# techshoww/RoMa

Measured on AMD Instinct MI355X. Metric: image-pairs/sec at 560->864, higher is better.
Workload: dtype fp16; 1 GPU; roma_outdoor 560->864 full coarse-to-fine symmetric match (BASELINE configs[1]; configs[2] = --pairs 8 --gpus 8); launch=eager launches, coarse_res=560, upsample_res=864, parallelism=single GPU

## Files before the change

include/roma_hip.h:

```cpp
#ifndef ROMA_HIP_H
#define ROMA_HIP_H

#include <stdint.h>

#ifdef __cplusplus
extern "C" {
#endif

#define ROMA_ABI_VERSION 5

enum { ROMA_F32 = 0, ROMA_F16 = 1, ROMA_BF16 = 2 };
enum { ROMA_NCHW = 0, ROMA_NHWC = 1 };
enum { ROMA_LC_AUTO = 0, ROMA_LC_TILE8X4 = 1, ROMA_LC_TILE8X8 = 2, ROMA_LC_ROWS8 = 3 };
enum { ROMA_E_ARG = -1, ROMA_E_DTYPE = -2, ROMA_E_SHAPE = -3, ROMA_E_ALIGN = -4, ROMA_E_UNSUPPORTED = -5 };

int roma_abi_version(void);
const char* roma_last_error(void);

int roma_local_corr(const void* f0, const void* f1, const float* flow, void* out,
                    int B, int C, int H, int W, int r, int dtype,
                    int layout, int f0_pitch, int f1_pitch, int out_layout, int out_pitch, int f1_batch_shift, int variant,
                    void* stream);

int roma_warp_bilinear(const void* src, const float* flow, void* dst,
                       int B, int C, int Hs, int Ws, int H, int W, int dtype,
                       int layout, int src_pitch, int dst_layout, int dst_pitch, int src_batch_shift, void* stream);

int roma_disp_emb(const float* flow, const float* weight, const float* bias, void* dst,
                  int B, int E, int H, int W, float gain, int dtype, int dst_layout, int dst_pitch, void* stream);

int roma_interp_bilinear(const float* x, float* y, int N, int Hi, int Wi, int Ho, int Wo, void* stream);

int roma_interp_bilinear_pair(const float* x0, float* y0, int N0, const float* x1, float* y1, int N1, int Hi, int Wi, int Ho, int Wo,
                              void* stream);

int roma_refiner_assemble(const void* src, const float* flow, const float* weight, const float* bias, void* buf, int B, int C, int E,
                          int D, int pitch, int Hs, int Ws, int H, int W, int src_pitch, int src_batch_shift, float gain, int dtype,
                          void* stream);

int roma_flow_update(float* flow, float* cert, const float* cert_in, const float* delta,
                     int B, int H, int W, float sx, float sy, void* stream);

int roma_cls_to_flow_refine(const void* logits, float* flow_out, float* cert_out,
                            int B, int C, int HW, long stride_b, long stride_c, long stride_p,
                            int dtype, void* stream);

int roma_cos_kernel(const void* x, const void* y, float* K, int B, int N, int M, int D, int dtype, int x_pitch, int y_pitch,
                    int y_batch_shift, float T, float eps, float diag_add, void* stream);

int roma_chol_diag_block(float* A, int lda, long strideA, float* W, int ldw, long strideW, int nb, int B, int* info,
                         int info_base, void* stream);

int roma_chol_step(float* A, int lda, long strideA, int n, int ncols, int j, int nb, const float* W, int ldw, long strideW, float* R,
                   int ldr, long strideR, float* Wn, int ldwn, long strideWn, int* info, int info_base, int B, void* stream);

int roma_chol_subst_step(int dir, const float* W, int ldw, long strideW, const float* R, long strideRb, long strideRs, int ldr, float* T,
                         long strideTb, long strideTs, int ldt, int t_in_panel, float* X, int ldx, long strideX, int n, int m, int nb,
                         int s, int B, void* stream);

int roma_attention_fwd(const void* q, const void* k, const void* v, void* o, int B, int H, int Nq, int Nk, int head_dim, long q_sb,
                       long q_sn, long q_sh, long k_sb, long k_sn, long k_sh, long v_sb, long v_sn, long v_sh, long o_sb, long o_sn,
                       long o_sh, float scale, int dtype, void* stream);

int roma_match_finalize(const float* flow, const float* cert, const float* cert16, float* warp, float* certainty,
                        int P, int H, int W, int H16, int W16, int symmetric, void* stream);

int roma_kde_density(const float* x, float* density, int N, int down, float std, int half_mode, void* stream);

int roma_race_keys(const float* p, const long* counter, float* keys, long N, float thresh, unsigned seed, unsigned stage,
                   void* stream);

long roma_race_select_workspace(int P, long N, int k);
int roma_race_select(const float* p, const long* counter, const long* seeds, int P, long N, int k, float thresh, unsigned stage,
                     long* sel_key, long* sel_idx, void* workspace, long workspace_bytes, void* stream);

int roma_kde_density_batch(const float* x, const long* index, float* density, int P, long N, int n, int down, float std,
                           int half_mode, void* stream);

int roma_nn_argmin(const float* q, const float* r, int* idx, int NQ, int NR, void* stream);

int roma_resample_u8(const void* in, void* out, int H, int W, int C, int out_size, int axis, const int* bounds,
                     const int* coef, int ksize, void* stream);
int roma_normalize_u8(const void* in, float* out, int H, int W, const float* mean3, const float* std3, void* stream);

int roma_bias_relu_nchw(void* x, const void* bias, int B, int C, int HW, int dtype, void* stream);

int roma_bias_relu_pool2_nchw(void* x, const void* bias, void* pooled, int B, int C, int H, int W, int dtype, void* stream);

int roma_bias_relu_nhwc(void* x, const void* bias, long npix, int C, int dtype, void* stream);
int roma_bias_relu_pool2_nhwc(void* x, const void* bias, void* pooled, int B, int C, int H, int W, int dtype, void* stream);

int roma_dwconv5x5_bn_relu(const void* x, const float* w, const float* scale, const float* shift, void* y,
                           int B, int C, int H, int W, int dtype, int x_pitch, int y_pitch, void* stream);

int roma_refiner_block(const void* x, const void* w25, const float* scale, const float* shift, const void* wt,
                       const float* bias, void* y, int B, int C, int H, int W, int kpad, int dtype, int x_pitch, int y_pitch,
                       void* stream);

int roma_refiner_wide_pack(const void* wt, void* wp, int D);
int roma_refiner_wide_taps(const void* w25, void* w25p, int D);
int roma_refiner_block_wide(const void* x, const void* w25p, const float* scale, const float* shift, const void* wp,
                            const float* bias, void* y, int B, int H, int W, int D, int x_pitch, int y_pitch, int dtype,
                            void* stream);

int roma_pointwise_mfma(const void* x, const void* wt, const float* bias, void* y, long M, int C, int kpad, int dtype,
                        int x_pitch, int y_pitch, void* stream);

int roma_refiner_block_mid(const void* x, const float* w25, const float* scale, const float* shift, const void* wt,
                           const float* bias, void* y, int B, int C, int H, int W, int dtype, int x_pitch, int y_pitch,
                           void* stream);

int roma_refiner_head(const void* x, const float* wo, const float* bo, float* flow, const float* cert_in, float* cert_out,
                      float* delta_out, int B, int H, int W, int C, int pitch, int dtype, float sx, float sy, void* stream);

int roma_pointwise_small(const void* x, const float* wt, const float* bias, void* y, long M, int C, int dtype,
                         int x_pitch, int y_pitch, void* stream);

int roma_project_skinny(const void* x, const void* wt, const float* bias, void* y, long M, int K, int N, int dtype, int x_pitch,
                        int y_pitch, void* stream);

int roma_add_layernorm(void* x, int x_dtype, long x_stride, const void* y, int y_dtype, long y_stride, const float* ls,
                       const float* gamma, const float* beta, void* out, int out_dtype, long out_stride, long rows, int C,
                       float eps, void* stream);

int roma_tiny_corr_posembed(const float* f0, const float* f1, float* out, int B, int C,
                            int H0, int W0, int H1, int W1, int exact, void* stream);

int roma_jpeg_info(const void* data, long nbytes, int* info);
int roma_jpeg_entropy_decode(const void* data, long nbytes, int16_t* coef, uint16_t* qt);
int roma_jpeg_reconstruct(const int16_t* coef, const uint16_t* qt, void* planes, void* rgb, const int* info, void* stream);

long roma_ransac_workspace(int kind, int P, int N, int iters, long* offsets);
int roma_ransac_hypotheses(int kind, const double* xa, const double* xb, int P, int N, int iters, float threshold, unsigned seed,
                           int p0, void* ws, long ws_bytes, void* stream);
int roma_ransac_select(int kind, const double* xa, const double* xb, int P, int N, int iters, float threshold, int lo_iters,
                       const void* ws, long ws_bytes, double* model, unsigned char* mask, void* stream);

int roma_ransac_hypotheses_ex(int kind, const double* xa, const double* xb, int P, int N, int iters, float threshold, int scoring,
                              unsigned seed, int p0, void* ws, long ws_bytes, void* stream);
int roma_ransac_select_ex(int kind, const double* xa, const double* xb, int P, int N, int iters, float threshold, int scoring,
                          int lo_iters, const void* ws, long ws_bytes, double* model, unsigned char* mask, void* stream);
int roma_magsac_table(float* loss, float* weight);

long roma_essential_workspace(int P, int N, int iters, long* offsets);
int roma_essential_hypotheses(const double* xa, const double* xb, const double* Ka, const double* Kb, int P, int N, int iters,
                              float threshold, unsigned seed, int p0, void* ws, long ws_bytes, void* stream);
int roma_essential_select(const double* xa, const double* xb, const double* Ka, const double* Kb, int P, int N, int iters,
                          float threshold, int lo_iters, const void* ws, long ws_bytes, double* E, unsigned char* mask, void* stream);
int roma_recover_pose(const double* xa, const double* xb, const double* Ka, const double* Kb, const double* E,
                      const unsigned char* mask_in, int P, int N, double* R, double* t, int* count, unsigned char* mask_out,
                      void* stream);

int roma_essential_hypotheses_ex(const double* xa, const double* xb, const double* Ka, const double* Kb, int P, int N, int iters,
                                 float threshold, int scoring, unsigned seed, int p0, void* ws, long ws_bytes, void* stream);
int roma_essential_select_ex(const double* xa, const double* xb, const double* Ka, const double* Kb, int P, int N, int iters,
                             float threshold, int scoring, int lo_iters, const void* ws, long ws_bytes, double* E, unsigned char* mask,
                             void* stream);

int roma_refine_pose(const double* xa, const double* xb, const double* Ka, const double* Kb, const double* R_in, const double* t_in,
                     const unsigned char* mask_in, int P, int N, double threshold, int iters, double* R, double* t,
                     unsigned char* mask, double* cost, int* count, int* steps, void* stream);

int roma_refine_fundamental(const double* xa, const double* xb, const double* F_in, const unsigned char* mask_in, int P, int N,
                            double threshold, int iters, double* F, unsigned char* mask, double* cost, int* count, int* steps,
                            void* stream);

int roma_refine_homography(const double* xa, const double* xb, const double* H_in, const unsigned char* mask_in, int P, int N,
                           double threshold, int iters, double* H, unsigned char* mask, double* cost, int* count, int* steps,
                           void* stream);

long roma_absolute_pose_workspace(int P, int N, int iters, long* offsets);
int roma_absolute_pose_hypotheses(const double* X, const double* x, const double* K, int P, int N, int iters, float threshold,
                                  int scoring, unsigned seed, int p0, void* ws, long ws_bytes, void* stream);
int roma_absolute_pose_select(const double* X, const double* x, const double* K, int P, int N, int iters, float threshold, int scoring,
                              int lo_iters, const void* ws, long ws_bytes, double* R, double* t, unsigned char* mask, void* stream);
int roma_refine_absolute_pose(const double* X, const double* x, const double* K, const double* R_in, const double* t_in,
                              const unsigned char* mask_in, int P, int N, double threshold, int iters, double* R, double* t,
                              unsigned char* mask, double* cost, int* count, int* steps, void* stream);

int roma_triangulate(const float* m, const float* to_px, const double* Ka, const double* Kb, const double* R, const double* t,
                     const unsigned char* mask_in, int P, int N, int method, float max_reproj, float max_cos_parallax, float* points,
                     float* depth_a, float* depth_b, float* reproj, float* cos_parallax, unsigned char* valid, void* stream);

int roma_triangulate_nview(const float* const* obs, const float* to_px, const unsigned char* const* visible, long vis_row_stride,
                           const double* K, const double* R, const double* t, int V, int rows, int row_len, long row_stride,
                           long point_stride, float max_view_error, int iters, int min_views, int ref_view, float max_reproj,
                           float max_cos_parallax, float* points, float* depth, float* reproj, float* cos_parallax, unsigned* views,
                           unsigned char* valid, void* stream);

int roma_warp_kpts(const float* x, int x_stride, const float* depth_a, const float* depth_b, const double* T, const double* Ka,
                   const double* Kb, int P, int N, int Ha, int Wa, int Hb, int Wb, int mode, double threshold, double* x2,
                   unsigned char* valid, double* rel_err, void* stream);

int roma_dense_match_metrics(const float* warp, long pitch, const float* depth_a, const float* depth_b, const double* T,
                             const double* Ka, const double* Kb, int P, int H, int W, int Ha, int Wa, int Hb, int Wb, int mode,
                             double threshold, void* workspace, long workspace_bytes, double* epe_sum, long long* counts, double* gd,
                             unsigned char* valid, void* stream);

#ifdef __cplusplus
}
#endif
#endif
```

roma_amd/_lib.py:

```python
from __future__ import annotations

import ctypes
import os
from ctypes import c_char_p, c_float, c_int, c_long, c_void_p

_HERE = os.path.dirname(os.path.abspath(__file__))
LIB_PATH = os.path.join(_HERE, "csrc", "libroma_hip.so")

ROMA_F32, ROMA_F16, ROMA_BF16 = 0, 1, 2
ROMA_NCHW, ROMA_NHWC = 0, 1
LC_VARIANTS = {"auto": 0, "tile8x4": 1, "tile8x8": 2, "rows8": 3}
ABI_VERSION = 5
SCORE_MSAC, SCORE_MAGSAC = 0, 1
ROMA_E_ARG, ROMA_E_DTYPE, ROMA_E_SHAPE, ROMA_E_ALIGN, ROMA_E_UNSUPPORTED = -1, -2, -3, -4, -5

SIGNATURES = {
    "roma_abi_version": [],
    "roma_last_error": [],
    "roma_local_corr": [c_void_p, c_void_p, c_void_p, c_void_p, c_int, c_int, c_int, c_int, c_int, c_int,
                        c_int, c_int, c_int, c_int, c_int, c_int, c_int, c_void_p],
    "roma_warp_bilinear": [c_void_p, c_void_p, c_void_p, c_int, c_int, c_int, c_int, c_int, c_int, c_int,
                           c_int, c_int, c_int, c_int, c_int, c_void_p],
    "roma_disp_emb": [c_void_p, c_void_p, c_void_p, c_void_p, c_int, c_int, c_int, c_int, c_float, c_int, c_int, c_int, c_void_p],
    "roma_interp_bilinear": [c_void_p, c_void_p, c_int, c_int, c_int, c_int, c_int, c_void_p],
    "roma_interp_bilinear_pair": [c_void_p, c_void_p, c_int, c_void_p, c_void_p, c_int, c_int, c_int, c_int, c_int, c_void_p],
    "roma_refiner_assemble": [c_void_p, c_void_p, c_void_p, c_void_p, c_void_p, c_int, c_int, c_int, c_int, c_int, c_int, c_int, c_int,
                              c_int, c_int, c_int, c_float, c_int, c_void_p],
    "roma_project_skinny": [c_void_p, c_void_p, c_void_p, c_void_p, c_long, c_int, c_int, c_int, c_int, c_int, c_void_p],
    "roma_flow_update": [c_void_p, c_void_p, c_void_p, c_void_p, c_int, c_int, c_int, c_float, c_float, c_void_p],
    "roma_cls_to_flow_refine": [c_void_p, c_void_p, c_void_p, c_int, c_int, c_int, c_long, c_long, c_long, c_int, c_void_p],
    "roma_cos_kernel": [c_void_p, c_void_p, c_void_p, c_int, c_int, c_int, c_int, c_int, c_int, c_int, c_int, c_float, c_float,
                        c_float, c_void_p],
    "roma_add_layernorm": [c_void_p, c_int, c_long, c_void_p, c_int, c_long, c_void_p, c_void_p, c_void_p, c_void_p, c_int, c_long,
                           c_long, c_int, c_float, c_void_p],
    "roma_attention_fwd": [c_void_p, c_void_p, c_void_p, c_void_p, c_int, c_int, c_int, c_int, c_int] + [c_long] * 12 + [c_float, c_int, c_void_p],
    "roma_chol_diag_block": [c_void_p, c_int, c_long, c_void_p, c_int, c_long, c_int, c_int, c_void_p, c_int, c_void_p],
    "roma_chol_step": [c_void_p, c_int, c_long, c_int, c_int, c_int, c_int, c_void_p, c_int, c_long, c_void_p, c_int, c_long,
                       c_void_p, c_int, c_long, c_void_p, c_int, c_int, c_void_p],
    "roma_chol_subst_step": [c_int, c_void_p, c_int, c_long, c_void_p, c_long, c_long, c_int, c_void_p, c_long, c_long, c_int, c_int,
                             c_void_p, c_int, c_long, c_int, c_int, c_int, c_int, c_int, c_void_p],
    "roma_match_finalize": [c_void_p, c_void_p, c_void_p, c_void_p, c_void_p, c_int, c_int, c_int, c_int, c_int, c_int, c_void_p],
    "roma_kde_density": [c_void_p, c_void_p, c_int, c_int, c_float, c_int, c_void_p],
    "roma_nn_argmin": [c_void_p, c_void_p, c_void_p, c_int, c_int, c_void_p],
    "roma_race_keys": [c_void_p, c_void_p, c_void_p, c_long, c_float, ctypes.c_uint, ctypes.c_uint, c_void_p],
    "roma_race_select_workspace": [c_int, c_long, c_int],
    "roma_race_select": [c_void_p, c_void_p, c_void_p, c_int, c_long, c_int, c_float, ctypes.c_uint, c_void_p, c_void_p, c_void_p, c_long,
                         c_void_p],
    "roma_kde_density_batch": [c_void_p, c_void_p, c_void_p, c_int, c_long, c_int, c_int, c_float, c_int, c_void_p],
    "roma_dwconv5x5_bn_relu": [c_void_p, c_void_p, c_void_p, c_void_p, c_void_p, c_int, c_int, c_int, c_int, c_int, c_int, c_int, c_void_p],
    "roma_resample_u8": [c_void_p, c_void_p, c_int, c_int, c_int, c_int, c_int, c_void_p, c_void_p, c_int, c_void_p],
    "roma_normalize_u8": [c_void_p, c_void_p, c_int, c_int, c_void_p, c_void_p, c_void_p],
    "roma_bias_relu_nchw": [c_void_p, c_void_p, c_int, c_int, c_int, c_int, c_void_p],
    "roma_bias_relu_pool2_nchw": [c_void_p, c_void_p, c_void_p, c_int, c_int, c_int, c_int, c_int, c_void_p],
    "roma_bias_relu_nhwc": [c_void_p, c_void_p, c_long, c_int, c_int, c_void_p],
    "roma_bias_relu_pool2_nhwc": [c_void_p, c_void_p, c_void_p, c_int, c_int, c_int, c_int, c_int, c_void_p],
    "roma_pointwise_mfma": [c_void_p, c_void_p, c_void_p, c_void_p, c_long, c_int, c_int, c_int, c_int, c_int, c_void_p],
    "roma_refiner_block": [c_void_p, c_void_p, c_void_p, c_void_p, c_void_p, c_void_p, c_void_p, c_int, c_int, c_int, c_int, c_int, c_int,
                           c_int, c_int, c_void_p],
    "roma_refiner_block_mid": [c_void_p, c_void_p, c_void_p, c_void_p, c_void_p, c_void_p, c_void_p, c_int, c_int, c_int, c_int, c_int, c_int,
                               c_int, c_void_p],
    "roma_refiner_wide_pack": [c_void_p, c_void_p, c_int],
    "roma_refiner_wide_taps": [c_void_p, c_void_p, c_int],
    "roma_jpeg_info": [c_void_p, c_long, c_void_p],
    "roma_jpeg_entropy_decode": [c_void_p, c_long, c_void_p, c_void_p],
    "roma_jpeg_reconstruct": [c_void_p, c_void_p, c_void_p, c_void_p, c_void_p, c_void_p],
    "roma_refiner_block_wide": [c_void_p, c_void_p, c_void_p, c_void_p, c_void_p, c_void_p, c_void_p, c_int, c_int, c_int, c_int, c_int, c_int,
                                c_int, c_void_p],
    "roma_refiner_head": [c_void_p, c_void_p, c_void_p, c_void_p, c_void_p, c_void_p, c_void_p, c_int, c_int, c_int, c_int, c_int, c_int,
                          c_float, c_float, c_void_p],
    "roma_pointwise_small": [c_void_p, c_void_p, c_void_p, c_void_p, c_long, c_int, c_int, c_int, c_int, c_void_p],
    "roma_tiny_corr_posembed": [c_void_p, c_void_p, c_void_p, c_int, c_int, c_int, c_int, c_int, c_int, c_int, c_void_p],
    "roma_ransac_workspace": [c_int, c_int, c_int, c_int, c_void_p],
    "roma_ransac_hypotheses": [c_int, c_void_p, c_void_p, c_int, c_int, c_int, c_float, ctypes.c_uint, c_int, c_void_p, c_long, c_void_p],
    "roma_ransac_select": [c_int, c_void_p, c_void_p, c_int, c_int, c_int, c_float, c_int, c_void_p, c_long, c_void_p, c_void_p,
                           c_void_p],
    "roma_ransac_hypotheses_ex": [c_int, c_void_p, c_void_p, c_int, c_int, c_int, c_float, c_int, ctypes.c_uint, c_int, c_void_p, c_long,
                                  c_void_p],
    "roma_ransac_select_ex": [c_int, c_void_p, c_void_p, c_int, c_int, c_int, c_float, c_int, c_int, c_void_p, c_long, c_void_p, c_void_p,
                              c_void_p],
    "roma_magsac_table": [c_void_p, c_void_p],
    "roma_essential_workspace": [c_int, c_int, c_int, c_void_p],
    "roma_essential_hypotheses": [c_void_p, c_void_p, c_void_p, c_void_p, c_int, c_int, c_int, c_float, ctypes.c_uint, c_int, c_void_p,
                                  c_long, c_void_p],
    "roma_essential_select": [c_void_p, c_void_p, c_void_p, c_void_p, c_int, c_int, c_int, c_float, c_int, c_void_p, c_long, c_void_p,
                              c_void_p, c_void_p],
    "roma_essential_hypotheses_ex": [c_void_p, c_void_p, c_void_p, c_void_p, c_int, c_int, c_int, c_float, c_int, ctypes.c_uint, c_int,
                                     c_void_p, c_long, c_void_p],
    "roma_essential_select_ex": [c_void_p, c_void_p, c_void_p, c_void_p, c_int, c_int, c_int, c_float, c_int, c_int, c_void_p, c_long,
                                 c_void_p, c_void_p, c_void_p],
    "roma_recover_pose": [c_void_p, c_void_p, c_void_p, c_void_p, c_void_p, c_void_p, c_int, c_int, c_void_p, c_void_p, c_void_p,
                          c_void_p, c_void_p],
    "roma_refine_pose": [c_void_p, c_void_p, c_void_p, c_void_p, c_void_p, c_void_p, c_void_p, c_int, c_int, ctypes.c_double, c_int,
                         c_void_p, c_void_p, c_void_p, c_void_p, c_void_p, c_void_p, c_void_p],
    "roma_refine_fundamental": [c_void_p, c_void_p, c_void_p, c_void_p, c_int, c_int, ctypes.c_double, c_int, c_void_p, c_void_p, c_void_p,
                                c_void_p, c_void_p, c_void_p],
    "roma_refine_homography": [c_void_p, c_void_p, c_void_p, c_void_p, c_int, c_int, ctypes.c_double, c_int, c_void_p, c_void_p, c_void_p,
                               c_void_p, c_void_p, c_void_p],
    "roma_triangulate": [c_void_p, c_void_p, c_void_p, c_void_p, c_void_p, c_void_p, c_void_p, c_int, c_int, c_int, c_float, c_float,
                         c_void_p, c_void_p, c_void_p, c_void_p, c_void_p, c_void_p, c_void_p],
    "roma_triangulate_nview": [c_void_p, c_void_p, c_void_p, c_long, c_void_p, c_void_p, c_void_p, c_int, c_int, c_int, c_long, c_long,
                               c_float, c_int, c_int, c_int, c_float, c_float, c_void_p, c_void_p, c_void_p, c_void_p, c_void_p, c_void_p,
                               c_void_p],
    "roma_warp_kpts": [c_void_p, c_int, c_void_p, c_void_p, c_void_p, c_void_p, c_void_p, c_int, c_int, c_int, c_int, c_int, c_int, c_int,
                       ctypes.c_double, c_void_p, c_void_p, c_void_p, c_void_p],
    "roma_dense_match_metrics": [c_void_p, c_long, c_void_p, c_void_p, c_void_p, c_void_p, c_void_p, c_int, c_int, c_int, c_int, c_int, c_int,
                                 c_int, c_int, ctypes.c_double, c_void_p, c_long, c_void_p, c_void_p, c_void_p, c_void_p, c_void_p],
    "roma_absolute_pose_workspace": [c_int, c_int, c_int, c_void_p],
    "roma_absolute_pose_hypotheses": [c_void_p, c_void_p, c_void_p, c_int, c_int, c_int, c_float, c_int, ctypes.c_uint, c_int, c_void_p,
                                      c_long, c_void_p],
    "roma_absolute_pose_select": [c_void_p, c_void_p, c_void_p, c_int, c_int, c_int, c_float, c_int, c_int, c_void_p, c_long, c_void_p,
                                  c_void_p, c_void_p, c_void_p],
    "roma_refine_absolute_pose": [c_void_p, c_void_p, c_void_p, c_void_p, c_void_p, c_void_p, c_int, c_int, ctypes.c_double, c_int,
                                  c_void_p, c_void_p, c_void_p, c_void_p, c_void_p, c_void_p, c_void_p],
}
_RESTYPES = {"roma_last_error": c_char_p, "roma_ransac_workspace": c_long, "roma_essential_workspace": c_long,
             "roma_race_select_workspace": c_long, "roma_absolute_pose_workspace": c_long}

_lib = None


class RomaHipError(RuntimeError):
    pass


def load() -> ctypes.CDLL:
    global _lib
    if _lib is not None:
        return _lib
    if not os.path.exists(LIB_PATH):
        raise RomaHipError(f"{LIB_PATH} is missing: build it with `python -c 'import __graft_entry__ as g; g.build()'` "
                           f"or `make -C roma_amd/csrc`.  roma_amd has no CPU/PyTorch fallback for its kernels.")
    lib = ctypes.CDLL(LIB_PATH)
    for name, argtypes in SIGNATURES.items():
        fn = getattr(lib, name)
        fn.argtypes = argtypes
        fn.restype = _RESTYPES.get(name, c_int)
    if lib.roma_abi_version() != ABI_VERSION:
        raise RomaHipError(f"libroma_hip.so ABI {lib.roma_abi_version()} != binding ABI {ABI_VERSION}")
    _lib = lib
    return lib


def check(rc: int, what: str):
    if rc == 0:
        return
    msg = load().roma_last_error().decode(errors="replace")
    if rc < 0:
        raise ValueError(f"{what}: {msg} (code {rc})")
    raise RomaHipError(f"{what}: HIP error {rc}: {msg}")
```

roma_amd/csrc/refiner_block.hip:

```cpp
#include <algorithm>
#include "common.h"
#include "lc_device.h"
#include "refiner_mid_device.h"

namespace roma {
namespace {

typedef _Float16 h8v __attribute__((ext_vector_type(8)));
typedef __bf16 b8v __attribute__((ext_vector_type(8)));

__device__ __forceinline__ float4_t mfma_blk(const u32x4& a, const u32x4& b, float4_t c, half_t) {
  return __builtin_amdgcn_mfma_f32_16x16x32_f16(__builtin_bit_cast(h8v, a), __builtin_bit_cast(h8v, b), c, 0, 0, 0);
}
__device__ __forceinline__ float4_t mfma_blk(const u32x4& a, const u32x4& b, float4_t c, bf16_t) {
  return __builtin_amdgcn_mfma_f32_16x16x32_bf16(__builtin_bit_cast(b8v, a), __builtin_bit_cast(b8v, b), c, 0, 0, 0);
}

struct RBParams {
  const void* x;
  void* y;
  const void* w25;
  const void* wt;
  const float* scale;
  const float* shift;
  const float* bias;
  int B, H, W, C, x_pitch, y_pitch;
  int tiles_x, tiles_y;
  float inv_tiles_per_img, inv_tiles_x;
};

constexpr int XT = 16, YT = 8, HX = XT + 4, HY = YT + 4, NPOS = HX * HY;

template <typename T, int KP>
__global__ __launch_bounds__(256, 1) void refiner_block_kernel(RBParams p) {
  constexpr int KPAD = 32 * KP;
  constexpr int NT = KPAD / 16;
  constexpr int RS = KPAD / 8 + 1;
  extern __shared__ __attribute__((aligned(16))) unsigned char smem[];
  u32x4* s_in = reinterpret_cast<u32x4*>(smem);
  u32x4* s_pw = s_in + NPOS * RS;
  u32x4* s_dw = s_pw + KPAD * RS;
  float* s_cs = reinterpret_cast<float*>(s_dw + 25 * (KPAD / 8));
  T* s_out = reinterpret_cast<T*>(s_in);
  constexpr int OS = KPAD + 8;

  const int tid = threadIdx.x, lane = tid & 63, wv = tid >> 6;
  const int m = lane & 15, kq = lane >> 4;
  const int PKT = p.C / 8;
  const T* x = static_cast<const T*>(p.x);
  T* y = static_cast<T*>(p.y);
  const int tiles_per_img = p.tiles_x * p.tiles_y;
  auto tile_origin = [&](int tile, int& b, int& ty0, int& tx0) {
    b = (int)(((float)tile + 0.5f) * p.inv_tiles_per_img);
    const int tt = tile - b * tiles_per_img;
    const int tyi = (int)(((float)tt + 0.5f) * p.inv_tiles_x);
    ty0 = tyi * YT;
    tx0 = (tt - tyi * p.tiles_x) * XT;
  };

  for (int i = tid; i < KPAD * (KPAD / 8); i += 256) {
    const int n = i / (KPAD / 8), k = i % (KPAD / 8);
    s_pw[n * RS + k] = reinterpret_cast<const u32x4*>(p.wt)[i];
  }
  for (int i = tid; i < 25 * (KPAD / 8); i += 256) s_dw[i] = reinterpret_cast<const u32x4*>(p.w25)[i];
  for (int i = tid; i < KPAD; i += 256) {
    s_cs[i] = p.scale[i];
    s_cs[KPAD + i] = p.shift[i];
    s_cs[2 * KPAD + i] = p.bias[i];
  }
  const int ntile = p.tiles_x * p.tiles_y * p.B;
  constexpr int NLD = (NPOS * (KPAD / 8) + 255) / 256;
  const int nload = NPOS * PKT;
  u32x4 pre[NLD];
  auto fetch = [&](int tile) {
    int b, ty0, tx0;
    tile_origin(tile, b, ty0, tx0);
    const T* xb = x + (size_t)b * p.H * p.W * p.x_pitch;
#pragma unroll
    for (int j = 0; j < NLD; ++j) {
      const int i = min(tid + j * 256, nload - 1);
      const int pos = i / PKT, k = i - pos * PKT;
      const int yy = ty0 - 2 + pos / HX, xx = tx0 - 2 + pos % HX;
      const bool ok = yy >= 0 && yy < p.H && xx >= 0 && xx < p.W;
      const int yc = min(max(yy, 0), p.H - 1), xc = min(max(xx, 0), p.W - 1);
      u32x4 v = *reinterpret_cast<const u32x4*>(xb + ((size_t)yc * p.W + xc) * p.x_pitch + k * 8);
      if (!ok) v = u32x4{0, 0, 0, 0};
      pre[j] = v;
    }
  };
  for (int i = tid; i < NPOS * (KPAD / 8 - PKT); i += 256) {
    const int pos = i / (KPAD / 8 - PKT), k = PKT + i % (KPAD / 8 - PKT);
    s_in[pos * RS + k] = u32x4{0, 0, 0, 0};
  }
  if ((int)blockIdx.x < ntile) fetch(blockIdx.x);
  for (int tile = blockIdx.x; tile < ntile; tile += gridDim.x) {
    int b, ty0, tx0;
    tile_origin(tile, b, ty0, tx0);
    __syncthreads();
#pragma unroll
    for (int j = 0; j < NLD; ++j) {
      const int i = tid + j * 256;
      if (i < nload) {
        const int pos = i / PKT, k = i - pos * PKT;
        s_in[pos * RS + k] = pre[j];
      }
    }
    __syncthreads();
    if (tile + (int)gridDim.x < ntile) fetch(tile + gridDim.x);
    u32x4 afrag[2][KP];
#pragma unroll
    for (int ks = 0; ks < KP; ++ks) {
      const int pk = 4 * ks + kq;
      float acc0[8], acc1[8];
#pragma unroll
      for (int e = 0; e < 8; ++e) acc0[e] = acc1[e] = 0.f;
#pragma unroll
      for (int dy = 0; dy < 6; ++dy) {
#pragma unroll
        for (int dx = 0; dx < 5; ++dx) {
          float fi[8];
          unpack16<T>(s_in[((2 * wv + dy) * HX + m + dx) * RS + pk], fi);
          if (dy < 5) {
            float fw[8];
            unpack16<T>(s_dw[(dy * 5 + dx) * (KPAD / 8) + pk], fw);
#pragma unroll
            for (int e = 0; e < 8; ++e) acc0[e] = __builtin_fmaf(fi[e], fw[e], acc0[e]);
          }
          if (dy >= 1) {
            float fw[8];
            unpack16<T>(s_dw[((dy - 1) * 5 + dx) * (KPAD / 8) + pk], fw);
#pragma unroll
            for (int e = 0; e < 8; ++e) acc1[e] = __builtin_fmaf(fi[e], fw[e], acc1[e]);
          }
        }
      }
      float v0[8], v1[8];
#pragma unroll
      for (int e = 0; e < 8; ++e) {
        const float sc = s_cs[pk * 8 + e], sh = s_cs[KPAD + pk * 8 + e];
        v0[e] = fmaxf(__builtin_fmaf(acc0[e], sc, sh), 0.f);
        v1[e] = fmaxf(__builtin_fmaf(acc1[e], sc, sh), 0.f);
      }
      afrag[0][ks] = pack16<T>(v0);
      afrag[1][ks] = pack16<T>(v1);
    }
    float4_t acc[2][NT];
#pragma unroll
    for (int nt = 0; nt < NT; ++nt) acc[0][nt] = acc[1][nt] = float4_t{0.f, 0.f, 0.f, 0.f};
#pragma unroll
    for (int nt = 0; nt < NT; ++nt) {
#pragma unroll
      for (int ks = 0; ks < KP; ++ks) {
        const u32x4 bfrag = s_pw[(nt * 16 + m) * RS + 4 * ks + kq];
        acc[0][nt] = mfma_blk(afrag[0][ks], bfrag, acc[0][nt], T{});
        acc[1][nt] = mfma_blk(afrag[1][ks], bfrag, acc[1][nt], T{});
      }
    }
    __syncthreads();
#pragma unroll
    for (int row = 0; row < 2; ++row)
#pragma unroll
      for (int nt = 0; nt < NT; ++nt) {
        const int ch = nt * 16 + m;
        const float bsv = s_cs[2 * KPAD + ch];
#pragma unroll
        for (int r4 = 0; r4 < 4; ++r4)
          s_out[((2 * wv + row) * XT + 4 * kq + r4) * OS + ch] = from_f32<T>(acc[row][nt][r4] + bsv);
      }
    __syncthreads();
    T* yb = y + (size_t)b * p.H * p.W * p.y_pitch;
    for (int i = tid; i < XT * YT * PKT; i += 256) {
      const int pix = i / PKT, k = i - pix * PKT;
      const int yy = ty0 + pix / XT, xx = tx0 + pix % XT;
      if (yy < p.H && xx < p.W)
        *reinterpret_cast<u32x4*>(yb + ((size_t)yy * p.W + xx) * p.y_pitch + k * 8) = *reinterpret_cast<const u32x4*>(s_out + pix * OS + k * 8);
    }
  }
}

template <typename T, int KP>
int launch_rb(RBParams p, hipStream_t s) {
  constexpr int KPAD = 32 * KP, RS = KPAD / 8 + 1;
  const size_t smem = (size_t)(NPOS * RS + KPAD * RS + 25 * (KPAD / 8)) * 16 + 3 * KPAD * 4;
  static std::atomic<uint64_t> attr_done{0};
  if (int rc = ensure_dyn_smem(reinterpret_cast<const void*>(refiner_block_kernel<T, KP>), (int)smem, attr_done, "roma_refiner_block")) return rc;
  const long ntile = (long)p.B * p.tiles_x * p.tiles_y;
  ROMA_REQUIRE(ntile < (1 << 21), ROMA_E_SHAPE, "roma_refiner_block: %ld tiles in one launch (< 2^21)", ntile);
  p.inv_tiles_per_img = 1.0f / (float)(p.tiles_x * p.tiles_y);
  p.inv_tiles_x = 1.0f / (float)p.tiles_x;
  const int per_cu = KP == 1 ? 4 : 1;
  const int grid = ntile < 256 * per_cu ? (int)ntile : 256 * per_cu;
  hipLaunchKernelGGL((refiner_block_kernel<T, KP>), dim3(grid), dim3(256), smem, s, p);
  ROMA_CHECK_LAUNCH();
}


constexpr int TPX = 16, TPY = 16, TPHX = TPX + 4, TPHY = TPY + 4;
constexpr int TP_PR = 64;
constexpr int TP_PLB = TPHY * TP_PR;
constexpr int TP_NCH = 24, TP_FRAG = 13 * 16;
constexpr int TP_TROW = TPX * 64 + 16;
constexpr int TP_OS = 40;
constexpr int TP_TOEP = TP_NCH * 5 * TP_FRAG;
constexpr int TP_PL = TP_NCH * TP_PLB, TP_TB = TPX * TPY * TP_OS * 2, TP_PW = 32 * 5 * 16;
constexpr int TP_SMEM = TP_TOEP + TP_PL + TP_TB + TP_PW + 3 * 32 * 4;
static_assert(TPY * TP_TROW <= TP_TB && 2 * TP_SMEM <= 160 * 1024, "LDS budget of the Toeplitz block: two workgroups per CU");

template <typename T>
__global__ __launch_bounds__(256, 2) void refiner_block_toep_kernel(RBParams p) {
  extern __shared__ __attribute__((aligned(16))) unsigned char smem[];
  unsigned char* s_toep = smem;
  unsigned char* s_pl = s_toep + TP_TOEP;
  unsigned char* s_t = s_pl + TP_PL;
  u32x4* s_pw = reinterpret_cast<u32x4*>(s_t + TP_TB);
  float* s_cs = reinterpret_cast<float*>(s_pw + 32 * 5);
  const int tid = threadIdx.x, lane = tid & 63;
  const int wv = __builtin_amdgcn_readfirstlane(tid >> 6);
  const int m = lane & 15, q = lane >> 4;
  const T* x = static_cast<const T*>(p.x);
  T* y = static_cast<T*>(p.y);
  const int tiles_per_img = p.tiles_x * p.tiles_y;
  auto tile_origin = [&](int tile, int& b, int& ty0, int& tx0) {
    b = (int)(((float)tile + 0.5f) * p.inv_tiles_per_img);
    const int tt = tile - b * tiles_per_img;
    const int tyi = (int)(((float)tt + 0.5f) * p.inv_tiles_x);
    ty0 = tyi * TPY;
    tx0 = (tt - tyi * p.tiles_x) * TPX;
  };

  {
    const T* w25 = static_cast<const T*>(p.w25);
    for (int i = tid; i < TP_NCH * 5 * 13; i += 256) {
      const int f = i / 13, wi = i - f * 13, c = f / 5, dy = f - c * 5;
      T v[8];
#pragma unroll
      for (int j = 0; j < 8; ++j) {
        const int dx = wi - 7 + j;
        v[j] = (wi < 12 && dx >= 0 && dx <= 4) ? w25[(dy * 5 + dx) * 32 + c] : from_f32<T>(0.f);
      }
      *reinterpret_cast<u32x4*>(s_toep + (size_t)i * 16) = *reinterpret_cast<const u32x4*>(v);
    }
    for (int i = tid; i < 32 * 4; i += 256) s_pw[(i >> 2) * 5 + (i & 3)] = reinterpret_cast<const u32x4*>(p.wt)[i];
    if (tid < 32) { s_cs[tid] = p.scale[tid]; s_cs[32 + tid] = p.shift[tid]; s_cs[64 + tid] = p.bias[tid]; }
    for (int i = tid; i < (TP_PL + TP_TB) / 16; i += 256) reinterpret_cast<u32x4*>(s_pl)[i] = u32x4{0, 0, 0, 0};
  }
  const int ntile = tiles_per_img * p.B;
  constexpr int NLD = (TPHX * TPHY * 3 + 255) / 256;
  u32x4 pre[NLD];
  uint32_t okm = 0;
  uint32_t pdst[NLD];
  int ihy[NLD], ihx[NLD], ik8[NLD];
#pragma unroll
  for (int j = 0; j < NLD; ++j) {
    const int idx = tid + 256 * j, idc = min(idx, TPHX * TPHY * 3 - 1);
    const int k = idc / (TPHX * TPHY), pos = idc - k * (TPHX * TPHY), hy = pos / TPHX, hx = pos - hy * TPHX;
    pdst[j] = idx < TPHX * TPHY * 3 ? (uint32_t)(k * 8 * TP_PLB + hy * TP_PR + hx * 2) : 0xffffffffu;
    ihy[j] = hy - 2; ihx[j] = hx - 2; ik8[j] = k * 8;
  }
  auto fetch = [&](int tile) {
    int b, ty0, tx0;
    tile_origin(tile, b, ty0, tx0);
    const T* xb = x + (size_t)b * p.H * p.W * p.x_pitch;
    okm = 0xffffffffu;
#pragma unroll
    for (int j = 0; j < NLD; ++j) {
      const int yy = ty0 + ihy[j], xx = tx0 + ihx[j];
      if (!(yy >= 0 && yy < p.H && xx >= 0 && xx < p.W)) okm &= ~(1u << j);
      pre[j] = *reinterpret_cast<const u32x4*>(xb + (uint32_t)((min(max(yy, 0), p.H - 1) * p.W + min(max(xx, 0), p.W - 1)) * p.x_pitch + ik8[j]));
    }
  };
  auto scatter = [&]() {
#pragma unroll
    for (int j = 0; j < NLD; ++j) {
      if (pdst[j] == 0xffffffffu) continue;
      const bool ok = (okm >> j) & 1u;
#pragma unroll
      for (int e = 0; e < 8; ++e) {
        const uint32_t w = ok ? pre[j][e >> 1] : 0u;
        *reinterpret_cast<uint16_t*>(s_pl + pdst[j] + e * TP_PLB) = (uint16_t)((e & 1) ? (w >> 16) : (w & 0xffffu));
      }
    }
  };
  const bool xcd_order = (gridDim.x & 7) == 0 && ntile >= 64;
  const int nx = xcd_order ? (int)(gridDim.x >> 3) : (int)gridDim.x;
  const int band = xcd_order ? (ntile + 7) >> 3 : ntile;
  const int t_beg = xcd_order ? (int)(blockIdx.x & 7) * band + (int)(blockIdx.x >> 3) : (int)blockIdx.x;
  const int t_end = xcd_order ? min(((int)(blockIdx.x & 7) + 1) * band, ntile) : ntile;
  if (t_beg < t_end) fetch(t_beg);
  __syncthreads();
  if (t_beg < t_end) scatter();
  if (t_beg + nx < t_end) fetch(t_beg + nx);
  __syncthreads();

  const int swz = (m >> 1) & 3;
  const int wsh = 8 * q - m;
  const int woff = (wsh >= -7 && wsh <= 4 ? wsh + 7 : 12) * 16;
  float scv[8], shv[8], bsv4[2][4];
#pragma unroll
  for (int e = 0; e < 8; ++e) { scv[e] = s_cs[min(wv, 2) * 8 + e]; shv[e] = s_cs[32 + min(wv, 2) * 8 + e]; }
#pragma unroll
  for (int nb = 0; nb < 2; ++nb)
#pragma unroll
    for (int i = 0; i < 4; ++i) bsv4[nb][i] = s_cs[64 + nb * 16 + 4 * q + i];
  for (int tile = t_beg; tile < t_end; tile += nx) {
    int b, ty0, tx0;
    tile_origin(tile, b, ty0, tx0);
    const bool more = tile + nx < t_end, more2 = tile + 2 * nx < t_end;
    if (wv < 3) {
      float vals[8][4];
      u32x4 av[5], bv[5];
      auto load_op = [&](int c, int dy, u32x4& a, u32x4& bq) {
        a = *reinterpret_cast<const u32x4*>(s_toep + (c * 5 + dy) * TP_FRAG + woff);
        bq = *reinterpret_cast<const u32x4*>(s_pl + c * TP_PLB + (m + dy) * TP_PR + q * 16);
      };
#pragma unroll
      for (int dy = 0; dy < 5; ++dy) load_op(wv * 8, dy, av[dy], bv[dy]);
#pragma unroll
      for (int e = 0; e < 8; ++e) {
        const int c = wv * 8 + e;
        u32x4 an[5], bn[5];
        float4_t acc = {0.f, 0.f, 0.f, 0.f};
#pragma unroll
        for (int dy = 0; dy < 5; ++dy) {
          __builtin_amdgcn_sched_barrier(0);
          acc = lc::mfma16r(av[dy], bv[dy], acc, T{});
          if (e < 7) load_op(c + 1, dy, an[dy], bn[dy]);
        }
        __builtin_amdgcn_sched_barrier(0);
#pragma unroll
        for (int i = 0; i < 4; ++i) vals[e][i] = fmaxf(__builtin_fmaf(acc[i], scv[e], shv[e]), 0.f);
        if (e < 7) {
#pragma unroll
          for (int dy = 0; dy < 5; ++dy) { av[dy] = an[dy]; bv[dy] = bn[dy]; }
        }
      }
#pragma unroll
      for (int i = 0; i < 4; ++i) {
        float f8[8];
#pragma unroll
        for (int e = 0; e < 8; ++e) f8[e] = vals[e][i];
        const int xo = 4 * q + i;
        *reinterpret_cast<u32x4*>(s_t + m * TP_TROW + xo * 64 + ((wv ^ ((xo >> 1) & 3)) << 4)) = pack16<T>(f8);
      }
    }
    __syncthreads();
    float4_t acc2[4][2];
#pragma unroll
    for (int r = 0; r < 4; ++r) {
      const u32x4 tb = *reinterpret_cast<const u32x4*>(s_t + (wv * 4 + r) * TP_TROW + m * 64 + ((q ^ swz) << 4));
#pragma unroll
      for (int nb = 0; nb < 2; ++nb) acc2[r][nb] = lc::mfma16r(s_pw[(nb * 16 + m) * 5 + q], tb, float4_t{0.f, 0.f, 0.f, 0.f}, T{});
    }
    __syncthreads();
    T* s_out = reinterpret_cast<T*>(s_t);
#pragma unroll
    for (int r = 0; r < 4; ++r)
#pragma unroll
      for (int nb = 0; nb < 2; ++nb) {
        T o4[4];
#pragma unroll
        for (int i = 0; i < 4; ++i) o4[i] = from_f32<T>(acc2[r][nb][i] + bsv4[nb][i]);
        *reinterpret_cast<uint2*>(s_out + ((wv * 4 + r) * TPX + m) * TP_OS + nb * 16 + 4 * q) = *reinterpret_cast<const uint2*>(o4);
      }
    if (more) scatter();
    if (more2) fetch(tile + 2 * nx);
    __syncthreads();
    T* yb = y + (size_t)b * p.H * p.W * p.y_pitch;
#pragma unroll
    for (int j = 0; j < 3; ++j) {
      const int i = tid + 256 * j, pix = i / 3, k = i - pix * 3;
      const int yy = ty0 + (pix >> 4), xx = tx0 + (pix & 15);
      if (yy < p.H && xx < p.W)
        *reinterpret_cast<u32x4*>(yb + ((size_t)yy * p.W + xx) * p.y_pitch + k * 8) = *reinterpret_cast<const u32x4*>(s_out + pix * TP_OS + k * 8);
    }
    __syncthreads();
    for (int i = tid; i < TPX * TPY; i += 256) {
      const int row = i >> 4, xo = i & 15;
      *reinterpret_cast<u32x4*>(s_t + row * TP_TROW + xo * 64 + ((3 ^ ((xo >> 1) & 3)) << 4)) = u32x4{0, 0, 0, 0};
    }
  }
}

template <typename T>
int launch_rb_toep(RBParams p, hipStream_t s) {
  static std::atomic<uint64_t> attr_done{0};
  if (int rc = ensure_dyn_smem(reinterpret_cast<const void*>(refiner_block_toep_kernel<T>), TP_SMEM, attr_done, "roma_refiner_block")) return rc;
  p.tiles_x = (p.W + TPX - 1) / TPX;
  p.tiles_y = (p.H + TPY - 1) / TPY;
  const long ntile = (long)p.B * p.tiles_x * p.tiles_y;
  ROMA_REQUIRE(ntile < (1 << 21), ROMA_E_SHAPE, "roma_refiner_block: %ld tiles in one launch (< 2^21)", ntile);
  p.inv_tiles_per_img = 1.0f / (float)(p.tiles_x * p.tiles_y);
  p.inv_tiles_x = 1.0f / (float)p.tiles_x;
  const int grid = ntile < 2 * num_cus() ? (int)ntile : 2 * num_cus();
  hipLaunchKernelGGL((refiner_block_toep_kernel<T>), dim3(grid), dim3(256), TP_SMEM, s, p);
  ROMA_CHECK_LAUNCH();
}

template <typename T>
int launch_rb_any(const RBParams& p, int kpad, hipStream_t s) {
  if (kpad == 32 && p.C == 24) return launch_rb_toep<T>(p, s);
  return kpad == 32 ? launch_rb<T, 1>(p, s) : launch_rb<T, 5>(p, s);
}



struct PWParams {
  const void* x;
  void* y;
  const void* wt;
  const float* bias;
  long M;
  int C, x_pitch, y_pitch;
};

template <typename T, int KP>
__global__ __launch_bounds__(256, 2) void pointwise_mfma_kernel(PWParams p) {
  constexpr int KPAD = 32 * KP, RS = KPAD / 8 + 1, OS = KPAD + 8;
  extern __shared__ __attribute__((aligned(16))) unsigned char smem[];
  u32x4* s_pw = reinterpret_cast<u32x4*>(smem);
  float* s_b = reinterpret_cast<float*>(s_pw + KPAD * RS);
  T* s_out = reinterpret_cast<T*>(s_b + KPAD);
  const int tid = threadIdx.x, lane = tid & 63, wv = tid >> 6;
  const int m = lane & 15, kq = lane >> 4;
  const int PKT = p.C / 8;
  for (int i = tid; i < KPAD * (KPAD / 8); i += 256) {
    const int n = i / (KPAD / 8), k = i % (KPAD / 8);
    s_pw[n * RS + k] = reinterpret_cast<const u32x4*>(p.wt)[i];
  }
  for (int i = tid; i < KPAD; i += 256) s_b[i] = p.bias[i];
  __syncthreads();
  const T* x = static_cast<const T*>(p.x);
  T* y = static_cast<T*>(p.y);
  T* so = s_out + wv * 16 * OS;
  const long ntile = (p.M + 15) / 16;
  for (long tile = (long)blockIdx.x * 4 + wv; tile < ntile; tile += (long)gridDim.x * 4) {
    const long row0 = tile * 16;
    const long r = row0 + m < p.M ? row0 + m : p.M - 1;
    u32x4 a[1][KP];
#pragma unroll
    for (int ks = 0; ks < KP; ++ks) {
      const int pk = 4 * ks + kq;
      u32x4 v = *reinterpret_cast<const u32x4*>(x + r * p.x_pitch + (pk < PKT ? pk : 0) * 8);
      if (pk >= PKT) v = u32x4{0, 0, 0, 0};
      a[0][ks] = v;
    }
    T* const stage[1] = {so};
    mid::pw_row_groups<T, KP, 1>(a, s_pw, s_b, stage, m, kq);
    for (int i = lane; i < 16 * PKT; i += 64) {
      const int row = i / PKT, k = i - row * PKT;
      if (row0 + row < p.M) *reinterpret_cast<u32x4*>(y + (row0 + row) * p.y_pitch + k * 8) = *reinterpret_cast<const u32x4*>(so + row * OS + k * 8);
    }
  }
}

template <typename T, int KP>
int launch_pw(const PWParams& p, hipStream_t s) {
  constexpr int KPAD = 32 * KP, RS = KPAD / 8 + 1, OS = KPAD + 8;
  const size_t smem = (size_t)KPAD * RS * 16 + KPAD * 4 + (size_t)4 * 16 * OS * sizeof(T);
  static std::atomic<uint64_t> attr_done{0};
  if (int rc = ensure_dyn_smem(reinterpret_cast<const void*>(pointwise_mfma_kernel<T, KP>), (int)smem, attr_done, "roma_pointwise_mfma")) return rc;
  const long need = (p.M + 63) / 64;
  const int grid = (int)(need < 512 ? need : 512);
  hipLaunchKernelGGL((pointwise_mfma_kernel<T, KP>), dim3(grid), dim3(256), smem, s, p);
  ROMA_CHECK_LAUNCH();
}

}
}

using namespace roma;

extern "C" int roma_refiner_block(const void* x, const void* w25, const float* scale, const float* shift, const void* wt,
                                  const float* bias, void* y, int B, int C, int H, int W, int kpad, int dtype, int x_pitch, int y_pitch,
                                  void* stream) {
  ROMA_REQUIRE(x && w25 && scale && shift && wt && bias && y, ROMA_E_ARG, "roma_refiner_block: null pointer");
  ROMA_REQUIRE(B > 0 && C > 0 && H > 0 && W > 0 && x_pitch >= C && y_pitch >= C, ROMA_E_SHAPE, "roma_refiner_block: bad shape");
  ROMA_REQUIRE(dtype == ROMA_F16 || dtype == ROMA_BF16, ROMA_E_DTYPE, "roma_refiner_block: fp16 / bf16 only (the fp32 parity mode uses the separate kernels)");
  ROMA_REQUIRE((kpad == 32 || kpad == 160) && C <= kpad && C % 8 == 0, ROMA_E_UNSUPPORTED, "roma_refiner_block: C=%d, kpad=%d (kpad must be 32 or 160, C a multiple of 8)", C, kpad);
  ROMA_REQUIRE(x_pitch % 8 == 0 && y_pitch % 8 == 0 && aligned16(x) && aligned16(y) && aligned16(w25) && aligned16(wt), ROMA_E_ALIGN,
               "roma_refiner_block: pitches must be multiples of 8 and bases 16-byte aligned");
  RBParams p{x, y, w25, wt, scale, shift, bias, B, H, W, C, x_pitch, y_pitch, (W + XT - 1) / XT, (H + YT - 1) / YT, 0.f, 0.f};
  hipStream_t s = static_cast<hipStream_t>(stream);
  return dtype == ROMA_F16 ? launch_rb_any<half_t>(p, kpad, s) : launch_rb_any<bf16_t>(p, kpad, s);
}

extern "C" int roma_pointwise_mfma(const void* x, const void* wt, const float* bias, void* y, long M, int C, int kpad, int dtype,
                                   int x_pitch, int y_pitch, void* stream) {
  ROMA_REQUIRE(x && wt && bias && y, ROMA_E_ARG, "roma_pointwise_mfma: null pointer");
  ROMA_REQUIRE(M > 0 && C > 0 && x_pitch >= C && y_pitch >= C, ROMA_E_SHAPE, "roma_pointwise_mfma: bad shape");
  ROMA_REQUIRE(dtype == ROMA_F16 || dtype == ROMA_BF16, ROMA_E_DTYPE, "roma_pointwise_mfma: fp16 / bf16 only");
  ROMA_REQUIRE((kpad == 32 || kpad == 160) && C <= kpad && C % 8 == 0, ROMA_E_UNSUPPORTED, "roma_pointwise_mfma: C=%d, kpad=%d", C, kpad);
  ROMA_REQUIRE(x_pitch % 8 == 0 && y_pitch % 8 == 0 && aligned16(x) && aligned16(y) && aligned16(wt), ROMA_E_ALIGN,
               "roma_pointwise_mfma: pitches must be multiples of 8 and bases 16-byte aligned");
  PWParams p{x, y, wt, bias, M, C, x_pitch, y_pitch};
  hipStream_t s = static_cast<hipStream_t>(stream);
  if (dtype == ROMA_F16) return kpad == 32 ? launch_pw<half_t, 1>(p, s) : launch_pw<half_t, 5>(p, s);
  return kpad == 32 ? launch_pw<bf16_t, 1>(p, s) : launch_pw<bf16_t, 5>(p, s);
}
```

roma_amd/csrc/refiner_head.hip:

```cpp
#include "common.h"

namespace roma {
namespace {

template <typename T, int L>
__global__ __launch_bounds__(256) void refiner_head_kernel(const T* __restrict__ x, const float* __restrict__ wo,
                                                          const float* __restrict__ bo, float* __restrict__ flow,
                                                          const float* __restrict__ cert_in, float* __restrict__ cert_out,
                                                          float* __restrict__ delta_out, int B, int HW, int C, int pitch, float sx, float sy) {
  constexpr int E = ElemTraits<T>::kPer16B;
  const int PK = C / E;
  const size_t M = (size_t)B * HW;
  const int sub = threadIdx.x % L;
  for (size_t m = ((size_t)blockIdx.x * blockDim.x + threadIdx.x) / L; m < M; m += (size_t)gridDim.x * blockDim.x / L) {
    float a0 = 0.f, a1 = 0.f, a2 = 0.f;
    for (int pk = sub; pk < PK; pk += L) {
      float f[E];
      unpack16<T>(*reinterpret_cast<const u32x4*>(x + m * pitch + pk * E), f);
      const float* w = wo + (size_t)pk * E * 3;
#pragma unroll
      for (int e = 0; e < E; ++e) {
        a0 = __builtin_fmaf(f[e], w[e * 3 + 0], a0);
        a1 = __builtin_fmaf(f[e], w[e * 3 + 1], a1);
        a2 = __builtin_fmaf(f[e], w[e * 3 + 2], a2);
      }
    }
#pragma unroll
    for (int o = L / 2; o > 0; o >>= 1) {
      a0 += __shfl_xor(a0, o, 64);
      a1 += __shfl_xor(a1, o, 64);
      a2 += __shfl_xor(a2, o, 64);
    }
    if (sub == 0) {
      a0 += bo[0]; a1 += bo[1]; a2 += bo[2];
      const int b = (int)(m / HW);
      const size_t p = m - (size_t)b * HW;
      float* fl = flow + (size_t)b * 2 * HW + p;
      fl[0] += sx * a0;
      fl[HW] += sy * a1;
      cert_out[m] = (cert_in ? cert_in[m] : 0.f) + a2;
      if (delta_out) {
        delta_out[(size_t)b * 3 * HW + p] = a0;
        delta_out[(size_t)b * 3 * HW + HW + p] = a1;
        delta_out[(size_t)b * 3 * HW + 2 * (size_t)HW + p] = a2;
      }
    }
  }
}

}
}

using namespace roma;

extern "C" int roma_refiner_head(const void* x, const float* wo, const float* bo, float* flow, const float* cert_in, float* cert_out,
                                 float* delta_out, int B, int H, int W, int C, int pitch, int dtype, float sx, float sy, void* stream) {
  ROMA_REQUIRE(x && wo && bo && flow && cert_out, ROMA_E_ARG, "roma_refiner_head: null pointer");
  ROMA_REQUIRE(B > 0 && H > 0 && W > 0 && C > 0 && pitch >= C, ROMA_E_SHAPE, "roma_refiner_head: bad shape");
  ROMA_REQUIRE(dtype >= ROMA_F32 && dtype <= ROMA_BF16, ROMA_E_DTYPE, "roma_refiner_head: unknown dtype %d", dtype);
  const int e = dtype == ROMA_F32 ? 4 : 8;
  ROMA_REQUIRE(C % e == 0 && pitch % e == 0 && aligned16(x), ROMA_E_ALIGN, "roma_refiner_head: C and pitch must be multiples of %d, x 16-byte aligned", e);
  hipStream_t s = static_cast<hipStream_t>(stream);
  const int pk = C / e;
  const int L = pk >= 64 ? 64 : (pk >= 16 ? 16 : 4);
  const size_t threads = (size_t)B * H * W * L;
  size_t g = (threads + 255) / 256;
  if (g > 32768) g = 32768;
#define ROMA_RH(T, LL) \
  hipLaunchKernelGGL((refiner_head_kernel<T, LL>), dim3((int)g), dim3(256), 0, s, (const T*)x, wo, bo, flow, cert_in, cert_out, delta_out, B, H * W, C, pitch, sx, sy)
#define ROMA_RH_T(T) \
  if (L == 64) { ROMA_RH(T, 64); } else if (L == 16) { ROMA_RH(T, 16); } else { ROMA_RH(T, 4); }
  if (dtype == ROMA_F32) { ROMA_RH_T(float) } else if (dtype == ROMA_F16) { ROMA_RH_T(half_t) } else { ROMA_RH_T(bf16_t) }
#undef ROMA_RH_T
#undef ROMA_RH
  ROMA_CHECK_LAUNCH();
}
```

roma_amd/csrc/refiner_mid.hip:

```cpp
#include "common.h"
#include "refiner_mid_device.h"

namespace roma {
namespace {

constexpr int MID_NT = 512;
constexpr int MID_KP = 5, MID_KPAD = 32 * MID_KP;
constexpr int MID_RS = MID_KPAD / 8 + 1;
constexpr int MID_SMAX = 28, MID_ROWS = MID_SMAX * mid::kStrip;
constexpr int MID_SMEM = (MID_ROWS * MID_RS + MID_KPAD * MID_RS) * 16 + 25 * MID_KPAD * 4 + MID_KPAD * 4 + MID_ROWS * 4 + 16 * (MID_KPAD / 8) * 4;
static_assert(MID_SMEM <= 160 * 1024, "LDS budget: t 75.3 KB + weights 53.8 KB + taps 16 KB + bias + the two index tables");
static_assert(MID_ROWS % 16 == 0 && MID_ROWS / 16 <= 16, "a wave takes row groups wv and wv + 8");

struct MidParams {
  const void* x;
  void* y;
  const float* w25;
  const float* scale;
  const float* shift;
  const void* wt;
  const float* bias;
  int B, H, W, C, x_pitch, y_pitch;
  int S;
  unsigned nstrip, ntile, band;
};

template <typename T>
__global__ __launch_bounds__(MID_NT) void refiner_mid_kernel(MidParams p) {
  constexpr int RS = MID_RS, OS = MID_KPAD + 8;
  static_assert(OS == RS * 8, "a staged output row is one row of t");
  extern __shared__ __attribute__((aligned(16))) unsigned char smem[];
  u32x4* s_t = reinterpret_cast<u32x4*>(smem);
  u32x4* s_pw = s_t + MID_ROWS * RS;
  float* s_w = reinterpret_cast<float*>(s_pw + MID_KPAD * RS);
  float* s_b = s_w + 25 * MID_KPAD;
  int* s_pix = reinterpret_cast<int*>(s_b + MID_KPAD);
  int* s_item = s_pix + MID_ROWS;
  const int tid = threadIdx.x;
  const int wv = __builtin_amdgcn_readfirstlane(tid >> 6);
  const int C = p.C, H = p.H, W = p.W, PK = C / 8, S = p.S;

  for (int i = tid; i < MID_KPAD * (MID_KPAD / 8); i += MID_NT) {
    const int n = i / (MID_KPAD / 8), k = i % (MID_KPAD / 8);
    s_pw[n * RS + k] = reinterpret_cast<const u32x4*>(p.wt)[i];
  }
  for (int i = tid; i < 25 * C / 4; i += MID_NT) reinterpret_cast<float4_t*>(s_w)[i] = reinterpret_cast<const float4_t*>(p.w25)[i];
  for (int i = tid; i < MID_KPAD; i += MID_NT) s_b[i] = p.bias[i];
  for (int i = tid; i < MID_ROWS; i += MID_NT) s_pix[i] = -1;
  for (int i = tid; i < 16 * (MID_KPAD / 8); i += MID_NT) s_item[i] = i < 16 * PK ? (i / PK) << 8 | (i % PK) : -1;
  __syncthreads();

  const T* x = static_cast<const T*>(p.x);
  T* y = static_cast<T*>(p.y);
  const unsigned WS = (unsigned)(W + mid::kStrip - 1) / mid::kStrip;
  const int sl = tid / PK, k = tid - sl * PK;
  const int ngrp = (S * mid::kStrip + 15) / 16;
  const unsigned nx = gridDim.x >> 3;
  const unsigned beg = (blockIdx.x & 7u) * p.band;
  const unsigned end = min(beg + p.band, p.ntile);
  for (unsigned tile = beg + (blockIdx.x >> 3); tile < end; tile += nx) {
    if (sl < S) {
      const unsigned strip = tile * (unsigned)S + (unsigned)sl;
      if (strip < p.nstrip) {
        unsigned r = strip;
        const int xs = (int)(r % WS) * mid::kStrip;
        r /= WS;
        const int ys = (int)(r % (unsigned)H), b = (int)(r / (unsigned)H);
        u32x4* trow = s_t + sl * mid::kStrip * RS + k;
        mid::dw_strip<T>(x, s_w, p.scale, p.shift, b, ys, xs, k * 8, C, H, W, p.x_pitch, mid::kStrip,
                         [&](int o, const u32x4& v) { trow[o * RS] = v; });
        if (k == 0) {
          const int pix0 = (b * H + ys) * W + xs;
#pragma unroll
          for (int o = 0; o < mid::kStrip; ++o) s_pix[sl * mid::kStrip + o] = xs + o < W ? pix0 + o : -1;
        }
      } else if (k == 0) {
#pragma unroll
        for (int o = 0; o < mid::kStrip; ++o) s_pix[sl * mid::kStrip + o] = -1;
      }
    }
    __syncthreads();
    int lane = tid & 63;
    asm volatile("" : "+v"(lane));
    const int m = lane & 15, kq = lane >> 4;
    auto fragments = [&](int g, u32x4 (&a)[MID_KP]) {
#pragma unroll
      for (int ks = 0; ks < MID_KP; ++ks) {
        const int pk = 4 * ks + kq;
        u32x4 v = s_t[(g * 16 + m) * RS + (pk < PK ? pk : 0)];
        if (pk >= PK) v = u32x4{0, 0, 0, 0};
        a[ks] = v;
      }
    };
    auto store_groups = [&](const int (&g)[2], auto ng) {
      constexpr int G = decltype(ng)::value, NIT = 16 * (MID_KPAD / 8) / 64;
      int item[NIT], pix[G][NIT];
#pragma unroll
      for (int j = 0; j < NIT; ++j) item[j] = s_item[lane + 64 * j];
#pragma unroll
      for (int q = 0; q < G; ++q)
#pragma unroll
        for (int j = 0; j < NIT; ++j) pix[q][j] = item[j] >= 0 ? s_pix[g[q] * 16 + (item[j] >> 8)] : -1;
#pragma unroll
      for (int q = 0; q < G; ++q) {
        const T* so = reinterpret_cast<const T*>(s_t + g[q] * 16 * RS);
#pragma unroll
        for (int j = 0; j < NIT; ++j)
          if (pix[q][j] >= 0)
            *reinterpret_cast<u32x4*>(y + (size_t)pix[q][j] * p.y_pitch + (item[j] & 255) * 8) =
                *reinterpret_cast<const u32x4*>(so + (item[j] >> 8) * OS + (item[j] & 255) * 8);
      }
    };
    if (wv + 8 < ngrp) {
      u32x4 a[2][MID_KP];
      fragments(wv, a[0]);
      fragments(wv + 8, a[1]);
      T* const stage[2] = {reinterpret_cast<T*>(s_t + wv * 16 * RS), reinterpret_cast<T*>(s_t + (wv + 8) * 16 * RS)};
      mid::pw_row_groups<T, MID_KP, 2>(a, s_pw, s_b, stage, m, kq);
      store_groups({wv, wv + 8}, std::integral_constant<int, 2>{});
    } else if (wv < ngrp) {
      u32x4 a[1][MID_KP];
      fragments(wv, a[0]);
      T* const stage[1] = {reinterpret_cast<T*>(s_t + wv * 16 * RS)};
      mid::pw_row_groups<T, MID_KP, 1>(a, s_pw, s_b, stage, m, kq);
      store_groups({wv, wv}, std::integral_constant<int, 1>{});
    }
    __syncthreads();
  }
}

template <typename T>
int launch_mid(MidParams p, hipStream_t s) {
  static std::atomic<uint64_t> attr_done{0};
  if (int rc = ensure_dyn_smem(reinterpret_cast<const void*>(refiner_mid_kernel<T>), MID_SMEM, attr_done, "roma_refiner_block_mid")) return rc;
  const int cus = num_cus() & ~7;
  ROMA_REQUIRE(cus >= 8, ROMA_E_UNSUPPORTED, "roma_refiner_block_mid: needs a device with at least 8 compute units");
  const unsigned want = (p.ntile + 7u) & ~7u;
  const int grid = want < (unsigned)cus ? (int)want : cus;
  hipLaunchKernelGGL((refiner_mid_kernel<T>), dim3(grid), dim3(MID_NT), MID_SMEM, s, p);
  ROMA_CHECK_LAUNCH();
}

}
}

using namespace roma;

extern "C" int roma_refiner_block_mid(const void* x, const float* w25, const float* scale, const float* shift, const void* wt,
                                      const float* bias, void* y, int B, int C, int H, int W, int dtype, int x_pitch, int y_pitch,
                                      void* stream) {
  ROMA_REQUIRE(x && w25 && scale && shift && wt && bias && y, ROMA_E_ARG, "roma_refiner_block_mid: null pointer");
  ROMA_REQUIRE(B > 0 && C > 0 && H > 0 && W > 0 && x_pitch >= C && y_pitch >= C, ROMA_E_SHAPE, "roma_refiner_block_mid: bad shape");
  ROMA_REQUIRE(dtype == ROMA_F16 || dtype == ROMA_BF16, ROMA_E_DTYPE, "roma_refiner_block_mid: fp16 / bf16 only");
  ROMA_REQUIRE(C > 32 && C <= MID_KPAD && C % 8 == 0, ROMA_E_UNSUPPORTED,
               "roma_refiner_block_mid: C=%d (a multiple of 8, 32 < C <= 160)", C);
  ROMA_REQUIRE(x_pitch % 8 == 0 && y_pitch % 8 == 0 && aligned16(x) && aligned16(y) && aligned16(w25) && aligned16(scale) &&
                   aligned16(shift) && aligned16(wt),
               ROMA_E_ALIGN, "roma_refiner_block_mid: pitches must be multiples of 8 and bases 16-byte aligned");
  const size_t npix = (size_t)B * H * W;
  ROMA_REQUIRE(npix * x_pitch * 2 < (1ull << 32) && npix * y_pitch * 2 < (1ull << 32), ROMA_E_SHAPE,
               "roma_refiner_block_mid: a map of 4 GB or more in one launch");
  const char *xb = static_cast<const char*>(x), *yb = static_cast<const char*>(y);
  ROMA_REQUIRE(yb + npix * y_pitch * 2 <= xb || xb + npix * x_pitch * 2 <= yb, ROMA_E_ARG, "roma_refiner_block_mid: x and y overlap");
  MidParams p{x, y, w25, scale, shift, wt, bias, B, H, W, C, x_pitch, y_pitch, 0, 0, 0, 0};
  const int S0 = MID_NT / (C / 8);
  p.S = S0 < MID_SMAX ? S0 : MID_SMAX;
  p.nstrip = (unsigned)((size_t)B * H * ((W + mid::kStrip - 1) / mid::kStrip));
  p.ntile = (p.nstrip + p.S - 1) / p.S;
  p.band = (p.ntile + 7) / 8;
  hipStream_t s = static_cast<hipStream_t>(stream);
  return dtype == ROMA_F16 ? launch_mid<half_t>(p, s) : launch_mid<bf16_t>(p, s);
}
```

roma_amd/csrc/refiner_wide.hip:

```cpp
#include "common.h"
#include "lc_device.h"

namespace roma {
namespace {

using lc::mfma16r;

struct RWParams {
  const void* x;
  void* y;
  const void* w25p;
  const void* wp;
  const float* scale;
  const float* shift;
  const float* bias;
  int B, H, W, x_pitch, y_pitch, tiles_x, tiles_y;
};

typedef const __attribute__((address_space(4))) float cfloat;
__device__ __forceinline__ cfloat* as_const(const float* p) { return (cfloat*)(uintptr_t)p; }

constexpr int TW = 16, TH = 8, HXW = TW + 4, HYH = TH + 4, HPR = 16;
constexpr int PLANE = HYH * HPR * 32 + 16;
constexpr int NTAPV = 5 * 4 * 2 * 6;

template <typename T, int D>
__global__ __launch_bounds__(512, 1) void refiner_wide_kernel(RWParams p) {
  constexpr int NKP = D / 32, NB = D / 16, NBW = NB / 4, MBW = 4;
  constexpr int WBUF = D * 64, XBUF = 4 * PLANE, TBUF = TW * TH * 64, DWBUF = NTAPV * 16;
  static_assert(NB % 4 == 0 && 2 * (WBUF + XBUF + TBUF + DWBUF) <= 160 * 1024, "tile does not fit");
  extern __shared__ __attribute__((aligned(16))) unsigned char smem[];
  unsigned char* s_w = smem;
  unsigned char* s_x = s_w + 2 * WBUF;
  unsigned char* s_t = s_x + 2 * XBUF;
  unsigned char* s_dw = s_t + 2 * TBUF;
  const uint32_t lds_w = (uint32_t)(size_t)(__attribute__((address_space(3))) unsigned char*)s_w;

  const int tid = threadIdx.x, lane = tid & 63;
  const int wave = __builtin_amdgcn_readfirstlane(tid >> 6);
  const int tiles = p.tiles_x * p.tiles_y;
  const int b = blockIdx.x / tiles, tt = blockIdx.x - b * tiles;
  const int ty0 = (tt / p.tiles_x) * TH, tx0 = (tt % p.tiles_x) * TW;
  const T* xb = static_cast<const T*>(p.x) + (size_t)b * p.H * p.W * p.x_pitch;
  T* yb = static_cast<T*>(p.y) + (size_t)b * p.H * p.W * p.y_pitch;

  uint32_t xsrc[2], xdst;
  bool xok[2], xuse;
  {
    const int pr = min(tid >> 2, (HXW / 2) * HYH - 1), kql = tid & 3;
    const int hy = pr / (HXW / 2), jj = pr - hy * (HXW / 2);
    const int yy = ty0 - 2 + hy;
    xuse = tid < 4 * (HXW / 2) * HYH;
#pragma unroll
    for (int s = 0; s < 2; ++s) {
      const int xx = tx0 - 2 + 2 * jj + s;
      xok[s] = xuse && yy >= 0 && yy < p.H && xx >= 0 && xx < p.W;
      xsrc[s] = (uint32_t)((min(max(yy, 0), p.H - 1) * p.W + min(max(xx, 0), p.W - 1)) * p.x_pitch + kql * 8);
    }
    xdst = (uint32_t)(kql * PLANE + (hy * HPR + jj) * 32);
  }
  u32x4 xreg[2], dwreg;
  auto load_x = [&](int kp) {
#pragma unroll
    for (int s = 0; s < 2; ++s) xreg[s] = *reinterpret_cast<const u32x4*>(xb + xsrc[s] + kp * 32);
    if (tid < NTAPV) dwreg = reinterpret_cast<const u32x4*>(p.w25p)[kp * NTAPV + tid];
  };
  auto store_x = [&](int buf) {
    if (xuse) {
      const u32x4 a = xok[0] ? xreg[0] : u32x4{0, 0, 0, 0}, c = xok[1] ? xreg[1] : u32x4{0, 0, 0, 0};
      u32x4 lo, hi;
      lo[0] = __builtin_amdgcn_perm(c[0], a[0], 0x05040100u); lo[1] = __builtin_amdgcn_perm(c[0], a[0], 0x07060302u);
      lo[2] = __builtin_amdgcn_perm(c[1], a[1], 0x05040100u); lo[3] = __builtin_amdgcn_perm(c[1], a[1], 0x07060302u);
      hi[0] = __builtin_amdgcn_perm(c[2], a[2], 0x05040100u); hi[1] = __builtin_amdgcn_perm(c[2], a[2], 0x07060302u);
      hi[2] = __builtin_amdgcn_perm(c[3], a[3], 0x05040100u); hi[3] = __builtin_amdgcn_perm(c[3], a[3], 0x07060302u);
      *reinterpret_cast<u32x4*>(s_x + buf * XBUF + xdst) = lo;
      *reinterpret_cast<u32x4*>(s_x + buf * XBUF + xdst + 16) = hi;
    }
    if (tid < NTAPV) *reinterpret_cast<u32x4*>(s_dw + buf * DWBUF + tid * 16) = dwreg;
  };
  auto dma_w_all = [&](int kp, int buf) {
    const unsigned char* src = static_cast<const unsigned char*>(p.wp) + (size_t)kp * WBUF;
#pragma unroll
    for (int k = 0; k < (WBUF / 1024 + 7) / 8; ++k) {
      const int ii = k * 8 + wave;
      if (ii < WBUF / 1024) lc::dma16_so(src, (uint32_t)(ii * 1024 + lane * 16), lds_w + (uint32_t)(buf * WBUF + ii * 1024));
    }
  };
  const int kq = wave & 3;
  const int hsel = lane & 1, jp = (lane >> 1) & 7;
  const int prow = (wave >> 2) * 4 + (lane >> 4);
  const int ple = prow * 16 + 2 * jp;
  const uint32_t xrd = (uint32_t)(kq * PLANE + ((prow * HPR + jp) * 2 + hsel) * 16);
  const uint32_t twr = (uint32_t)(ple * 64 + ((kq ^ ((ple >> 1) & 3)) << 4) + hsel * 8);
  const int n16 = lane & 15, kg = lane >> 4;
  const int mh = wave & 1, nq = wave >> 1;
  const uint32_t fo = (uint32_t)(n16 * 64 + ((kg ^ ((n16 >> 1) & 3)) << 4));
  float4_t acc[NBW][MBW];
#pragma unroll
  for (int nb = 0; nb < NBW; ++nb)
#pragma unroll
    for (int mb = 0; mb < MBW; ++mb) acc[nb][mb] = float4_t{0.f, 0.f, 0.f, 0.f};

  auto dw_panel = [&](int kp, int buf) {
    const int c0 = __builtin_amdgcn_readfirstlane(kp * 32 + kq * 8);
    const unsigned char* wts = s_dw + buf * DWBUF + (kq * 2 + hsel) * 96;
    float ae[4], ao[4];
#pragma unroll
    for (int e = 0; e < 4; ++e) ae[e] = ao[e] = 0.f;
    const unsigned char* xs = s_x + buf * XBUF + xrd;
#pragma unroll
    for (int dy = 0; dy < 5; ++dy) {
      u32x4 ev[3], tv[6];
#pragma unroll
      for (int k = 0; k < 3; ++k) ev[k] = *reinterpret_cast<const u32x4*>(xs + (dy * HPR + k) * 32);
#pragma unroll
      for (int q = 0; q < 6; ++q) tv[q] = *reinterpret_cast<const u32x4*>(wts + dy * (4 * 2 * 96) + q * 16);
      __builtin_amdgcn_sched_barrier(0);
#pragma unroll
      for (int k = 0; k < 3; ++k)
#pragma unroll
        for (int e = 0; e < 4; ++e) {
          const half2_t xe = __builtin_bit_cast(half2_t, (uint32_t)ev[k][e]);
          ae[e] = __builtin_amdgcn_fdot2(xe, __builtin_bit_cast(half2_t, (uint32_t)tv[k][e]), ae[e], false);
          ao[e] = __builtin_amdgcn_fdot2(xe, __builtin_bit_cast(half2_t, (uint32_t)tv[3 + k][e]), ao[e], false);
        }
      __builtin_amdgcn_sched_barrier(0);
    }
    cfloat* sc = as_const(p.scale) + c0;
    cfloat* sh = as_const(p.shift) + c0;
    uint32_t oe[2], oo[2];
#pragma unroll
    for (int e = 0; e < 4; e += 2) {
      float re[2], ro[2];
#pragma unroll
      for (int i = 0; i < 2; ++i) {
        const float scv = hsel ? sc[4 + e + i] : sc[e + i], shv = hsel ? sh[4 + e + i] : sh[e + i];
        re[i] = fmaxf(__builtin_fmaf(ae[e + i], scv, shv), 0.f);
        ro[i] = fmaxf(__builtin_fmaf(ao[e + i], scv, shv), 0.f);
      }
      oe[e >> 1] = __builtin_bit_cast(uint32_t, half2_t{(half_t)re[0], (half_t)re[1]});
      oo[e >> 1] = __builtin_bit_cast(uint32_t, half2_t{(half_t)ro[0], (half_t)ro[1]});
    }
    *reinterpret_cast<uint2*>(s_t + buf * TBUF + twr) = uint2{oe[0], oe[1]};
    *reinterpret_cast<uint2*>(s_t + buf * TBUF + twr + 64) = uint2{oo[0], oo[1]};
  };
  static_assert(4 * NBW == WBUF / 1024, "one weight DMA per wave 0-3 and MFMA block");
  auto mfma_panel = [&](int buf, int kpn) {
    const unsigned char* tb = s_t + buf * TBUF + mh * (MBW * 1024) + fo;
    const unsigned char* wb = s_w + buf * WBUF + nq * (NBW * 1024) + fo;
    const unsigned char* src = static_cast<const unsigned char*>(p.wp) + (size_t)max(kpn, 0) * WBUF;
    u32x4 bt[MBW];
#pragma unroll
    for (int mb = 0; mb < MBW; ++mb) bt[mb] = *reinterpret_cast<const u32x4*>(tb + mb * 1024);
#pragma unroll
    for (int nb = 0; nb < NBW; ++nb) {
      if (kpn >= 0) {
        const int ii = nb * 4 + wave;
        lc::dma16_so(src, (uint32_t)(ii * 1024 + lane * 16), lds_w + (uint32_t)((buf ^ 1) * WBUF + ii * 1024));
      }
      const u32x4 aw = *reinterpret_cast<const u32x4*>(wb + nb * 1024);
#pragma unroll
      for (int mb = 0; mb < MBW; ++mb) acc[nb][mb] = mfma16r(aw, bt[mb], acc[nb][mb], T{});
    }
  };

  dma_w_all(0, 0);
  load_x(0);
  store_x(0);
  if (NKP > 1) load_x(1);
  __syncthreads();
  dw_panel(0, 0);
  if (NKP > 1) store_x(1);
  asm volatile("s_waitcnt vmcnt(0)" ::: "memory");
  __syncthreads();
  auto phase = [&](int kp, auto buf_c) {
    constexpr int buf = decltype(buf_c)::value;
    if (kp + 2 < NKP) load_x(kp + 2);
    const bool dw_first = wave >= 4;
    if (dw_first && kp + 1 < NKP) dw_panel(kp + 1, buf ^ 1);
    mfma_panel(buf, !dw_first && kp + 1 < NKP ? kp + 1 : -1);
    if (!dw_first && kp + 1 < NKP) dw_panel(kp + 1, buf ^ 1);
    if (kp + 2 < NKP) store_x(buf);
    asm volatile("s_waitcnt vmcnt(0)" ::: "memory");
    __syncthreads();
  };
  for (int kp = 0; kp < NKP; kp += 2) {
    phase(kp, std::integral_constant<int, 0>{});
    if (kp + 1 < NKP) phase(kp + 1, std::integral_constant<int, 1>{});
  }
  constexpr int OPITCH = D * 2 + 16;
  static_assert(TW * TH * OPITCH <= 160 * 1024, "output tile fits LDS");
  unsigned char* s_o = smem;
#pragma unroll
  for (int nb = 0; nb < NBW; ++nb) {
    const int ch = (nq * NBW + nb) * 16 + 4 * kg;
    const float4_t bv = *reinterpret_cast<const float4_t*>(p.bias + ch);
#pragma unroll
    for (int mb = 0; mb < MBW; ++mb) {
      const float4_t v = acc[nb][mb] + bv;
      const half2_t lo{(half_t)v[0], (half_t)v[1]}, hi{(half_t)v[2], (half_t)v[3]};
      uint2 pk;
      pk.x = __builtin_bit_cast(uint32_t, lo);
      pk.y = __builtin_bit_cast(uint32_t, hi);
      *reinterpret_cast<uint2*>(s_o + ((mh * MBW + mb) * 16 + n16) * OPITCH + ch * 2) = pk;
    }
  }
  __syncthreads();
  constexpr int PKR = D / 8;
  for (int id = tid; id < TW * TH * PKR; id += 512) {
    const int px = id / PKR, pk = id - px * PKR;
    const int oy = ty0 + (px >> 4), ox = tx0 + (px & 15);
    if (oy < p.H && ox < p.W)
      *reinterpret_cast<u32x4*>(yb + (size_t)(oy * p.W + ox) * p.y_pitch + pk * 8) = *reinterpret_cast<const u32x4*>(s_o + px * OPITCH + pk * 16);
  }
}

}
}

using namespace roma;

extern "C" int roma_refiner_wide_pack(const void* wt, void* wp, int D) {
  ROMA_REQUIRE(wt && wp, ROMA_E_ARG, "roma_refiner_wide_pack: null pointer");
  ROMA_REQUIRE(D > 0 && D % 64 == 0, ROMA_E_SHAPE, "roma_refiner_wide_pack: D = %d must be a multiple of 64", D);
  const uint16_t* src = static_cast<const uint16_t*>(wt);
  uint16_t* dst = static_cast<uint16_t*>(wp);
  for (int kp = 0; kp < D / 32; ++kp)
    for (int n = 0; n < D; ++n)
      for (int slot = 0; slot < 4; ++slot) {
        const int kgl = slot ^ ((n >> 1) & 3);
        for (int e = 0; e < 8; ++e) dst[((size_t)kp * D + n) * 32 + slot * 8 + e] = src[(size_t)n * D + kp * 32 + kgl * 8 + e];
      }
  return 0;
}

extern "C" int roma_refiner_wide_taps(const void* w25, void* w25p, int D) {
  ROMA_REQUIRE(w25 && w25p, ROMA_E_ARG, "roma_refiner_wide_taps: null pointer");
  ROMA_REQUIRE(D > 0 && D % 32 == 0, ROMA_E_SHAPE, "roma_refiner_wide_taps: D = %d must be a multiple of 32", D);
  const uint16_t* src = static_cast<const uint16_t*>(w25);
  uint16_t* dst = static_cast<uint16_t*>(w25p);
  static const int lo[6] = {0, 2, 4, -1, 1, 3}, hi[6] = {1, 3, -1, 0, 2, 4};
  size_t o = 0;
  for (int kp = 0; kp < D / 32; ++kp)
    for (int dy = 0; dy < 5; ++dy)
      for (int kq = 0; kq < 4; ++kq)
        for (int h = 0; h < 2; ++h)
          for (int st = 0; st < 6; ++st)
            for (int ch = 0; ch < 4; ++ch) {
              const int c = kp * 32 + kq * 8 + h * 4 + ch;
              dst[o++] = lo[st] < 0 ? (uint16_t)0 : src[(size_t)(dy * 5 + lo[st]) * D + c];
              dst[o++] = hi[st] < 0 ? (uint16_t)0 : src[(size_t)(dy * 5 + hi[st]) * D + c];
            }
  return 0;
}

extern "C" int roma_refiner_block_wide(const void* x, const void* w25p, const float* scale, const float* shift, const void* wp,
                                       const float* bias, void* y, int B, int H, int W, int D, int x_pitch, int y_pitch, int dtype,
                                       void* stream) {
  ROMA_REQUIRE(x && w25p && scale && shift && wp && bias && y, ROMA_E_ARG, "roma_refiner_block_wide: null pointer");
  ROMA_REQUIRE(B > 0 && H > 0 && W > 0, ROMA_E_SHAPE, "roma_refiner_block_wide: bad shape");
  ROMA_REQUIRE(D == 576 && dtype == ROMA_F16, ROMA_E_UNSUPPORTED, "roma_refiner_block_wide: built for D = 576, fp16 (got D = %d, dtype %d)", D, dtype);
  ROMA_REQUIRE(x_pitch >= D && y_pitch >= D && x_pitch % 8 == 0 && y_pitch % 4 == 0 && aligned16(x) && aligned16(wp) && aligned16(w25p) &&
               aligned16(y) && y_pitch % 8 == 0 && aligned16(bias), ROMA_E_ALIGN, "roma_refiner_block_wide: pitch / alignment");
  ROMA_REQUIRE((size_t)H * W * x_pitch < (1ull << 31), ROMA_E_SHAPE, "roma_refiner_block_wide: map too large for 32-bit offsets");
  RWParams p{x, y, w25p, wp, scale, shift, bias, B, H, W, x_pitch, y_pitch, (W + TW - 1) / TW, (H + TH - 1) / TH};
  constexpr int smem_loop = 2 * (576 * 64 + 4 * PLANE + TW * TH * 64 + NTAPV * 16), smem_out = TW * TH * (576 * 2 + 16);
  constexpr int smem = smem_loop > smem_out ? smem_loop : smem_out;
  static std::atomic<uint64_t> attr_done{0};
  if (int rc = ensure_dyn_smem(reinterpret_cast<const void*>(refiner_wide_kernel<half_t, 576>), smem, attr_done, "roma_refiner_block_wide")) return rc;
  hipLaunchKernelGGL((refiner_wide_kernel<half_t, 576>), dim3(B * p.tiles_x * p.tiles_y), dim3(512), smem, static_cast<hipStream_t>(stream), p);
  ROMA_CHECK_LAUNCH();
}
```

roma_amd/matcher.py:

```python
from __future__ import annotations

import math
import os
from collections import namedtuple
from typing import Dict, Optional
from warnings import warn

import numpy as np
import torch
import torch.nn as nn
import torch.nn.functional as F

from . import ops
from .transformer import Block, TransformerDecoder

IMAGENET_MEAN = (0.485, 0.456, 0.406)
IMAGENET_STD = (0.229, 0.224, 0.225)


def pixel_grid(b, h, w, device):
    ys = torch.linspace(-1 + 1 / h, 1 - 1 / h, h, device=device)
    xs = torch.linspace(-1 + 1 / w, 1 - 1 / w, w, device=device)
    return torch.stack((xs[None, :].expand(h, w), ys[:, None].expand(h, w)), dim=0)[None].expand(b, 2, h, w).contiguous()


def _params_version(module):
    return tuple((p.data_ptr(), 0 if p.is_inference() else p._version) for p in list(module.parameters()) + list(module.buffers()))


def _zero_pad(t, *shape):
    out = torch.zeros(shape, dtype=t.dtype, device=t.device)
    out[tuple(slice(0, s) for s in t.shape)] = t
    return out


BlockInOut = namedtuple("BlockInOut", "w25 scale shift wt_in_out bias")
BlockOutIn = namedtuple("BlockOutIn", "w25 scale shift wt_out_in bias")
BlockWide = namedtuple("BlockWide", "taps scale shift wt_panels bias")
RefinerPlan = namedtuple("RefinerPlan", "D Dp blocks wo bo we be")


def padded_width(D):
    m = 64 if D > 160 else 8
    return (D + m - 1) // m * m


def block_impl(Dp, dtype, B, h, w):
    half = dtype in (torch.float16, torch.bfloat16)
    if dtype == torch.float16 and Dp == 576 and B * ((h + 7) // 8) * ((w + 15) // 16) >= 2 * 256:
        return "wide"
    if half and Dp <= 32:
        return "fused"
    if half and Dp <= 160:
        return "split_mfma"
    return "split_small" if Dp <= 32 else "split_gemm"


MID_ONE_MIN_PIXELS = 2 * 280 * 280


def mid_block_impl(dtype, Dp, B, h, w):
    half = dtype in (torch.float16, torch.bfloat16)
    if not (half and 32 < Dp <= 160):
        return "two"
    return "one" if B * h * w >= MID_ONE_MIN_PIXELS else "two"


def project_impl(dtype, channels_last, K, N, out_pitch):
    half = dtype in (torch.float16, torch.bfloat16)
    if half and channels_last and (K, N) in ((64, 9), (128, 64)) and out_pitch % 8 == 0:
        return "skinny"
    return "gemm"


def assemble_impl(dtype, y_channels_last, y_pitch, C, E, D, Dp):
    half = dtype in (torch.float16, torch.bfloat16)
    if not (half and y_channels_last and y_pitch % 8 == 0):
        return "split"
    if C % 8 == 0 and E % 8 == 0:
        return "fused"
    return "fused" if (C, E, D, Dp) == (9, 6, 24, 24) and y_pitch >= 16 else "split"


class ConvRefiner(nn.Module):

    def __init__(self, in_dim, hidden_dim, out_dim, hidden_blocks, displacement_emb_dim, local_corr_radius=None,
                 amp_dtype=torch.float16):
        super().__init__()
        assert in_dim == hidden_dim, "depthwise refiner blocks keep the channel count (all shipped models)"

        def block(i, o):
            return nn.Sequential(nn.Conv2d(i, o, 5, 1, 2, groups=i), nn.BatchNorm2d(o), nn.ReLU(inplace=True), nn.Conv2d(o, o, 1, 1, 0))

        self.block1 = block(in_dim, hidden_dim)
        self.hidden_blocks = nn.Sequential(*[block(hidden_dim, hidden_dim) for _ in range(hidden_blocks)])
        self.out_conv = nn.Conv2d(hidden_dim, out_dim, 1, 1, 0)
        self.disp_emb = nn.Conv2d(2, displacement_emb_dim, 1, 1, 0)
        self.has_displacement_emb = True
        self.local_corr_radius = local_corr_radius
        self.in_dim, self.out_dim = in_dim, out_dim
        self.amp_dtype = amp_dtype
        self._prep = None

    def prepare(self, dtype):
        key = (dtype, _params_version(self))
        if self._prep is not None and self._prep[0] == key:
            return self._prep[1]
        D = self.in_dim
        Dp = padded_width(D)
        dev = self.out_conv.weight.device
        blocks = {impl: [] for impl in (block_impl(Dp, dtype, 1, 1, 1), block_impl(Dp, dtype, 512, 8, 16))}
        for blk in [self.block1] + list(self.hidden_blocks):
            dw, bn, _, pw = blk
            s = bn.weight.float() / torch.sqrt(bn.running_var.float() + bn.eps)
            w25 = torch.zeros(25, Dp, device=dev)
            w25[:, :D] = dw.weight.float().reshape(D, 25).t()
            scale = torch.zeros(Dp, device=dev)
            shift = torch.zeros(Dp, device=dev)
            scale[:D] = s
            b_dw = dw.bias.float() if dw.bias is not None else torch.zeros(D, device=dev)
            shift[:D] = (b_dw - bn.running_mean.float()) * s + bn.bias.float()
            wt = torch.zeros(Dp, Dp, device=dev)
            wt[:D, :D] = pw.weight.float().reshape(D, D).t()
            b = torch.zeros(Dp, device=dev)
            b[:D] = pw.bias.float()
            for impl, out in blocks.items():
                if impl == "wide":
                    out.append(BlockWide(ops.refiner_wide_taps(w25, dtype), scale, shift, ops.refiner_wide_pack(wt.t().contiguous().to(dtype)), b))
                elif impl == "fused":
                    out.append(BlockOutIn(_zero_pad(w25, 25, 32).to(dtype), _zero_pad(scale, 32), _zero_pad(shift, 32),
                                          _zero_pad(wt.t(), 32, 32).to(dtype), _zero_pad(b, 32)))
                elif impl == "split_mfma":
                    out.append(BlockOutIn(w25, scale, shift, _zero_pad(wt.t(), 160, 160).to(dtype), _zero_pad(b, 160)))
                else:
                    out.append(BlockInOut(w25, scale, shift, wt.to(dtype), b.to(dtype)))
        wo = torch.zeros(Dp, self.out_dim, device=dev)
        wo[:D] = self.out_conv.weight.float().reshape(self.out_dim, D).t()
        prep = RefinerPlan(D, Dp, blocks, wo.contiguous(), self.out_conv.bias.float(),
                           self.disp_emb.weight.float().reshape(-1, 2).contiguous(), self.disp_emb.bias.float())
        self._prep = (key, prep)
        return prep

    def new_buffer(self, B, h, w, dtype, device):
        return torch.empty((B, h, w, self.prepare(dtype).Dp), dtype=dtype, device=device)

    @torch.no_grad()
    def _body(self, x, y, flow, scale_factor, dtype, buf=None, batch_shift=0):
        P = self.prepare(dtype)
        B, C, h, w = x.shape
        D, Dp = P.D, P.Dp
        E = P.we.shape[0]
        r = self.local_corr_radius
        K = (2 * r + 1) ** 2 if r else 0
        assert 2 * C + E + K == D, "feature width does not match this refiner"
        x_in_place = buf is not None
        if buf is None:
            buf = torch.empty((B, h, w, Dp), dtype=dtype, device=x.device)
        assert buf.shape == (B, h, w, Dp) and buf.dtype == dtype and buf.is_contiguous()
        d = buf.permute(0, 3, 1, 2)
        if x_in_place:
            assert x.data_ptr() == buf.data_ptr() and x.stride(1) == 1, "x must already be channels [0, C) of buf"
        else:
            d[:, :C].copy_(x)
        yy = y.to(dtype)
        y_layout, y_pitch, yy = ops.feat_layout(yy)
        y_ok = y_layout == ops.ROMA_NHWC and yy.data_ptr() % 16 == 0
        if assemble_impl(dtype, y_ok, y_pitch, C, E, D, Dp) == "fused":
            ops.refiner_assemble(buf, yy, flow, P.we, P.be, 40 / 32 * scale_factor, C, D, batch_shift=batch_shift)
        else:
            if Dp > D:
                buf[..., D:].zero_()
            ops.warp_bilinear(yy, flow, out=d[:, C:2 * C], batch_shift=batch_shift)
            ops.disp_emb(flow, P.we, P.be, 40 / 32 * scale_factor, out=d[:, 2 * C:2 * C + E])
        if r:
            ops.local_correlation(d[:, :C], yy, r, flow=flow, out=d[:, 2 * C + E:D], batch_shift=batch_shift)
        impl = block_impl(Dp, dtype, B, h, w)
        cur = buf
        mid_one = impl == "split_mfma" and mid_block_impl(dtype, Dp, B, h, w) == "one"
        nxt = torch.empty_like(buf) if impl in ("wide", "fused") or mid_one else None
        for blk in P.blocks[impl]:
            if impl == "wide":
                ops.refiner_block_wide(cur, blk.taps, blk.scale, blk.shift, blk.wt_panels, blk.bias, out=nxt)
                cur, nxt = nxt, cur
            elif impl == "fused":
                ops.refiner_block(cur, blk.w25, blk.scale, blk.shift, blk.wt_out_in, blk.bias, Dp, out=nxt)
                cur, nxt = nxt, cur
            elif mid_one:
                ops.refiner_block_mid(cur, blk.w25, blk.scale, blk.shift, blk.wt_out_in, blk.bias, Dp, out=nxt)
                cur, nxt = nxt, cur
            else:
                t = ops.dwconv5x5_bn_relu(cur.permute(0, 3, 1, 2), blk.w25, blk.scale, blk.shift)
                rows = t.permute(0, 2, 3, 1).reshape(B * h * w, Dp)
                if impl == "split_mfma":
                    cur = ops.pointwise_mfma(rows, blk.wt_out_in, blk.bias, Dp)
                elif impl == "split_small":
                    cur = ops.pointwise_small(rows, blk.wt_in_out, blk.bias)
                else:
                    cur = torch.addmm(blk.bias, rows, blk.wt_in_out)
                cur = cur.view(B, h, w, Dp)
        return cur, P

    @torch.no_grad()
    def forward(self, x, y, flow, scale_factor=1, logits=None, dtype=None):
        flow = flow.float().contiguous()
        cur, P = self._body(x, y, flow, scale_factor, dtype or self.amp_dtype)
        B, h, w, Dp = cur.shape
        out = torch.addmm(P.bo, cur.reshape(B * h * w, Dp).float(), P.wo)
        out = out.view(B, h, w, self.out_dim).permute(0, 3, 1, 2).contiguous()
        return out[:, :-1], out[:, -1:]

    @torch.no_grad()
    def forward_update(self, x, y, flow, certainty, scale_factor, sx, sy, dtype=None, buf=None, batch_shift=0):
        cur, P = self._body(x, y, flow, scale_factor, dtype or self.amp_dtype, buf=buf, batch_shift=batch_shift)
        return ops.refiner_head(cur, P.wo, P.bo, flow, certainty, sx, sy)


class CosKernel(nn.Module):
    def __init__(self, T=0.2, learn_temperature=False):
        super().__init__()
        self.T = T

    def __call__(self, x, y, eps=1e-6):
        return ops.cos_kernel(x, y, T=self.T, eps=eps)


class GP(nn.Module):

    def __init__(self, gp_dim=512, T=0.2, sigma_noise=0.1, kernel=None, **_):
        super().__init__()
        self.K = CosKernel(T=T)
        self.sigma_noise = sigma_noise
        self.pos_conv = nn.Conv2d(2, gp_dim, 1, 1)
        self.dim = gp_dim
        self._basis = {}

    def basis(self, b, h, w, device):
        key = (h, w, device, _params_version(self.pos_conv))
        f = self._basis.get(key)
        if f is None:
            g = pixel_grid(1, h, w, device)
            f = torch.cos(8 * math.pi * F.conv2d(g, self.pos_conv.weight.float(), self.pos_conv.bias.float()))
            f = f.flatten(2).transpose(1, 2).contiguous()
            self._basis = {key: f}
        return f.expand(b, -1, -1)

    @torch.no_grad()
    def forward(self, x, y, **kwargs):
        b, c, h1, w1 = x.shape
        _, _, h2, w2 = y.shape
        xs = x.float().flatten(2).transpose(1, 2).contiguous()
        ys = y.float().flatten(2).transpose(1, 2).contiguous()
        K_yy = ops.cos_kernel(ys, ys, T=self.K.T, diag_add=self.sigma_noise)
        K_xy = ops.cos_kernel(xs, ys, T=self.K.T)
        mu = self.posterior_product(K_xy, ops.spd_solve(K_yy, self.basis(1, h2, w2, x.device)))
        return mu.transpose(1, 2).reshape(b, self.dim, h1, w1)

    def posterior_rows(self, xs, ys, h2, w2, fp64=False, batch_shift=0, out=None, check="now"):
        B, n = xs.shape[0], xs.shape[1]
        s = batch_shift % B
        basis = self.basis(1, h2, w2, xs.device)
        if fp64:
            a = xs.double()
            c = (a.roll(-s, 0) if s else a) if ys is None else ys.double()

            def cosk(u, v):
                g = torch.einsum("bnd,bmd->bnm", u, v) / (u.norm(dim=-1)[..., None] * v.norm(dim=-1)[:, None] + 1e-6)
                return ((g - 1.0) / self.K.T).exp()

            Kyy = cosk(c, c) + self.sigma_noise * torch.eye(c.shape[1], device=c.device, dtype=torch.float64)
            Z = torch.cholesky_solve(basis.double().expand(B, -1, -1), torch.linalg.cholesky(Kyy))
            mu = (cosk(a, c) @ Z).float()
            if out is not None:
                out.copy_(mu)
                return out
            return mu
        if ys is None:
            K_self = ops.cos_kernel(xs, xs, T=self.K.T, diag_add=self.sigma_noise)
            K_xy = ops.cos_kernel(xs, xs, T=self.K.T, batch_shift=s)
            Z = ops.spd_solve(K_self, basis, check=check)
            if s:
                assert 2 * s == B, "only the half swap of forward_symmetric"
                Z = torch.cat((Z[s:], Z[:s]), dim=0)
        else:
            K_yy = ops.cos_kernel(ys, ys, T=self.K.T, diag_add=self.sigma_noise)
            K_xy = ops.cos_kernel(xs, ys, T=self.K.T)
            Z = ops.spd_solve(K_yy, basis, check=check)
        return self.posterior_product(K_xy, Z, out)

    @staticmethod
    def posterior_product(K_xy, Z, out=None):
        mu = torch.bmm(K_xy.double(), Z.double())
        if out is None:
            return mu.float()
        out.copy_(mu)
        return out


class Decoder(nn.Module):
    def __init__(self, embedding_decoder, gps, proj, conv_refiner, detach=True, scales=("16", "8", "4", "2", "1"),
                 amp_dtype=torch.float16, **_):
        super().__init__()
        self.embedding_decoder, self.gps, self.proj, self.conv_refiner = embedding_decoder, gps, proj, conv_refiner
        self.scales = list(scales)
        self.refine_init = 4
        self.amp_dtype = amp_dtype
        self.gp_precision = "fp32"
        self.record = None
        self.flow_override = None
        self._proj = None

    def _embedding_decoder_for(self, dtype):
        if dtype == torch.float32:
            return self.embedding_decoder
        key = (dtype, _params_version(self.embedding_decoder))
        hit = self.__dict__.get("_embed_cast")
        if hit is None or hit[0] != key:
            import copy
            with torch.inference_mode(False), torch.no_grad():
                cp = copy.deepcopy(self.embedding_decoder).eval()
                for m in cp.modules():
                    if isinstance(m, nn.Linear):
                        m.to(dtype)
                hit = (key, cp)
            self.__dict__["_embed_cast"] = hit
        return hit[1]

    def get_placeholder_flow(self, b, h, w, device):
        return pixel_grid(b, h, w, device)

    def folded_proj(self, dtype):
        key = (dtype, _params_version(self.proj))
        if self._proj is not None and self._proj[0] == key:
            return self._proj[1]
        out = {}
        for s, seq in self.proj.items():
            conv, bn = seq[0], seq[1]
            g = bn.weight.float() / torch.sqrt(bn.running_var.float() + bn.eps)
            wt = (conv.weight.float().reshape(conv.out_channels, -1) * g[:, None]).t().contiguous().to(dtype)
            b = ((conv.bias.float() - bn.running_mean.float()) * g + bn.bias.float()).to(dtype)
            out[s] = (wt, b)
            if wt.shape[1] < 16:
                out[s + "/16"] = (F.pad(wt, (0, 16 - wt.shape[1])).contiguous(), F.pad(b, (0, 16 - b.shape[0])).contiguous())
            if project_impl(dtype, True, *wt.shape, 8) == "skinny":
                out[s + "/skinny"] = ops.project_skinny_pack(wt, b)
        self._proj = (key, out)
        return out

    def project(self, s, f, dtype, out=None):
        proj = self.folded_proj(dtype)
        wt, b = proj[s]
        B, C, h, w = f.shape
        f = f.to(dtype)
        n = wt.shape[1]
        dense_nhwc = f.stride() == (h * w * C, 1, w * C, C) and f.data_ptr() % 16 == 0
        if out is None:
            pitch = (n + 15) // 16 * 16 if project_impl(dtype, dense_nhwc, C, n, 8) == "skinny" else n
            out = torch.empty((B, h, w, pitch), dtype=dtype, device=f.device)[..., :n]
        out_rows = out.stride() == (h * w * out.stride(2), w * out.stride(2), out.stride(2), 1) and out.data_ptr() % 16 == 0
        if project_impl(dtype, dense_nhwc and out_rows, C, n, out.stride(2)) == "skinny":
            ops.project_skinny(f.permute(0, 2, 3, 1).reshape(B * h * w, C), *proj[s + "/skinny"], n,
                               out.as_strided((B * h * w, n), (out.stride(2), 1)))
            return out.permute(0, 3, 1, 2)
        tgt = out
        if n < 16 and out.stride(2) >= 16 and out.storage_offset() == 0:
            tgt = out.as_strided((B, h, w, 16), out.stride())
            wt, b = proj[s + "/16"]
        torch.baddbmm(b, f.flatten(2).transpose(1, 2), wt.unsqueeze(0).expand(B, -1, -1), out=tgt.view(B, h * w, tgt.shape[-1]))
        return out.permute(0, 3, 1, 2)

    @torch.no_grad()
    def forward(self, f1, f2, gt_warp=None, gt_prob=None, upsample=False, flow=None, certainty=None, scale_factor=1,
                swapped_pair=False, wait_events=None):
        dtype = self.amp_dtype
        all_scales = self.scales if not upsample else ["8", "4", "2", "1"]
        sizes = {s: tuple(f1[s].shape[-2:]) for s in f1}
        h, w = sizes[1]
        b = f1[1].shape[0]
        device = f1[1].device
        first = int(all_scales[0])
        if not upsample:
            flow = pixel_grid(b, *sizes[first], device)
            certainty = None
        else:
            flow, certainty = ops.interp_bilinear_pair(flow, certainty, sizes[first])
        corresps = {}
        for s in all_scales:
            ins = int(s)
            corresps[ins] = {}
            if wait_events and ins in wait_events:
                torch.cuda.current_stream().wait_event(wait_events[ins])
            hs, ws = sizes[ins]
            refiner = self.conv_refiner[s]
            buf = refiner.new_buffer(b, hs, ws, dtype, device)
            x = self.project(s, f1[ins], dtype, out=buf[..., :self.proj[s][0].out_channels])
            shift = 0
            if swapped_pair:
                y, shift = x, b // 2
            else:
                y = self.project(s, f2[ins], dtype)
            if ins in self.embedding_decoder.scales():
                n = hs * ws
                xs = x.permute(0, 2, 3, 1).reshape(b, n, -1)
                ys = None if swapped_pair else y.permute(0, 2, 3, 1).reshape(b, n, -1)
                gp = self.gps[s]
                C = xs.shape[2]
                npad = n if dtype == torch.float32 else n + (-n % 128)
                tokens = torch.empty((b, npad, gp.dim + C), dtype=torch.float32, device=device)
                if npad > n:
                    tokens[:, n:].zero_()
                tokens[:, :n, gp.dim:].copy_(xs)
                capturing = torch.cuda.is_current_stream_capturing()
                gp.posterior_rows(xs, ys, hs, ws, fp64=(self.gp_precision == "fp64"), batch_shift=shift,
                                  out=tokens[:, :n, :gp.dim],
                                  check=None if capturing else ("defer" if ops.deferring() else "now"))
                rows = self._embedding_decoder_for(dtype).forward_rows(tokens, n_valid=n, owned=True)
                flow, certainty = ops.cls_rows_to_flow(rows, b, hs, ws)
                if self.record is not None and not upsample:
                    self.record["argmax16"] = rows[..., :-1].float().argmax(dim=-1).cpu()
                    self.record["mu16"] = tokens[:, :n, :gp.dim].detach().clone()
            if self.flow_override is not None:
                forced = self.flow_override(ins, b, hs, ws, device, upsample)
                if forced is not None:
                    flow = forced
            flow, certainty = refiner.forward_update(
                x, y, flow, certainty, scale_factor, ins / (self.refine_init * w), ins / (self.refine_init * h), dtype=dtype, buf=buf,
                batch_shift=shift)
            corresps[ins].update({"certainty": certainty, "flow": flow})
            if s != "1":
                flow, certainty = ops.interp_bilinear_pair(flow, certainty, sizes[ins // 2])
        return corresps


def _check_rgb(im):
    if im.mode != "RGB":
        raise NotImplementedError("Can't handle non-RGB images")


def _check_not_i16(im):
    if im.mode == "I;16":
        raise NotImplementedError("Can't handle 16 bit images")


def preprocess(im, size):
    from PIL import Image
    h, w = size
    a = np.array(im.resize((w, h), Image.BICUBIC), dtype=np.float32).transpose(2, 0, 1) / 255.0
    t = torch.from_numpy(a)
    return (t - torch.tensor(IMAGENET_MEAN)[:, None, None]) / torch.tensor(IMAGENET_STD)[:, None, None]


class RegressionMatcher(nn.Module):
    def __init__(self, encoder, decoder, h=448, w=448, sample_mode="threshold_balanced", upsample_preds=False,
                 symmetric=False, name=None, attenuate_cert=None):
        super().__init__()
        self.attenuate_cert = attenuate_cert
        self.encoder, self.decoder = encoder, decoder
        self.name = name
        self.w_resized, self.h_resized = w, h
        self.sample_mode = sample_mode
        self.upsample_preds = upsample_preds
        self.upsample_res = (14 * 16 * 6, 14 * 16 * 6)
        self.symmetric = symmetric
        self.sample_thresh = 0.05
        self.host_preprocess = False
        self.device_jpeg = True

    def get_output_resolution(self):
        return self.upsample_res if self.upsample_preds else (self.h_resized, self.w_resized)

    def extract_backbone_features(self, batch, batched=True, upsample=False):
        if batched:
            return self.encoder(torch.cat((batch["im_A"], batch["im_B"]), dim=0), upsample=upsample)
        return self.encoder(batch["im_A"], upsample=upsample), self.encoder(batch["im_B"], upsample=upsample)

    def forward(self, batch, batched=True, upsample=False, scale_factor=1):
        pyr = batch.get("pyramid") or self.extract_backbone_features(batch, batched=batched, upsample=upsample)
        if batched:
            f_q = {s: f.chunk(2)[0] for s, f in pyr.items()}
            f_s = {s: f.chunk(2)[1] for s, f in pyr.items()}
        else:
            f_q, f_s = pyr
        return self.decoder(f_q, f_s, upsample=upsample, scale_factor=scale_factor, wait_events=batch.get("wait_events"),
                            **(batch.get("corresps") or {}))

    def forward_symmetric(self, batch, batched=True, upsample=False, scale_factor=1):
        pyr = batch.get("pyramid") or self.extract_backbone_features(batch, batched=batched, upsample=upsample)
        kw = {k: v for k, v in (batch.get("corresps") or {}).items() if k in ("flow", "certainty")}
        return self.decoder(pyr, None, upsample=upsample, scale_factor=scale_factor, swapped_pair=True,
                            wait_events=batch.get("wait_events"), **kw)

    def sample(self, matches, certainty, num=10000, seed=None):
        if seed is None:
            seed = int(torch.randint(0, 2 ** 31 - 1, (1,)).item())
        thresh = self.sample_thresh if "threshold" in self.sample_mode else -1.0
        matches, certainty = matches.reshape(-1, 4), certainty.reshape(-1)
        expansion = 4 if "balanced" in self.sample_mode else 1
        good = torch.topk(ops.race_keys(certainty, thresh, seed), min(expansion * num, len(certainty))).indices
        good_matches, good_certainty = matches[good], certainty[good]
        if thresh >= 0:
            good_certainty = torch.where(good_certainty > thresh, torch.ones_like(good_certainty), good_certainty)
        if "balanced" not in self.sample_mode:
            return good_matches, good_certainty
        density = ops.kde(good_matches, std=0.1)
        p = 1 / (density + 1)
        p[density < 10] = 1e-7
        bal = torch.topk(ops.race_keys(p, -1.0, seed, counter=good, stage=1), min(num, len(good_certainty))).indices
        return good_matches[bal], good_certainty[bal]

    def sample_batch(self, matches, certainty, num=10000, seeds=None):
        return ops.sample_batch(matches, certainty, num, seeds, self.sample_mode, self.sample_thresh)

    def to_pixel_coordinates(self, coords, H_A, W_A, H_B=None, W_B=None):
        if coords.shape[-1] == 2:
            return self._to_pixel_coordinates(coords, H_A, W_A)
        if isinstance(coords, (list, tuple)):
            kA, kB = coords[0], coords[1]
        else:
            kA, kB = coords[..., :2], coords[..., 2:]
        return self._to_pixel_coordinates(kA, H_A, W_A), self._to_pixel_coordinates(kB, H_B, W_B)

    def _to_pixel_coordinates(self, coords, H, W):
        return torch.stack((W / 2 * (coords[..., 0] + 1), H / 2 * (coords[..., 1] + 1)), axis=-1)

    def to_normalized_coordinates(self, coords, H_A, W_A, H_B, W_B):
        if isinstance(coords, (list, tuple)):
            kA, kB = coords[0], coords[1]
        else:
            kA, kB = coords[..., :2], coords[..., 2:]
        kA = torch.stack((2 / W_A * kA[..., 0] - 1, 2 / H_A * kA[..., 1] - 1), axis=-1)
        kB = torch.stack((2 / W_B * kB[..., 0] - 1, 2 / H_B * kB[..., 1] - 1), axis=-1)
        return kA, kB

    def match_keypoints(self, x_A, x_B, warp, certainty, return_tuple=True, return_inds=False):
        x_A_to_B = F.grid_sample(warp[..., -2:].permute(2, 0, 1)[None], x_A[None, None], align_corners=False, mode="bilinear")[0, :, 0].mT
        cert = F.grid_sample(certainty[None, None, ...], x_A[None, None], align_corners=False, mode="bilinear")[0, 0, 0]
        nn_b = ops.nn_argmin(x_A_to_B, x_B)
        nn_a = ops.nn_argmin(x_B, x_A_to_B)
        iA = torch.nonzero((nn_a[nn_b] == torch.arange(len(nn_b), device=nn_b.device)) & (cert > self.sample_thresh), as_tuple=True)[0]
        iB = nn_b[iA]
        if return_tuple:
            return (iA, iB) if return_inds else (x_A[iA], x_B[iB])
        return torch.cat((iA, iB), dim=-1) if return_inds else torch.cat((x_A[iA], x_B[iB]), dim=-1)

    def conf_from_fb_consistency(self, flow_forward, flow_backward, th=2):
        has_batch = flow_forward.dim() != 3
        if not has_batch:
            flow_forward, flow_backward = flow_forward[None], flow_backward[None]
        H, W = flow_forward.shape[-3:-1]
        th_n = 2 * th / max(H, W)
        dev = flow_forward.device
        coords = torch.stack(torch.meshgrid(torch.linspace(-1 + 1 / W, 1 - 1 / W, W, device=dev),
                                            torch.linspace(-1 + 1 / H, 1 - 1 / H, H, device=dev), indexing="xy"), dim=-1)
        coords_fb = ops.warp_bilinear(flow_backward.permute(0, 3, 1, 2), flow_forward.permute(0, 3, 1, 2)).permute(0, 2, 3, 1)
        in_th = ((coords - coords_fb).norm(dim=-1) < th_n).float()
        return in_th if has_batch else in_th[0]

    @torch.inference_mode()
    def match_tensors(self, A_lo, B_lo, A_hi=None, B_hi=None):
        with ops.deferred_spd_checks():
            return self._match_tensors(A_lo, B_lo, A_hi, B_hi)

    def _match_tensors(self, A_lo, B_lo, A_hi=None, B_hi=None):
        symmetric = self.symmetric
        batch = {"im_A": A_lo, "im_B": B_lo}
        hi_pyr = None
        overlap = getattr(self, "overlap_upsample_encoder", True) and hasattr(self.encoder, "vit_features")
        if overlap:
            x_lo = torch.cat((A_lo, B_lo), dim=0)
            pyr = {16: self.encoder.vit_features(x_lo)}
            main = torch.cuda.current_stream()
            side = self._side_stream = getattr(self, "_side_stream", None) or torch.cuda.Stream()
            side.wait_stream(main)
            with torch.cuda.stream(side):
                pyr.update(self.encoder.cnn(x_lo, self.encoder.amp_dtype))
                lo_ready = torch.cuda.Event()
                lo_ready.record(side)
                if self.upsample_preds and A_hi is not None and B_hi is not None:
                    hi_pyr = self.extract_backbone_features({"im_A": A_hi, "im_B": B_hi}, batched=True, upsample=True)
            batch["pyramid"] = pyr
            batch["wait_events"] = {8: lo_ready}
        else:
            batch["pyramid"] = self.extract_backbone_features(batch, batched=True)
        corresps = self.forward_symmetric(batch) if symmetric else self.forward(batch, batched=True)
        hs, ws = A_lo.shape[-2:]
        cert16 = corresps[16]["certainty"] if self.attenuate_cert else None
        if self.upsample_preds:
            if A_hi is None or B_hi is None:
                raise ValueError("upsample_preds=True needs the high-resolution images (A_hi, B_hi)")
            hs, ws = A_hi.shape[-2:]
            scale_factor = math.sqrt(hs * ws / (A_lo.shape[-2] * A_lo.shape[-1]))
            batch = {"im_A": A_hi, "im_B": B_hi, "corresps": corresps[1]}
            if hi_pyr is not None:
                torch.cuda.current_stream().wait_stream(self._side_stream)
                batch["pyramid"] = hi_pyr
            corresps = (self.forward_symmetric(batch, upsample=True, scale_factor=scale_factor) if symmetric
                        else self.forward(batch, batched=True, upsample=True, scale_factor=scale_factor))
        return ops.match_finalize(corresps[1]["flow"], corresps[1]["certainty"], cert16, symmetric=symmetric)

    def make_graphed(self, A_lo, B_lo, A_hi=None, B_hi=None, warmup=2):
        ins = [None if t is None else t.clone() for t in (A_lo, B_lo, A_hi, B_hi)]
        with torch.inference_mode():
            for _ in range(warmup):
                self.match_tensors(*ins)
            torch.cuda.synchronize()
            graph = torch.cuda.CUDAGraph()
            with torch.cuda.graph(graph):
                out = self.match_tensors(*ins)

        def run(*new):
            for dst, src in zip(ins, new):
                if dst is not None and src is not None and src.data_ptr() != dst.data_ptr():
                    dst.copy_(src)
            graph.replay()
            return out

        run.graph, run.static_inputs, run.static_outputs = graph, ins, out
        return run

    @torch.inference_mode()
    def encode(self, im_lo, im_hi=None):
        lo = self.encoder(im_lo, upsample=False)
        hi = self.encoder(im_hi, upsample=True) if (self.upsample_preds and im_hi is not None) else None
        return {"lo": lo, "hi": hi, "lo_size": tuple(im_lo.shape[-2:]), "hi_size": None if im_hi is None else tuple(im_hi.shape[-2:])}

    @torch.inference_mode()
    def match_encoded(self, enc_A, enc_B):
        if not self.symmetric:
            raise NotImplementedError("match_encoded implements the symmetric mode the shipped models use")
        with ops.deferred_spd_checks():
            return self._match_encoded(enc_A, enc_B)

    def _match_encoded(self, enc_A, enc_B):
        pyr = {s: torch.cat((enc_A["lo"][s], enc_B["lo"][s]), dim=0) for s in enc_A["lo"]}
        corresps = self.forward_symmetric({"pyramid": pyr})
        cert16 = corresps[16]["certainty"] if self.attenuate_cert else None
        if self.upsample_preds:
            if enc_A["hi"] is None or enc_B["hi"] is None:
                raise ValueError("upsample_preds=True needs encode(im_lo, im_hi)")
            (h, w), (hs, ws) = enc_A["lo_size"], enc_A["hi_size"]
            pyr = {s: torch.cat((enc_A["hi"][s], enc_B["hi"][s]), dim=0) for s in enc_A["hi"]}
            corresps = self.forward_symmetric({"pyramid": pyr, "corresps": corresps[1]}, upsample=True,
                                              scale_factor=math.sqrt(hs * ws / (h * w)))
        return ops.match_finalize(corresps[1]["flow"], corresps[1]["certainty"], cert16, symmetric=True)

    @torch.inference_mode()
    def match(self, im_A_input, im_B_input, *args, batched=False, device=None, im_A_hi=None, im_B_hi=None):
        from PIL import Image
        if device is None:
            device = torch.device("cuda" if torch.cuda.is_available() else "cpu")
        device = torch.device(device)
        if device.type != "cuda":
            raise RuntimeError("roma_amd runs on an MI355X only; there is no CPU path (use the oracle for CPU numbers)")
        self.train(False)
        if batched:
            b, c, h, w = im_A_input.shape
            b2, c2, h2, w2 = im_B_input.shape
            assert w == w2 and h == h2, "For batched images we assume same size"
            if h != self.h_resized or self.w_resized != w:
                warn("Model resolution and batch resolution differ, may produce unexpected results")
            hi = (None, None) if im_A_hi is None else (im_A_hi.to(device), im_B_hi.to(device))
            return self.match_tensors(im_A_input.to(device), im_B_input.to(device), *hi)
        ims = []
        for im in (im_A_input, im_B_input):
            if isinstance(im, (str, os.PathLike)):
                if not getattr(self, "host_preprocess", False) and getattr(self, "device_jpeg", True):
                    from .preproc import decode_jpeg_device
                    dec = decode_jpeg_device(im, device) if str(im).lower().endswith((".jpg", ".jpeg")) else None
                    if dec is not None:
                        ims.append(dec)
                        continue
                im = Image.open(im)
                _check_not_i16(im)
                im = im.convert("RGB")
            else:
                _check_rgb(im)
            ims.append(im)
        if getattr(self, "host_preprocess", False):
            lo = [preprocess(im, (self.h_resized, self.w_resized))[None].to(device) for im in ims]
            hi = [preprocess(im, self.upsample_res)[None].to(device) for im in ims] if self.upsample_preds else [None, None]
        else:
            from .preproc import preprocess_device
            src = [im if isinstance(im, torch.Tensor) else torch.from_numpy(np.array(im, dtype=np.uint8)).to(device) for im in ims]
            lo = [preprocess_device(s, (self.h_resized, self.w_resized), device)[None] for s in src]
            hi = [preprocess_device(s, self.upsample_res, device)[None] for s in src] if self.upsample_preds else [None, None]
        warp, cert = self.match_tensors(lo[0], lo[1], hi[0], hi[1])
        return warp[0], cert[0]

    def visualize_warp(self, warp, certainty, im_A=None, im_B=None, im_A_path=None, im_B_path=None, device="cuda",
                       symmetric=True, save_path=None, unnormalize=False):
        from PIL import Image
        H, W2, _ = warp.shape
        W = W2 // 2 if symmetric else W2
        if im_A is None:
            im_A, im_B = Image.open(im_A_path).convert("RGB"), Image.open(im_B_path).convert("RGB")
        if not isinstance(im_A, torch.Tensor):
            im_A, im_B = im_A.resize((W, H)), im_B.resize((W, H))
            x_B = (torch.tensor(np.array(im_B)) / 255).to(device).permute(2, 0, 1)
            x_A = (torch.tensor(np.array(im_A)) / 255).to(device).permute(2, 0, 1)
        else:
            x_A, x_B = im_A, im_B
        a2b = F.grid_sample(x_B[None], warp[:, :W, 2:][None], mode="bilinear", align_corners=False)[0]
        if symmetric:
            b2a = F.grid_sample(x_A[None], warp[:, W:, :2][None], mode="bilinear", align_corners=False)[0]
            warp_im = torch.cat((a2b, b2a), dim=2)
        else:
            warp_im = a2b
        white = torch.ones((H, W2 if symmetric else W), device=device)
        vis = certainty * warp_im + (1 - certainty) * white
        if save_path is not None:
            arr = (vis.permute(1, 2, 0).clamp(0, 1).cpu().numpy() * 255).astype(np.uint8)
            Image.fromarray(arr).save(save_path)
        return vis
```

roma_amd/ops.py:

```python
from __future__ import annotations

import math
from typing import Optional

import torch

from . import _lib
from ._lib import ROMA_BF16, ROMA_F16, ROMA_F32, ROMA_NCHW, ROMA_NHWC, check

_DT = {torch.float32: ROMA_F32, torch.float16: ROMA_F16, torch.bfloat16: ROMA_BF16}


class KernelTimer:

    def __init__(self):
        self.enabled = False
        self.bracket_overhead_s = 0.0
        self.records = []

    def start(self):
        self.records.clear()
        torch.cuda.synchronize()
        pairs = []
        for _ in range(32):
            s, e = torch.cuda.Event(enable_timing=True), torch.cuda.Event(enable_timing=True)
            s.record()
            e.record()
            pairs.append((s, e))
        torch.cuda.synchronize()
        gaps = sorted(s.elapsed_time(e) * 1e-3 for s, e in pairs)
        self.bracket_overhead_s = gaps[len(gaps) // 2]
        self.enabled = True

    def stop(self):
        self.enabled = False

    def wrap(self, name, nbytes, tag, launch):
        if not self.enabled or torch.cuda.is_current_stream_capturing():
            return launch()
        s, e = torch.cuda.Event(enable_timing=True), torch.cuda.Event(enable_timing=True)
        s.record()
        out = launch()
        e.record()
        self.records.append((name, nbytes, s, e, tag))
        return out

    def summary(self):
        out = {}
        for name, nbytes, s, e, tag in self.records:
            d = out.setdefault(name, {"launches": 0, "bytes": 0, "seconds": 0.0, "by_tag": {}})
            t = max(s.elapsed_time(e) * 1e-3 - self.bracket_overhead_s, 1e-7)
            d["launches"] += 1
            d["bytes"] += nbytes
            d["seconds"] += t
            bt = d["by_tag"].setdefault(tag, [0, 0, 0.0])
            bt[0] += 1
            bt[1] += nbytes
            bt[2] += t
        return out


TIMER = KernelTimer()


def _need_gpu(*ts):
    dev = None
    for t in ts:
        if t is None:
            continue
        if not t.is_cuda:
            raise RuntimeError("roma_amd kernels run on an MI355X (ROCm device tensors) only; got a "
                               f"{t.device} tensor and there is no CPU fallback")
        if dev is None:
            dev = t.device
        elif t.device != dev:
            raise RuntimeError(f"roma_amd kernel arguments live on different devices ({dev} and {t.device})")
    if dev is not None and dev.index != torch.cuda.current_device():
        raise RuntimeError(f"roma_amd kernel arguments live on {dev} but the current device is cuda:{torch.cuda.current_device()}; "
                           "wrap the call in `with torch.cuda.device(t.device):`")


def _stream():
    return torch.cuda.current_stream().cuda_stream


def _dt(t):
    try:
        return _DT[t.dtype]
    except KeyError:
        raise ValueError(f"unsupported dtype {t.dtype}") from None


def _p(t):
    return None if t is None else t.data_ptr()


def feat_layout(t: torch.Tensor):
    B, C, H, W = t.shape
    sb, sc, sh, sw = t.stride()
    if sc == 1 and sh == W * sw and sb == H * W * sw and sw >= C:
        return ROMA_NHWC, sw, t
    if t.is_contiguous():
        return ROMA_NCHW, C, t
    t = t.contiguous()
    return ROMA_NCHW, C, t


def nhwc_empty(B, C, H, W, dtype, device, pitch=None):
    pitch = pitch or C
    buf = torch.empty((B, H, W, pitch), dtype=dtype, device=device)
    return buf[..., :C].permute(0, 3, 1, 2)


def local_correlation(feature0, feature1, local_radius, padding_mode="zeros", flow=None, sample_mode="bilinear", out=None,
                      batch_shift=0, variant="auto"):
    if padding_mode != "zeros" or sample_mode != "bilinear":
        raise NotImplementedError("only padding_mode='zeros', sample_mode='bilinear' (the modes RoMa uses)")
    _need_gpu(feature0, feature1, flow, out)
    if feature0.shape != feature1.shape or feature0.dtype != feature1.dtype:
        raise ValueError("feature0/feature1 must have the same shape and dtype")
    B, C, H, W = feature0.shape
    r = int(local_radius)
    K = (2 * r + 1) ** 2
    l0, p0, f0 = feat_layout(feature0)
    l1, p1, f1 = feat_layout(feature1)
    if l0 != l1:
        f1 = f1.contiguous(memory_format=torch.channels_last if l0 == ROMA_NHWC else torch.contiguous_format)
        l1, p1, f1 = feat_layout(f1)
    if flow is not None:
        if tuple(flow.shape) != (B, 2, H, W):
            raise ValueError(f"flow must be (B,2,h,w), got {tuple(flow.shape)}")
        flow = flow.float().contiguous()
    if out is None:
        out = nhwc_empty(B, K, H, W, feature0.dtype, feature0.device) if l0 == ROMA_NHWC else \
            torch.empty((B, K, H, W), dtype=feature0.dtype, device=feature0.device)
    lo, po, o = feat_layout(out)
    if o is not out or tuple(out.shape) != (B, K, H, W) or out.dtype != feature0.dtype:
        raise ValueError("out must be a (B,K,h,w) tensor of the input dtype, contiguous or channels-last")
    es = f0.element_size()
    nbytes = 2 * B * C * H * W * es + B * 2 * H * W * 4 + B * K * H * W * es
    TIMER.wrap("local_corr", nbytes, f"C{C}_h{H}x{W}_r{r}",
               lambda: check(_lib.load().roma_local_corr(_p(f0), _p(f1), _p(flow), _p(out), B, C, H, W, r, _dt(f0), l0, p0, p1,
                                                         lo, po, int(batch_shift) % B, _lib.LC_VARIANTS[variant], _stream()), "roma_local_corr"))
    return out


def warp_bilinear(src, flow, out=None, batch_shift=0):
    _need_gpu(src, flow, out)
    B, C, Hs, Ws = src.shape
    _, _, H, W = flow.shape
    ls, ps, s = feat_layout(src)
    flow = flow.float().contiguous()
    if out is None:
        out = nhwc_empty(B, C, H, W, src.dtype, src.device) if ls == ROMA_NHWC else torch.empty((B, C, H, W), dtype=src.dtype, device=src.device)
    lo, po, o = feat_layout(out)
    if o is not out:
        raise ValueError("out must be contiguous or channels-last")
    check(_lib.load().roma_warp_bilinear(_p(s), _p(flow), _p(out), B, C, Hs, Ws, H, W, _dt(s), ls, ps, lo, po, int(batch_shift) % B, _stream()),
          "roma_warp_bilinear")
    return out


def disp_emb(flow, weight, bias, gain, out=None, dtype=torch.float32):
    _need_gpu(flow, weight, bias, out)
    B, _, H, W = flow.shape
    E = weight.shape[0]
    flow = flow.float().contiguous()
    w = weight.reshape(E, 2).float().contiguous()
    bvec = bias.float().contiguous()
    if out is None:
        out = torch.empty((B, E, H, W), dtype=dtype, device=flow.device)
    lo, po, o = feat_layout(out)
    if o is not out:
        raise ValueError("out must be contiguous or channels-last")
    check(_lib.load().roma_disp_emb(_p(flow), _p(w), _p(bvec), _p(out), B, E, H, W, float(gain), _dt(out), lo, po, _stream()),
          "roma_disp_emb")
    return out


def interp_bilinear(x, size):
    _need_gpu(x)
    B, C, Hi, Wi = x.shape
    Ho, Wo = int(size[0]), int(size[1])
    x = x.float().contiguous()
    y = torch.empty((B, C, Ho, Wo), dtype=torch.float32, device=x.device)
    check(_lib.load().roma_interp_bilinear(_p(x), _p(y), B * C, Hi, Wi, Ho, Wo, _stream()), "roma_interp_bilinear")
    return y


def interp_bilinear_pair(a, b, size):
    _need_gpu(a, b)
    B, Ca, Hi, Wi = a.shape
    Bb, Cb = b.shape[:2]
    if tuple(b.shape[2:]) != (Hi, Wi):
        raise ValueError(f"the two maps differ in size: {tuple(a.shape)} and {tuple(b.shape)}")
    Ho, Wo = int(size[0]), int(size[1])
    a = a.float().contiguous()
    b = b.float().contiguous()
    ya = torch.empty((B, Ca, Ho, Wo), dtype=torch.float32, device=a.device)
    yb = torch.empty((Bb, Cb, Ho, Wo), dtype=torch.float32, device=a.device)
    check(_lib.load().roma_interp_bilinear_pair(_p(a), _p(ya), B * Ca, _p(b), _p(yb), Bb * Cb, Hi, Wi, Ho, Wo, _stream()),
          "roma_interp_bilinear_pair")
    return ya, yb


def refiner_assemble(buf, src, flow, weight, bias, gain, C, D, batch_shift=0):
    _need_gpu(buf, src, flow, weight, bias)
    B, H, W, Dp = buf.shape
    E = weight.shape[0]
    ls, ps, s = feat_layout(src)
    if ls != ROMA_NHWC or s is not src or src.dtype != buf.dtype or not buf.is_contiguous():
        raise ValueError("refiner_assemble: buf must be contiguous (B,h,w,Dp), src channels-last and of buf's dtype")
    if tuple(flow.shape) != (B, 2, H, W) or src.shape[0] != B or src.shape[1] != C:
        raise ValueError(f"refiner_assemble: flow {tuple(flow.shape)} / src {tuple(src.shape)} do not match buf {tuple(buf.shape)}, C = {C}")
    flow = flow.float().contiguous()
    w = weight.reshape(E, 2).float().contiguous()
    bvec = bias.float().contiguous()
    check(_lib.load().roma_refiner_assemble(_p(src), _p(flow), _p(w), _p(bvec), _p(buf), B, C, E, D, Dp, src.shape[2], src.shape[3], H, W,
                                            ps, int(batch_shift) % B, float(gain), _dt(buf), _stream()), "roma_refiner_assemble")
    return buf


def flow_update(flow, certainty, delta, sx, sy):
    _need_gpu(flow, certainty, delta)
    B, _, H, W = flow.shape
    assert flow.dtype == torch.float32 and flow.is_contiguous() and delta.dtype == torch.float32 and delta.is_contiguous()
    cert_in = None if certainty is None else certainty.float().contiguous()
    cert = torch.empty((B, 1, H, W), dtype=torch.float32, device=flow.device)
    check(_lib.load().roma_flow_update(_p(flow), _p(cert), _p(cert_in), _p(delta), B, H, W, float(sx), float(sy), _stream()),
          "roma_flow_update")
    return flow, cert


def cls_to_flow_refine(cls):
    _need_gpu(cls)
    B, C, H, W = cls.shape
    sb, sc, sh, sw = cls.stride()
    if sh != W * sw:
        cls = cls.contiguous()
        sb, sc, sh, sw = cls.stride()
    flow = torch.empty((B, 2, H, W), dtype=torch.float32, device=cls.device)
    check(_lib.load().roma_cls_to_flow_refine(_p(cls), _p(flow), None, B, C, H * W, sb, sc, sw, _dt(cls), _stream()),
          "roma_cls_to_flow_refine")
    return flow.permute(0, 2, 3, 1)


def cls_rows_to_flow(rows, B, H, W):
    _need_gpu(rows)
    assert rows.dim() == 3 and rows.shape[0] == B and rows.shape[1] == H * W and rows.stride(2) == 1
    C = rows.shape[2] - 1
    flow = torch.empty((B, 2, H, W), dtype=torch.float32, device=rows.device)
    cert = torch.empty((B, 1, H, W), dtype=torch.float32, device=rows.device)
    check(_lib.load().roma_cls_to_flow_refine(_p(rows), _p(flow), _p(cert), B, C, H * W, rows.stride(0), 1, rows.stride(1),
                                              _dt(rows), _stream()), "roma_cls_to_flow_refine")
    return flow, cert


def _rows(t):
    B, N, D = t.shape
    es = t.element_size()
    if t.stride(2) == 1 and t.stride(0) == N * t.stride(1) and t.stride(1) >= D and (t.stride(1) * es) % 16 == 0 \
            and t.data_ptr() % 16 == 0 and t.dtype in _DT:
        return t, t.stride(1)
    t = (t if t.dtype in _DT else t.float()).contiguous()
    return t, D


def cos_kernel(x, y, T=0.2, eps=1e-6, diag_add=0.0, batch_shift=0):
    _need_gpu(x, y)
    if x.dtype != y.dtype:
        x, y = x.float(), y.float()
    x, xp = _rows(x)
    y, yp = _rows(y)
    B, N, D = x.shape
    M = y.shape[1]
    K = torch.empty((B, N, M), dtype=torch.float32, device=x.device)
    check(_lib.load().roma_cos_kernel(_p(x), _p(y), _p(K), B, N, M, D, _dt(x), xp, yp, int(batch_shift) % B, float(T), float(eps),
                                      float(diag_add), _stream()), "roma_cos_kernel")
    return K


class _PendingSpdCheck:

    def __init__(self, info):
        self.host = torch.empty(info.shape, dtype=info.dtype, pin_memory=True)
        self.host.copy_(info, non_blocking=True)
        self.event = torch.cuda.Event()
        self.event.record()

    def result(self):
        self.event.synchronize()
        return self.host.tolist()


_PENDING = []


def _raise_if_not_spd(bad):
    if any(bad):
        b = next(i for i, v in enumerate(bad) if v)
        raise _lib.RomaHipError(f"spd_solve: matrix {b} of the batch is not positive definite (block step {(bad[b] - 1) // 64}, pivot "
                                f"{(bad[b] - 1) % 64} is <= 0 or NaN) — non-finite or degenerate features?  The reference's "
                                f"torch.linalg.inv raises here too (matcher.py:261).")


_DEFER_DEPTH = [0]


def deferring():
    return _DEFER_DEPTH[0] > 0


class deferred_spd_checks:

    def __enter__(self):
        _DEFER_DEPTH[0] += 1
        return self

    def __exit__(self, et, ev, tb):
        _DEFER_DEPTH[0] -= 1
        if _DEFER_DEPTH[0] > 0:
            return False
        todo, _PENDING[:] = list(_PENDING), []
        if et is None and not torch.cuda.is_current_stream_capturing():
            for chk in todo:
                _raise_if_not_spd(chk.result())
        return False


def raise_pending():
    if torch.cuda.is_current_stream_capturing():
        return
    todo, _PENDING[:] = list(_PENDING), []
    for chk in todo:
        _raise_if_not_spd(chk.result())


def spd_solve(K, F, check="now", refine=0):
    _need_gpu(K, F)
    assert K.dtype == torch.float32 and F.dtype == torch.float32
    tun = torch.cuda.tunable.is_enabled()
    if tun:
        torch.cuda.tunable.enable(False)
    try:
        X, info = _spd_solve(K, F, refine)
    finally:
        if tun:
            torch.cuda.tunable.enable(True)
    if check == "now":
        _raise_if_not_spd(info.tolist())
    elif check == "defer":
        _PENDING.append(_PendingSpdCheck(info))
    return X


def _spd_solve(K, F, refine=0):
    nb = 64
    B, n, _ = K.shape
    m = F.shape[2]
    lib = _lib.load()
    A = torch.cat((K, F.expand(B, -1, -1)), dim=2)
    steps = [(j, min(j + nb, n)) for j in range(0, n, nb)]
    W = torch.empty((B, len(steps), nb, nb), dtype=torch.float32, device=K.device)
    info = torch.zeros((B,), dtype=torch.int32, device=K.device)
    Rall = torch.empty((B, len(steps), nb, n + m), dtype=torch.float32, device=K.device)
    check(lib.roma_chol_diag_block(A.data_ptr(), A.stride(1), A.stride(0), W.data_ptr(), nb, W.stride(0), steps[0][1], B,
                                   info.data_ptr(), 0, _stream()), "roma_chol_diag_block")
    for s, (j, e) in enumerate(steps):
        last = s + 1 == len(steps)
        check(lib.roma_chol_step(A.data_ptr(), A.stride(1), A.stride(0), n, n + m, j, e - j, W[:, s].data_ptr(), nb, W.stride(0),
                                 Rall[:, s].data_ptr(), n + m, Rall.stride(0), None if last else W[:, s + 1].data_ptr(), nb, W.stride(0),
                                 info.data_ptr(), nb * (s + 1), B, _stream()), "roma_chol_step")
    X = torch.empty((B, n, m), dtype=torch.float32, device=K.device)
    S = len(steps)

    def subst(direction, T, sTb, sTs, ldt, in_panel, out):
        for s in (range(S - 1, -1, -1) if direction < 0 else range(S)):
            check(lib.roma_chol_subst_step(direction, W[:, s].data_ptr(), nb, W.stride(0), Rall.data_ptr(), Rall.stride(0), Rall.stride(1),
                                           n + m, T.data_ptr(), sTb, sTs, ldt, in_panel, out.data_ptr(), m, out.stride(0), n, m, nb, s, B,
                                           _stream()), "roma_chol_subst_step")

    subst(-1, Rall, Rall.stride(0), Rall.stride(1), n + m, 1, X)
    for _ in range(int(refine)):
        g = (F.double() - torch.bmm(K.double(), X.double())).float().contiguous()
        y = torch.empty_like(g)
        subst(+1, g, g.stride(0), nb * m, m, 0, y)
        d = torch.empty_like(g)
        subst(-1, y, y.stride(0), nb * m, m, 0, d)
        X = X + d
    return X, info


def match_finalize(flow, certainty, cert16, symmetric=True):
    _need_gpu(flow, certainty, cert16)
    B, _, H, W = flow.shape
    P = B // 2 if symmetric else B
    flow = flow.float().contiguous()
    certainty = certainty.float().contiguous()
    H16 = W16 = 0
    if cert16 is not None:
        cert16 = cert16.float().contiguous()
        H16, W16 = cert16.shape[-2:]
    WW = 2 * W if symmetric else W
    warp = torch.empty((P, H, WW, 4), dtype=torch.float32, device=flow.device)
    cert = torch.empty((P, H, WW), dtype=torch.float32, device=flow.device)
    check(_lib.load().roma_match_finalize(_p(flow), _p(certainty), _p(cert16), _p(warp), _p(cert), P, H, W, H16, W16,
                                          1 if symmetric else 0, _stream()), "roma_match_finalize")
    return warp, cert


def kde(x, std=0.1, half=True, down=None):
    _need_gpu(x)
    if x.dim() != 2 or x.shape[1] != 4:
        raise ValueError("kde expects (N,4) matches")
    xs = (x.half() if half else x).float().contiguous()
    N = xs.shape[0]
    dens = torch.empty((N,), dtype=torch.float32, device=x.device)
    check(_lib.load().roma_kde_density(_p(xs), _p(dens), N, int(down or 1), float(std), 1 if half else 0, _stream()), "roma_kde_density")
    return dens.half() if half else dens


def race_keys(p, thresh=-1.0, seed=0, counter=None, stage=0):
    _need_gpu(p, counter)
    p = p.reshape(-1).float().contiguous()
    if counter is not None:
        counter = counter.reshape(-1).long().contiguous()
        assert counter.numel() == p.numel()
    keys = torch.empty_like(p)
    check(_lib.load().roma_race_keys(_p(p), _p(counter), _p(keys), p.numel(), float(thresh), int(seed) & 0xFFFFFFFF,
                                     int(stage) & 0xFFFFFFFF, _stream()), "roma_race_keys")
    return keys


def seed_tensor(seeds, P, device):
    if seeds is None:
        seeds = torch.randint(0, 2 ** 31 - 1, (P,))
    if not torch.is_tensor(seeds):
        seeds = torch.tensor([int(s) & 0xFFFFFFFF for s in seeds], dtype=torch.int64)
    seeds = seeds.reshape(-1).to(torch.int64)
    if seeds.numel() != P:
        raise ValueError(f"{P} pairs need {P} seeds, got {seeds.numel()}")
    if not seeds.is_cuda:
        seeds = seeds.pin_memory().to(device, non_blocking=True)
    return seeds.contiguous()


def race_select(p, k, thresh=-1.0, seeds=None, counter=None, stage=0):
    _need_gpu(p, counter)
    if p.dim() != 2:
        raise ValueError("race_select expects (P,N) weights")
    if seeds is None:
        raise ValueError("race_select needs P seeds")
    p = p.float().contiguous()
    P, N = p.shape
    k = int(k)
    seeds = seed_tensor(seeds, P, p.device)
    _need_gpu(seeds)
    if counter is not None:
        counter = counter.long().contiguous()
        if counter.shape != p.shape:
            raise ValueError("race_select: counter must have the shape of p")
    lib = _lib.load()
    nbytes = lib.roma_race_select_workspace(P, N, k)
    if nbytes < 0:
        check(int(nbytes), "roma_race_select_workspace")
    ws = torch.empty((nbytes // 8 + 1,), dtype=torch.int64, device=p.device)
    sel_key = torch.empty((P, k), dtype=torch.int64, device=p.device)
    sel_idx = torch.empty((P, k), dtype=torch.int64, device=p.device)
    check(lib.roma_race_select(_p(p), _p(counter), _p(seeds), P, N, k, float(thresh), int(stage) & 0xFFFFFFFF, _p(sel_key), _p(sel_idx),
                               _p(ws), ws.numel() * 8, _stream()), "roma_race_select")
    order = torch.sort(sel_key, dim=1, descending=True).indices
    return sel_idx.gather(1, order)


def kde_batch(x, std=0.1, half=True, down=None, index=None):
    _need_gpu(x, index)
    if x.dim() != 3 or x.shape[2] != 4:
        raise ValueError("kde_batch expects (P,n,4) matches")
    x = x.float().contiguous()
    P, N = x.shape[:2]
    n = N
    if index is not None:
        if index.dim() != 2 or index.shape[0] != P:
            raise ValueError("kde_batch: index must be (P,n)")
        index = index.long().contiguous()
        n = index.shape[1]
    dens = torch.empty((P, n), dtype=torch.float32, device=x.device)
    check(_lib.load().roma_kde_density_batch(_p(x), _p(index), _p(dens), P, N, n, int(down or 1), float(std), 1 if half else 0, _stream()),
          "roma_kde_density_batch")
    return dens.half() if half else dens


def sample_batch(matches, certainty, num, seeds=None, sample_mode="threshold_balanced", sample_thresh=0.05):
    _need_gpu(matches, certainty)
    P = matches.shape[0]
    matches = matches.reshape(P, -1, 4).float().contiguous()
    certainty = certainty.reshape(P, -1).float().contiguous()
    N = certainty.shape[1]
    if matches.shape[1] != N:
        raise ValueError("sample_batch: matches and certainty disagree on the number of items per pair")
    seeds = seed_tensor(seeds, P, matches.device)
    thresh = sample_thresh if "threshold" in sample_mode else -1.0
    balanced = "balanced" in sample_mode
    k1 = min((4 if balanced else 1) * num, N)
    good = race_select(certainty, k1, thresh, seeds)
    good_certainty = certainty.gather(1, good)
    if thresh >= 0:
        good_certainty = torch.where(good_certainty > thresh, torch.ones_like(good_certainty), good_certainty)
    if not balanced:
        return matches.gather(1, good[..., None].expand(-1, -1, 4)), good_certainty
    density = kde_batch(matches, std=0.1, half=True, down=1, index=good)
    p = 1 / (density + 1)
    p = torch.where(density < 10, torch.full_like(p, 1e-7), p)
    bal = race_select(p, min(num, k1), -1.0, seeds, counter=good, stage=1)
    sel = good.gather(1, bal)
    return matches.gather(1, sel[..., None].expand(-1, -1, 4)), good_certainty.gather(1, bal)


def nn_argmin(q, r):
    _need_gpu(q, r)
    if q.dim() != 2 or q.shape[1] != 2 or r.dim() != 2 or r.shape[1] != 2:
        raise ValueError("nn_argmin expects (N,2) point sets")
    q, r = q.float().contiguous(), r.float().contiguous()
    idx = torch.empty((q.shape[0],), dtype=torch.int32, device=q.device)
    check(_lib.load().roma_nn_argmin(_p(q), _p(r), _p(idx), q.shape[0], r.shape[0], _stream()), "roma_nn_argmin")
    return idx.long()


def dwconv5x5_bn_relu(x, w25, scale, shift, out=None):
    _need_gpu(x, w25, scale, shift, out)
    B, C, H, W = x.shape
    lx, px, xx = feat_layout(x)
    if lx != ROMA_NHWC:
        raise ValueError("dwconv5x5_bn_relu needs channels-last input")
    if out is None:
        out = nhwc_empty(B, C, H, W, x.dtype, x.device, pitch=px)
    lo, po, o = feat_layout(out)
    if lo != ROMA_NHWC or o is not out:
        raise ValueError("dwconv5x5_bn_relu needs channels-last output")
    check(_lib.load().roma_dwconv5x5_bn_relu(_p(xx), _p(w25), _p(scale), _p(shift), _p(out), B, C, H, W, _dt(xx), px, po, _stream()),
          "roma_dwconv5x5_bn_relu")
    return out


def resample_u8(img, out_size, axis, bounds, coef, ksize):
    _need_gpu(img, bounds, coef)
    H, W, C = img.shape
    assert img.dtype == torch.uint8 and img.is_contiguous() and bounds.dtype == torch.int32 and coef.dtype == torch.int32
    assert bounds.shape == (out_size, 2) and coef.shape == (out_size, ksize) and bounds.is_contiguous() and coef.is_contiguous()
    out = torch.empty((H, out_size, C) if axis else (out_size, W, C), dtype=torch.uint8, device=img.device)
    check(_lib.load().roma_resample_u8(_p(img), _p(out), H, W, C, out_size, axis, _p(bounds), _p(coef), ksize, _stream()), "roma_resample_u8")
    return out


def normalize_u8(img, mean, std):
    import ctypes
    _need_gpu(img)
    H, W, C = img.shape
    assert C == 3 and img.dtype == torch.uint8 and img.is_contiguous()
    out = torch.empty((3, H, W), dtype=torch.float32, device=img.device)
    m = (ctypes.c_float * 3)(*mean)
    s = (ctypes.c_float * 3)(*std)
    check(_lib.load().roma_normalize_u8(_p(img), _p(out), H, W, ctypes.cast(m, ctypes.c_void_p), ctypes.cast(s, ctypes.c_void_p), _stream()),
          "roma_normalize_u8")
    return out


def _is_nhwc(x):
    return x.dim() == 4 and x.shape[1] > 1 and x.stride(1) == 1 and x.is_contiguous(memory_format=torch.channels_last)


def bias_relu_(x, bias):
    _need_gpu(x, bias)
    B, C, H, W = x.shape
    assert bias.dtype == x.dtype and bias.numel() == C and bias.is_contiguous()
    if _is_nhwc(x):
        check(_lib.load().roma_bias_relu_nhwc(_p(x), _p(bias), B * H * W, C, _dt(x), _stream()), "roma_bias_relu_nhwc")
        return x
    assert x.is_contiguous()
    step = max(1, 65535 // C)
    for b0 in range(0, B, step):
        xb = x[b0:b0 + step]
        check(_lib.load().roma_bias_relu_nchw(_p(xb), _p(bias), xb.shape[0], C, H * W, _dt(x), _stream()), "roma_bias_relu_nchw")
    return x


def bias_relu_pool2_(x, bias):
    _need_gpu(x, bias)
    B, C, H, W = x.shape
    assert bias.dtype == x.dtype and bias.numel() == C and bias.is_contiguous() and H % 2 == 0 and W % 2 == 0
    if _is_nhwc(x):
        out = torch.empty((B, H // 2, W // 2, C), dtype=x.dtype, device=x.device).permute(0, 3, 1, 2)
        check(_lib.load().roma_bias_relu_pool2_nhwc(_p(x), _p(bias), _p(out), B, C, H, W, _dt(x), _stream()), "roma_bias_relu_pool2_nhwc")
        return out
    assert x.is_contiguous()
    out = torch.empty((B, C, H // 2, W // 2), dtype=x.dtype, device=x.device)
    step = max(1, 65535 // C)
    for b0 in range(0, B, step):
        xb = x[b0:b0 + step]
        check(_lib.load().roma_bias_relu_pool2_nchw(_p(xb), _p(bias), _p(out[b0:b0 + step]), xb.shape[0], C, H, W, _dt(x), _stream()),
              "roma_bias_relu_pool2_nchw")
    return out


def pointwise_mfma(rows, wt, bias, C, out=None):
    _need_gpu(rows, wt, bias, out)
    M, pitch = rows.shape
    kpad = wt.shape[0]
    assert rows.is_contiguous() and wt.is_contiguous() and wt.dtype == rows.dtype and bias.numel() == kpad and bias.dtype == torch.float32
    if out is None:
        out = torch.empty_like(rows)
    assert out.shape == rows.shape and out.is_contiguous()
    check(_lib.load().roma_pointwise_mfma(_p(rows), _p(wt), _p(bias), _p(out), M, C, kpad, _dt(rows), pitch, pitch, _stream()),
          "roma_pointwise_mfma")
    return out


def project_skinny_pack(wt_in_out, bias):
    K, N = wt_in_out.shape
    Np = (N + 15) // 16 * 16
    wt = torch.zeros((Np, K), dtype=wt_in_out.dtype, device=wt_in_out.device)
    wt[:N] = wt_in_out.t()
    b = torch.zeros(Np, dtype=torch.float32, device=wt_in_out.device)
    b[:N] = bias.float()
    return wt, b


def project_skinny(rows, wt, bias, N, out):
    _need_gpu(rows, wt, bias, out)
    M, K = rows.shape
    if rows.stride(1) != 1 or out.stride(1) != 1 or out.shape[0] != M or out.shape[1] < N or out.dtype != rows.dtype or wt.dtype != rows.dtype:
        raise ValueError("project_skinny: rows (M,K) and out (M,>=N) must be unit-stride rows of one 16-bit dtype")
    if not wt.is_contiguous() or wt.shape[1] != K or wt.shape[0] < N or bias.dtype != torch.float32 or bias.numel() != wt.shape[0]:
        raise ValueError("project_skinny: wt / bias are not what project_skinny_pack returns for these rows")
    check(_lib.load().roma_project_skinny(_p(rows), _p(wt), _p(bias), _p(out), M, K, N, _dt(rows), rows.stride(0), out.stride(0), _stream()),
          "roma_project_skinny")
    return out


def refiner_wide_pack(wt_out_in):
    w = wt_out_in.detach().to("cpu").contiguous()
    assert w.dim() == 2 and w.shape[0] == w.shape[1] and w.element_size() == 2
    out = torch.empty_like(w)
    check(_lib.load().roma_refiner_wide_pack(w.data_ptr(), out.data_ptr(), w.shape[0]), "roma_refiner_wide_pack")
    return out.to(wt_out_in.device)


def refiner_wide_taps(w25, dtype=torch.float16):
    D = w25.shape[1]
    w = w25.detach().to("cpu").to(dtype).contiguous()
    assert w.shape == (25, D) and w.element_size() == 2
    out = torch.empty((D // 32, 5, 4, 2, 6, 4, 2), dtype=dtype)
    check(_lib.load().roma_refiner_wide_taps(w.data_ptr(), out.data_ptr(), D), "roma_refiner_wide_taps")
    return out.to(w25.device)


def refiner_block_wide(x_nhwc, w25p, scale, shift, wp, bias, out=None):
    _need_gpu(x_nhwc, w25p, scale, shift, wp, bias, out)
    B, H, W, D = x_nhwc.shape
    assert x_nhwc.is_contiguous() and w25p.shape == (D // 32, 5, 4, 2, 6, 4, 2) and w25p.dtype == x_nhwc.dtype and w25p.is_contiguous()
    assert all(t.dtype == torch.float32 and t.numel() == D and t.is_contiguous() for t in (scale, shift, bias))
    if out is None:
        out = torch.empty_like(x_nhwc)
    assert out.shape == x_nhwc.shape and out.is_contiguous() and out.data_ptr() != x_nhwc.data_ptr()
    check(_lib.load().roma_refiner_block_wide(_p(x_nhwc), _p(w25p), _p(scale), _p(shift), _p(wp), _p(bias), _p(out), B, H, W, D, D, D,
                                              _dt(x_nhwc), _stream()), "roma_refiner_block_wide")
    return out


def refiner_block(x_nhwc, w25, scale, shift, wt, bias, C, out=None):
    _need_gpu(x_nhwc, w25, scale, shift, wt, bias, out)
    B, h, w, pitch = x_nhwc.shape
    kpad = wt.shape[0]
    assert x_nhwc.is_contiguous() and wt.is_contiguous() and w25.is_contiguous() and wt.dtype == x_nhwc.dtype == w25.dtype
    assert w25.shape == (25, kpad) and wt.shape == (kpad, kpad) and scale.numel() == shift.numel() == bias.numel() == kpad
    if out is None:
        out = torch.empty_like(x_nhwc)
    assert out.is_contiguous() and out.shape == x_nhwc.shape and out.data_ptr() != x_nhwc.data_ptr()
    check(_lib.load().roma_refiner_block(_p(x_nhwc), _p(w25), _p(scale), _p(shift), _p(wt), _p(bias), _p(out), B, C, h, w, kpad,
                                         _dt(x_nhwc), pitch, pitch, _stream()), "roma_refiner_block")
    return out


def refiner_block_mid(x_nhwc, w25, scale, shift, wt, bias, C, out=None):
    _need_gpu(x_nhwc, w25, scale, shift, wt, bias, out)
    B, h, w, pitch = x_nhwc.shape
    assert x_nhwc.is_contiguous() and wt.is_contiguous() and w25.is_contiguous() and wt.dtype == x_nhwc.dtype
    assert w25.shape == (25, C) and wt.shape == (160, 160) and scale.numel() == shift.numel() == C and bias.numel() == 160
    assert all(t.dtype == torch.float32 and t.is_contiguous() for t in (w25, scale, shift, bias))
    if out is None:
        out = torch.empty_like(x_nhwc)
    assert out.is_contiguous() and out.shape == x_nhwc.shape and out.dtype == x_nhwc.dtype
    check(_lib.load().roma_refiner_block_mid(_p(x_nhwc), _p(w25), _p(scale), _p(shift), _p(wt), _p(bias), _p(out), B, C, h, w,
                                             _dt(x_nhwc), pitch, pitch, _stream()), "roma_refiner_block_mid")
    return out


def refiner_head(x_nhwc, wo, bo, flow, certainty, sx, sy, want_delta=False):
    _need_gpu(x_nhwc, wo, bo, flow, certainty)
    B, h, w, pitch = x_nhwc.shape
    C = wo.shape[0]
    assert x_nhwc.is_contiguous() and flow.is_contiguous() and flow.dtype == torch.float32 and wo.is_contiguous()
    cert_in = None if certainty is None else certainty.float().contiguous()
    cert = torch.empty((B, 1, h, w), dtype=torch.float32, device=flow.device)
    delta = torch.empty((B, 3, h, w), dtype=torch.float32, device=flow.device) if want_delta else None
    check(_lib.load().roma_refiner_head(_p(x_nhwc), _p(wo), _p(bo), _p(flow), _p(cert_in), _p(cert), _p(delta), B, h, w, C, pitch,
                                        _dt(x_nhwc), float(sx), float(sy), _stream()), "roma_refiner_head")
    return (flow, cert, delta) if want_delta else (flow, cert)


def pointwise_small(x_rows, wt, bias, out=None):
    _need_gpu(x_rows, wt, bias, out)
    M, C = x_rows.shape
    assert x_rows.stride(1) == 1
    if out is None:
        out = torch.empty((M, C), dtype=x_rows.dtype, device=x_rows.device)
    check(_lib.load().roma_pointwise_small(_p(x_rows), _p(wt), _p(bias), _p(out), M, C, _dt(x_rows), x_rows.stride(0), out.stride(0),
                                           _stream()), "roma_pointwise_small")
    return out


def attention(qkv, n_valid=None, out=None):
    _need_gpu(qkv, out)
    B, N, three, H, d = qkv.shape
    assert three == 3 and qkv.is_contiguous()
    if out is None:
        out = torch.empty((B, N, H * d), dtype=qkv.dtype, device=qkv.device)
    assert out.is_contiguous() and out.shape == (B, N, H * d) and out.dtype == qkv.dtype
    es = qkv.element_size()
    sb, sn, sh = qkv.stride(0), qkv.stride(1), qkv.stride(3)
    base = qkv.data_ptr()
    step = qkv.stride(2) * es
    check(_lib.load().roma_attention_fwd(base, base + step, base + 2 * step, out.data_ptr(), B, H, N, N if n_valid is None else int(n_valid), d,
                                         sb, sn, sh, sb, sn, sh, sb, sn, sh, out.stride(0), out.stride(1), d, float(d) ** -0.5, _dt(qkv),
                                         _stream()), "roma_attention_fwd")
    return out


def add_layernorm(x, y, ln_weight, ln_bias, eps, out_dtype, ls=None):
    _need_gpu(x, y, ln_weight, ln_bias, ls)
    C = x.shape[-1]
    assert x.is_contiguous() and (y is None or (y.is_contiguous() and y.shape == x.shape))
    rows = x.numel() // C
    out = torch.empty(x.shape, dtype=out_dtype, device=x.device)
    for t in (ln_weight, ln_bias, ls):
        assert t is None or (t.dtype == torch.float32 and t.is_contiguous() and t.numel() == C)
    check(_lib.load().roma_add_layernorm(_p(x), _dt(x), C, _p(y), _dt(y) if y is not None else 0, C, _p(ls), _p(ln_weight), _p(ln_bias),
                                         _p(out), _DT[out_dtype], C, rows, C, float(eps), _stream()), "roma_add_layernorm")
    return out


def tiny_corr_posembed(f0, f1, exact=False):
    _need_gpu(f0, f1)
    B, C, H0, W0 = f0.shape
    _, _, H1, W1 = f1.shape
    a = f0.float().permute(0, 2, 3, 1).contiguous()
    b = f1.float().permute(0, 2, 3, 1).contiguous()
    out = torch.empty((B, 2, H0, W0), dtype=torch.float32, device=f0.device)
    TIMER.wrap("tiny_corr", 2.0 * B * H0 * W0 * H1 * W1 * C, f"C{C}_{H0}x{W0}",
               lambda: check(_lib.load().roma_tiny_corr_posembed(_p(a), _p(b), _p(out), B, C, H0, W0, H1, W1, 1 if exact else 0, _stream()),
                             "roma_tiny_corr_posembed"))
    return out
```

Measured before the change: 60.56 image-pairs/s.

## Fuse refiner head projection into the last refiner block kernel

Adds head-fused variants of the Toeplitz, mid and wide refiner block kernels. The last block now projects its output straight to the 3-channel flow/certainty update while it is still in LDS, then writes flow and certainty, instead of storing the full feature map and launching a separate head kernel. This removes one global write and read of the last block's activations and one launch per refiner scale. In exchange it uses more LDS and registers in the block kernels, which could lower occupancy, and it adds a dispatch path (tail_impl) with more variants to keep correct.

```diff
diff --git a/include/roma_hip.h b/include/roma_hip.h
--- a/include/roma_hip.h
+++ b/include/roma_hip.h
@@ -112,6 +112,16 @@
 
 int roma_refiner_head(const void* x, const float* wo, const float* bo, float* flow, const float* cert_in, float* cert_out,
                       float* delta_out, int B, int H, int W, int C, int pitch, int dtype, float sx, float sy, void* stream);
+
+int roma_refiner_block_head(const void* x, const void* w25, const float* scale, const float* shift, const void* wt,
+                            const float* bias, int B, int C, int H, int W, int kpad, int dtype, int x_pitch, const float* wo,
+                            const float* bo, float* flow, const float* cert_in, float* cert_out, float sx, float sy, void* stream);
+int roma_refiner_block_mid_head(const void* x, const float* w25, const float* scale, const float* shift, const void* wt,
+                                const float* bias, int B, int C, int H, int W, int dtype, int x_pitch, const float* wo,
+                                const float* bo, float* flow, const float* cert_in, float* cert_out, float sx, float sy, void* stream);
+int roma_refiner_block_wide_head(const void* x, const void* w25p, const float* scale, const float* shift, const void* wp,
+                                 const float* bias, int B, int H, int W, int D, int x_pitch, int dtype, const float* wo,
+                                 const float* bo, float* flow, const float* cert_in, float* cert_out, float sx, float sy, void* stream);
 
 int roma_pointwise_small(const void* x, const float* wt, const float* bias, void* y, long M, int C, int dtype,
                          int x_pitch, int y_pitch, void* stream);
diff --git a/roma_amd/_lib.py b/roma_amd/_lib.py
--- a/roma_amd/_lib.py
+++ b/roma_amd/_lib.py
@@ -68,6 +68,9 @@
                                 c_int, c_void_p],
     "roma_refiner_head": [c_void_p, c_void_p, c_void_p, c_void_p, c_void_p, c_void_p, c_void_p, c_int, c_int, c_int, c_int, c_int, c_int,
                           c_float, c_float, c_void_p],
+    "roma_refiner_block_head": [c_void_p] * 6 + [c_int] * 7 + [c_void_p] * 5 + [c_float, c_float, c_void_p],
+    "roma_refiner_block_mid_head": [c_void_p] * 6 + [c_int] * 6 + [c_void_p] * 5 + [c_float, c_float, c_void_p],
+    "roma_refiner_block_wide_head": [c_void_p] * 6 + [c_int] * 6 + [c_void_p] * 5 + [c_float, c_float, c_void_p],
     "roma_pointwise_small": [c_void_p, c_void_p, c_void_p, c_void_p, c_long, c_int, c_int, c_int, c_int, c_void_p],
     "roma_tiny_corr_posembed": [c_void_p, c_void_p, c_void_p, c_int, c_int, c_int, c_int, c_int, c_int, c_int, c_void_p],
     "roma_ransac_workspace": [c_int, c_int, c_int, c_int, c_void_p],
diff --git a/roma_amd/csrc/refiner_block.hip b/roma_amd/csrc/refiner_block.hip
--- a/roma_amd/csrc/refiner_block.hip
+++ b/roma_amd/csrc/refiner_block.hip
@@ -1,6 +1,7 @@
 #include <algorithm>
 #include "common.h"
 #include "lc_device.h"
+#include "refiner_head_device.h"
 #include "refiner_mid_device.h"
 
 namespace roma {
@@ -27,6 +28,12 @@
   int B, H, W, C, x_pitch, y_pitch;
   int tiles_x, tiles_y;
   float inv_tiles_per_img, inv_tiles_x;
+  const float* wo;
+  const float* bo;
+  float* flow;
+  const float* cert_in;
+  float* cert_out;
+  float sx, sy;
 };
 
 constexpr int XT = 16, YT = 8, HX = XT + 4, HY = YT + 4, NPOS = HX * HY;
@@ -204,9 +211,10 @@
 constexpr int TP_TOEP = TP_NCH * 5 * TP_FRAG;
 constexpr int TP_PL = TP_NCH * TP_PLB, TP_TB = TPX * TPY * TP_OS * 2, TP_PW = 32 * 5 * 16;
 constexpr int TP_SMEM = TP_TOEP + TP_PL + TP_TB + TP_PW + 3 * 32 * 4;
-static_assert(TPY * TP_TROW <= TP_TB && 2 * TP_SMEM <= 160 * 1024, "LDS budget of the Toeplitz block: two workgroups per CU");
-
-template <typename T>
+constexpr int TP_SMEM_HEAD = TP_SMEM + (TP_NCH * 3 + 8) * 4;
+static_assert(TPY * TP_TROW <= TP_TB && 2 * TP_SMEM_HEAD <= 160 * 1024, "LDS budget of the Toeplitz block: two workgroups per CU");
+
+template <typename T, bool HEAD>
 __global__ __launch_bounds__(256, 2) void refiner_block_toep_kernel(RBParams p) {
   extern __shared__ __attribute__((aligned(16))) unsigned char smem[];
   unsigned char* s_toep = smem;
@@ -214,11 +222,12 @@
   unsigned char* s_t = s_pl + TP_PL;
   u32x4* s_pw = reinterpret_cast<u32x4*>(s_t + TP_TB);
   float* s_cs = reinterpret_cast<float*>(s_pw + 32 * 5);
+  float* s_wo = s_cs + 3 * 32;
   const int tid = threadIdx.x, lane = tid & 63;
   const int wv = __builtin_amdgcn_readfirstlane(tid >> 6);
   const int m = lane & 15, q = lane >> 4;
   const T* x = static_cast<const T*>(p.x);
-  T* y = static_cast<T*>(p.y);
+  [[maybe_unused]] T* y = static_cast<T*>(p.y);
   const int tiles_per_img = p.tiles_x * p.tiles_y;
   auto tile_origin = [&](int tile, int& b, int& ty0, int& tx0) {
     b = (int)(((float)tile + 0.5f) * p.inv_tiles_per_img);
@@ -242,6 +251,10 @@
     }
     for (int i = tid; i < 32 * 4; i += 256) s_pw[(i >> 2) * 5 + (i & 3)] = reinterpret_cast<const u32x4*>(p.wt)[i];
     if (tid < 32) { s_cs[tid] = p.scale[tid]; s_cs[32 + tid] = p.shift[tid]; s_cs[64 + tid] = p.bias[tid]; }
+    if constexpr (HEAD) {
+      if (tid < TP_NCH * 3) s_wo[tid] = p.wo[tid];
+      if (tid < 3) s_wo[TP_NCH * 3 + tid] = p.bo[tid];
+    }
     for (int i = tid; i < (TP_PL + TP_TB) / 16; i += 256) reinterpret_cast<u32x4*>(s_pl)[i] = u32x4{0, 0, 0, 0};
   }
   const int ntile = tiles_per_img * p.B;
@@ -302,6 +315,11 @@
   for (int nb = 0; nb < 2; ++nb)
 #pragma unroll
     for (int i = 0; i < 4; ++i) bsv4[nb][i] = s_cs[64 + nb * 16 + 4 * q + i];
+  [[maybe_unused]] float hw[24];
+  if constexpr (HEAD) {
+#pragma unroll
+    for (int i = 0; i < 24; ++i) hw[i] = s_wo[min(lane & 3, TP_NCH / 8 - 1) * 24 + i];
+  }
   for (int tile = t_beg; tile < t_end; tile += nx) {
     int b, ty0, tx0;
     tile_origin(tile, b, ty0, tx0);
@@ -362,16 +380,50 @@
         for (int i = 0; i < 4; ++i) o4[i] = from_f32<T>(acc2[r][nb][i] + bsv4[nb][i]);
         *reinterpret_cast<uint2*>(s_out + ((wv * 4 + r) * TPX + m) * TP_OS + nb * 16 + 4 * q) = *reinterpret_cast<const uint2*>(o4);
       }
+    [[maybe_unused]] const int sub = lane & 3, HW = p.H * p.W;
+    [[maybe_unused]] int hidx[4];
+    [[maybe_unused]] float hf0[4], hf1[4], hc[4];
+    if constexpr (HEAD) {
+#pragma unroll
+      for (int it = 0; it < 4; ++it) {
+        const int yy = ty0 + wv * 4 + it, xx = tx0 + (lane >> 2);
+        hidx[it] = sub == 0 && yy < p.H && xx < p.W ? yy * p.W + xx : -1;
+        hf0[it] = hf1[it] = hc[it] = 0.f;
+        if (hidx[it] >= 0) {
+          const float* fl = p.flow + (size_t)b * 2 * HW + hidx[it];
+          hf0[it] = fl[0];
+          hf1[it] = fl[HW];
+          if (p.cert_in) hc[it] = p.cert_in[(size_t)b * HW + hidx[it]];
+        }
+      }
+    }
     if (more) scatter();
     if (more2) fetch(tile + 2 * nx);
     __syncthreads();
-    T* yb = y + (size_t)b * p.H * p.W * p.y_pitch;
-#pragma unroll
-    for (int j = 0; j < 3; ++j) {
-      const int i = tid + 256 * j, pix = i / 3, k = i - pix * 3;
-      const int yy = ty0 + (pix >> 4), xx = tx0 + (pix & 15);
-      if (yy < p.H && xx < p.W)
-        *reinterpret_cast<u32x4*>(yb + ((size_t)yy * p.W + xx) * p.y_pitch + k * 8) = *reinterpret_cast<const u32x4*>(s_out + pix * TP_OS + k * 8);
+    if constexpr (HEAD) {
+#pragma unroll
+      for (int it = 0; it < 4; ++it) {
+        const T* row = s_out + ((wv * 4 + it) * TPX + (lane >> 2)) * TP_OS;
+        float a0 = 0.f, a1 = 0.f, a2 = 0.f;
+        if (sub < TP_NCH / 8) head::fma_packet<T>(*reinterpret_cast<const u32x4*>(row + sub * 8), hw, a0, a1, a2);
+        head::reduce<4>(a0, a1, a2);
+        if (hidx[it] >= 0) {
+          float* fl = p.flow + (size_t)b * 2 * HW + hidx[it];
+          head::finish(a0, a1, a2, s_wo + TP_NCH * 3, p.sx, p.sy, hf0[it], hf1[it], hc[it]);
+          fl[0] = hf0[it];
+          fl[HW] = hf1[it];
+          p.cert_out[(size_t)b * HW + hidx[it]] = hc[it];
+        }
+      }
+    } else {
+      T* yb = y + (size_t)b * p.H * p.W * p.y_pitch;
+#pragma unroll
+      for (int j = 0; j < 3; ++j) {
+        const int i = tid + 256 * j, pix = i / 3, k = i - pix * 3;
+        const int yy = ty0 + (pix >> 4), xx = tx0 + (pix & 15);
+        if (yy < p.H && xx < p.W)
+          *reinterpret_cast<u32x4*>(yb + ((size_t)yy * p.W + xx) * p.y_pitch + k * 8) = *reinterpret_cast<const u32x4*>(s_out + pix * TP_OS + k * 8);
+      }
     }
     __syncthreads();
     for (int i = tid; i < TPX * TPY; i += 256) {
@@ -381,10 +433,11 @@
   }
 }
 
-template <typename T>
+template <typename T, bool HEAD = false>
 int launch_rb_toep(RBParams p, hipStream_t s) {
+  constexpr int smem = HEAD ? TP_SMEM_HEAD : TP_SMEM;
   static std::atomic<uint64_t> attr_done{0};
-  if (int rc = ensure_dyn_smem(reinterpret_cast<const void*>(refiner_block_toep_kernel<T>), TP_SMEM, attr_done, "roma_refiner_block")) return rc;
+  if (int rc = ensure_dyn_smem(reinterpret_cast<const void*>(refiner_block_toep_kernel<T, HEAD>), smem, attr_done, "roma_refiner_block")) return rc;
   p.tiles_x = (p.W + TPX - 1) / TPX;
   p.tiles_y = (p.H + TPY - 1) / TPY;
   const long ntile = (long)p.B * p.tiles_x * p.tiles_y;
@@ -392,7 +445,7 @@
   p.inv_tiles_per_img = 1.0f / (float)(p.tiles_x * p.tiles_y);
   p.inv_tiles_x = 1.0f / (float)p.tiles_x;
   const int grid = ntile < 2 * num_cus() ? (int)ntile : 2 * num_cus();
-  hipLaunchKernelGGL((refiner_block_toep_kernel<T>), dim3(grid), dim3(256), TP_SMEM, s, p);
+  hipLaunchKernelGGL((refiner_block_toep_kernel<T, HEAD>), dim3(grid), dim3(256), smem, s, p);
   ROMA_CHECK_LAUNCH();
 }
 
@@ -479,9 +532,27 @@
   ROMA_REQUIRE((kpad == 32 || kpad == 160) && C <= kpad && C % 8 == 0, ROMA_E_UNSUPPORTED, "roma_refiner_block: C=%d, kpad=%d (kpad must be 32 or 160, C a multiple of 8)", C, kpad);
   ROMA_REQUIRE(x_pitch % 8 == 0 && y_pitch % 8 == 0 && aligned16(x) && aligned16(y) && aligned16(w25) && aligned16(wt), ROMA_E_ALIGN,
                "roma_refiner_block: pitches must be multiples of 8 and bases 16-byte aligned");
-  RBParams p{x, y, w25, wt, scale, shift, bias, B, H, W, C, x_pitch, y_pitch, (W + XT - 1) / XT, (H + YT - 1) / YT, 0.f, 0.f};
+  RBParams p{x, y, w25, wt, scale, shift, bias, B, H, W, C, x_pitch, y_pitch, (W + XT - 1) / XT, (H + YT - 1) / YT, 0.f, 0.f,
+             nullptr, nullptr, nullptr, nullptr, nullptr, 0.f, 0.f};
   hipStream_t s = static_cast<hipStream_t>(stream);
   return dtype == ROMA_F16 ? launch_rb_any<half_t>(p, kpad, s) : launch_rb_any<bf16_t>(p, kpad, s);
+}
+
+extern "C" int roma_refiner_block_head(const void* x, const void* w25, const float* scale, const float* shift, const void* wt,
+                                       const float* bias, int B, int C, int H, int W, int kpad, int dtype, int x_pitch, const float* wo,
+                                       const float* bo, float* flow, const float* cert_in, float* cert_out, float sx, float sy,
+                                       void* stream) {
+  ROMA_REQUIRE(x && w25 && scale && shift && wt && bias && wo && bo && flow && cert_out, ROMA_E_ARG, "roma_refiner_block_head: null pointer");
+  ROMA_REQUIRE(B > 0 && C > 0 && H > 0 && W > 0 && x_pitch >= C, ROMA_E_SHAPE, "roma_refiner_block_head: bad shape");
+  ROMA_REQUIRE(dtype == ROMA_F16 || dtype == ROMA_BF16, ROMA_E_DTYPE, "roma_refiner_block_head: fp16 / bf16 only");
+  ROMA_REQUIRE(kpad == 32 && C == TP_NCH, ROMA_E_UNSUPPORTED,
+               "roma_refiner_block_head: C=%d, kpad=%d (built for the block kernel of C = 24, kpad = 32)", C, kpad);
+  ROMA_REQUIRE(x_pitch % 8 == 0 && aligned16(x) && aligned16(w25) && aligned16(wt), ROMA_E_ALIGN,
+               "roma_refiner_block_head: pitches must be multiples of 8 and bases 16-byte aligned");
+  ROMA_REQUIRE((size_t)B * H * W * x_pitch * 2 < (1ull << 32), ROMA_E_SHAPE, "roma_refiner_block_head: a map of 4 GB or more in one launch");
+  RBParams p{x, nullptr, w25, wt, scale, shift, bias, B, H, W, C, x_pitch, x_pitch, 0, 0, 0.f, 0.f, wo, bo, flow, cert_in, cert_out, sx, sy};
+  hipStream_t s = static_cast<hipStream_t>(stream);
+  return dtype == ROMA_F16 ? launch_rb_toep<half_t, true>(p, s) : launch_rb_toep<bf16_t, true>(p, s);
 }
 
 extern "C" int roma_pointwise_mfma(const void* x, const void* wt, const float* bias, void* y, long M, int C, int kpad, int dtype,
diff --git a/roma_amd/csrc/refiner_head.hip b/roma_amd/csrc/refiner_head.hip
--- a/roma_amd/csrc/refiner_head.hip
+++ b/roma_amd/csrc/refiner_head.hip
@@ -1,4 +1,5 @@
 #include "common.h"
+#include "refiner_head_device.h"
 
 namespace roma {
 namespace {
@@ -14,31 +15,18 @@
   const int sub = threadIdx.x % L;
   for (size_t m = ((size_t)blockIdx.x * blockDim.x + threadIdx.x) / L; m < M; m += (size_t)gridDim.x * blockDim.x / L) {
     float a0 = 0.f, a1 = 0.f, a2 = 0.f;
-    for (int pk = sub; pk < PK; pk += L) {
-      float f[E];
-      unpack16<T>(*reinterpret_cast<const u32x4*>(x + m * pitch + pk * E), f);
-      const float* w = wo + (size_t)pk * E * 3;
-#pragma unroll
-      for (int e = 0; e < E; ++e) {
-        a0 = __builtin_fmaf(f[e], w[e * 3 + 0], a0);
-        a1 = __builtin_fmaf(f[e], w[e * 3 + 1], a1);
-        a2 = __builtin_fmaf(f[e], w[e * 3 + 2], a2);
-      }
-    }
-#pragma unroll
-    for (int o = L / 2; o > 0; o >>= 1) {
-      a0 += __shfl_xor(a0, o, 64);
-      a1 += __shfl_xor(a1, o, 64);
-      a2 += __shfl_xor(a2, o, 64);
-    }
+    for (int pk = sub; pk < PK; pk += L)
+      head::fma_packet<T>(*reinterpret_cast<const u32x4*>(x + m * pitch + pk * E), wo + (size_t)pk * E * 3, a0, a1, a2);
+    head::reduce<L>(a0, a1, a2);
     if (sub == 0) {
-      a0 += bo[0]; a1 += bo[1]; a2 += bo[2];
       const int b = (int)(m / HW);
       const size_t p = m - (size_t)b * HW;
       float* fl = flow + (size_t)b * 2 * HW + p;
-      fl[0] += sx * a0;
-      fl[HW] += sy * a1;
-      cert_out[m] = (cert_in ? cert_in[m] : 0.f) + a2;
+      float f0 = fl[0], f1 = fl[HW], c = cert_in ? cert_in[m] : 0.f;
+      head::finish(a0, a1, a2, bo, sx, sy, f0, f1, c);
+      fl[0] = f0;
+      fl[HW] = f1;
+      cert_out[m] = c;
       if (delta_out) {
         delta_out[(size_t)b * 3 * HW + p] = a0;
         delta_out[(size_t)b * 3 * HW + HW + p] = a1;
@@ -62,7 +50,7 @@
   ROMA_REQUIRE(C % e == 0 && pitch % e == 0 && aligned16(x), ROMA_E_ALIGN, "roma_refiner_head: C and pitch must be multiples of %d, x 16-byte aligned", e);
   hipStream_t s = static_cast<hipStream_t>(stream);
   const int pk = C / e;
-  const int L = pk >= 64 ? 64 : (pk >= 16 ? 16 : 4);
+  const int L = head::lanes_for(pk);
   const size_t threads = (size_t)B * H * W * L;
   size_t g = (threads + 255) / 256;
   if (g > 32768) g = 32768;
diff --git a/roma_amd/csrc/refiner_head_device.h b/roma_amd/csrc/refiner_head_device.h
--- /dev/null
+++ b/roma_amd/csrc/refiner_head_device.h
@@ -0,0 +1,54 @@
+#pragma once
+#include "common.h"
+
+namespace roma {
+namespace head {
+
+inline int lanes_for(int pk) { return pk >= 64 ? 64 : (pk >= 16 ? 16 : 4); }
+
+template <typename T>
+__device__ __forceinline__ void fma_packet(const u32x4& v, const float* w, float& a0, float& a1, float& a2) {
+  constexpr int E = ElemTraits<T>::kPer16B;
+  float f[E];
+  unpack16<T>(v, f);
+#pragma unroll
+  for (int e = 0; e < E; ++e) {
+    a0 = __builtin_fmaf(f[e], w[e * 3 + 0], a0);
+    a1 = __builtin_fmaf(f[e], w[e * 3 + 1], a1);
+    a2 = __builtin_fmaf(f[e], w[e * 3 + 2], a2);
+  }
+}
+
+template <int O>
+__device__ __forceinline__ float lane_xor(float v) {
+  if constexpr (O < 32)
+    return __builtin_bit_cast(float, __builtin_amdgcn_ds_swizzle(__builtin_bit_cast(int, v), (O << 10) | 0x1f));
+  else
+    return __shfl_xor(v, O, 64);
+}
+template <int O>
+__device__ __forceinline__ void reduce_step(float& a0, float& a1, float& a2) {
+  a0 += lane_xor<O>(a0);
+  a1 += lane_xor<O>(a1);
+  a2 += lane_xor<O>(a2);
+}
+
+template <int L>
+__device__ __forceinline__ void reduce(float& a0, float& a1, float& a2) {
+  static_assert(L == 4 || L == 16 || L == 64, "lanes_for");
+  if constexpr (L == 64) { reduce_step<32>(a0, a1, a2); reduce_step<16>(a0, a1, a2); }
+  if constexpr (L >= 16) { reduce_step<8>(a0, a1, a2); reduce_step<4>(a0, a1, a2); }
+  reduce_step<2>(a0, a1, a2);
+  reduce_step<1>(a0, a1, a2);
+}
+
+__device__ __forceinline__ void finish(float& a0, float& a1, float& a2, const float* bo, float sx, float sy, float& f0, float& f1,
+                                       float& c) {
+  a0 += bo[0]; a1 += bo[1]; a2 += bo[2];
+  f0 += sx * a0;
+  f1 += sy * a1;
+  c = c + a2;
+}
+
+}
+}
diff --git a/roma_amd/csrc/refiner_mid.hip b/roma_amd/csrc/refiner_mid.hip
--- a/roma_amd/csrc/refiner_mid.hip
+++ b/roma_amd/csrc/refiner_mid.hip
@@ -1,4 +1,5 @@
 #include "common.h"
+#include "refiner_head_device.h"
 #include "refiner_mid_device.h"
 
 namespace roma {
@@ -9,7 +10,8 @@
 constexpr int MID_RS = MID_KPAD / 8 + 1;
 constexpr int MID_SMAX = 28, MID_ROWS = MID_SMAX * mid::kStrip;
 constexpr int MID_SMEM = (MID_ROWS * MID_RS + MID_KPAD * MID_RS) * 16 + 25 * MID_KPAD * 4 + MID_KPAD * 4 + MID_ROWS * 4 + 16 * (MID_KPAD / 8) * 4;
-static_assert(MID_SMEM <= 160 * 1024, "LDS budget: t 75.3 KB + weights 53.8 KB + taps 16 KB + bias + the two index tables");
+constexpr int MID_SMEM_HEAD = MID_SMEM + (MID_KPAD * 3 + 4) * 4 + MID_ROWS * 4;
+static_assert(MID_SMEM_HEAD <= 160 * 1024, "LDS budget: t 75.3 KB + weights 53.8 KB + taps 16 KB + bias + the two index tables + wo");
 static_assert(MID_ROWS % 16 == 0 && MID_ROWS / 16 <= 16, "a wave takes row groups wv and wv + 8");
 
 struct MidParams {
@@ -23,10 +25,17 @@
   int B, H, W, C, x_pitch, y_pitch;
   int S;
   unsigned nstrip, ntile, band;
+  const float* wo;
+  const float* bo;
+  float* flow;
+  const float* cert_in;
+  float* cert_out;
+  float sx, sy;
 };
 
-template <typename T>
+template <typename T, int L>
 __global__ __launch_bounds__(MID_NT) void refiner_mid_kernel(MidParams p) {
+  constexpr bool HEAD = L > 0;
   constexpr int RS = MID_RS, OS = MID_KPAD + 8;
   static_assert(OS == RS * 8, "a staged output row is one row of t");
   extern __shared__ __attribute__((aligned(16))) unsigned char smem[];
@@ -36,6 +45,8 @@
   float* s_b = s_w + 25 * MID_KPAD;
   int* s_pix = reinterpret_cast<int*>(s_b + MID_KPAD);
   int* s_item = s_pix + MID_ROWS;
+  float* s_wo = reinterpret_cast<float*>(s_item + 16 * (MID_KPAD / 8));
+  int* s_fl = reinterpret_cast<int*>(s_wo + MID_KPAD * 3 + 4);
   const int tid = threadIdx.x;
   const int wv = __builtin_amdgcn_readfirstlane(tid >> 6);
   const int C = p.C, H = p.H, W = p.W, PK = C / 8, S = p.S;
@@ -48,10 +59,14 @@
   for (int i = tid; i < MID_KPAD; i += MID_NT) s_b[i] = p.bias[i];
   for (int i = tid; i < MID_ROWS; i += MID_NT) s_pix[i] = -1;
   for (int i = tid; i < 16 * (MID_KPAD / 8); i += MID_NT) s_item[i] = i < 16 * PK ? (i / PK) << 8 | (i % PK) : -1;
+  if constexpr (HEAD) {
+    for (int i = tid; i < C * 3; i += MID_NT) s_wo[i] = p.wo[i];
+    if (tid < 3) s_wo[MID_KPAD * 3 + tid] = p.bo[tid];
+  }
   __syncthreads();
 
   const T* x = static_cast<const T*>(p.x);
-  T* y = static_cast<T*>(p.y);
+  [[maybe_unused]] T* y = static_cast<T*>(p.y);
   const unsigned WS = (unsigned)(W + mid::kStrip - 1) / mid::kStrip;
   const int sl = tid / PK, k = tid - sl * PK;
   const int ngrp = (S * mid::kStrip + 15) / 16;
@@ -73,6 +88,10 @@
           const int pix0 = (b * H + ys) * W + xs;
 #pragma unroll
           for (int o = 0; o < mid::kStrip; ++o) s_pix[sl * mid::kStrip + o] = xs + o < W ? pix0 + o : -1;
+          if constexpr (HEAD) {
+#pragma unroll
+            for (int o = 0; o < mid::kStrip; ++o) s_fl[sl * mid::kStrip + o] = pix0 + o + b * H * W;
+          }
         }
       } else if (k == 0) {
 #pragma unroll
@@ -111,63 +130,148 @@
                 *reinterpret_cast<const u32x4*>(so + (item[j] >> 8) * OS + (item[j] & 255) * 8);
       }
     };
+    constexpr int LH = HEAD ? L : 4, NI = 16 / (64 / LH);
+    struct HeadPix { int idx[NI], fl[NI]; float f0[NI], f1[NI], c[NI]; };
+    const int sub = lane & (LH - 1), hrow = lane / LH;
+    const int HW = H * W;
+    auto head_load = [&](int g, HeadPix& h) {
+#pragma unroll
+      for (int it = 0; it < NI; ++it) {
+        const int r = g * 16 + it * (64 / LH) + hrow;
+        h.idx[it] = sub == 0 ? s_pix[r] : -1;
+        h.fl[it] = s_fl[r];
+        h.f0[it] = h.f1[it] = h.c[it] = 0.f;
+        if (h.idx[it] >= 0) {
+          const float* fl = p.flow + (size_t)h.fl[it];
+          h.f0[it] = fl[0];
+          h.f1[it] = fl[HW];
+          if (p.cert_in) h.c[it] = p.cert_in[h.idx[it]];
+        }
+      }
+    };
+    [[maybe_unused]] float hw[2][24];
+    auto head_weights = [&]() {
+#pragma unroll
+      for (int j = 0; j < 2; ++j)
+#pragma unroll
+        for (int i = 0; i < 6; ++i) {
+          const float4_t v = *reinterpret_cast<const float4_t*>(s_wo + min(sub + LH * j, PK - 1) * 24 + 4 * i);
+          hw[j][4 * i] = v[0]; hw[j][4 * i + 1] = v[1]; hw[j][4 * i + 2] = v[2]; hw[j][4 * i + 3] = v[3];
+        }
+    };
+    auto head_group = [&](int g, HeadPix& h) {
+#pragma unroll
+      for (int it = 0; it < NI; ++it) {
+        const u32x4* row = s_t + (g * 16 + it * (64 / LH) + hrow) * RS;
+        float a0 = 0.f, a1 = 0.f, a2 = 0.f;
+        if constexpr (LH == 16) {
+          head::fma_packet<T>(row[sub], hw[0], a0, a1, a2);
+          if (sub + LH < PK) head::fma_packet<T>(row[sub + LH], hw[1], a0, a1, a2);
+        } else {
+          for (int pk = sub; pk < PK; pk += LH) head::fma_packet<T>(row[pk], s_wo + pk * 24, a0, a1, a2);
+        }
+        head::reduce<LH>(a0, a1, a2);
+        if (h.idx[it] >= 0) {
+          float* fl = p.flow + (size_t)h.fl[it];
+          head::finish(a0, a1, a2, s_wo + MID_KPAD * 3, p.sx, p.sy, h.f0[it], h.f1[it], h.c[it]);
+          fl[0] = h.f0[it];
+          fl[HW] = h.f1[it];
+          p.cert_out[h.idx[it]] = h.c[it];
+        }
+      }
+    };
     if (wv + 8 < ngrp) {
       u32x4 a[2][MID_KP];
       fragments(wv, a[0]);
       fragments(wv + 8, a[1]);
+      HeadPix hp[2];
+      if constexpr (HEAD) { head_load(wv, hp[0]); head_load(wv + 8, hp[1]); }
       T* const stage[2] = {reinterpret_cast<T*>(s_t + wv * 16 * RS), reinterpret_cast<T*>(s_t + (wv + 8) * 16 * RS)};
       mid::pw_row_groups<T, MID_KP, 2>(a, s_pw, s_b, stage, m, kq);
-      store_groups({wv, wv + 8}, std::integral_constant<int, 2>{});
+      if constexpr (HEAD) {
+        if constexpr (LH == 16) head_weights();
+        head_group(wv, hp[0]);
+        head_group(wv + 8, hp[1]);
+      }
+      else store_groups({wv, wv + 8}, std::integral_constant<int, 2>{});
     } else if (wv < ngrp) {
       u32x4 a[1][MID_KP];
       fragments(wv, a[0]);
+      HeadPix hp;
+      if constexpr (HEAD) head_load(wv, hp);
       T* const stage[1] = {reinterpret_cast<T*>(s_t + wv * 16 * RS)};
       mid::pw_row_groups<T, MID_KP, 1>(a, s_pw, s_b, stage, m, kq);
-      store_groups({wv, wv}, std::integral_constant<int, 1>{});
+      if constexpr (HEAD) {
+        if constexpr (LH == 16) head_weights();
+        head_group(wv, hp);
+      }
+      else store_groups({wv, wv}, std::integral_constant<int, 1>{});
     }
     __syncthreads();
   }
 }
 
-template <typename T>
-int launch_mid(MidParams p, hipStream_t s) {
+template <typename T, int L>
+int launch_mid(MidParams p, hipStream_t s, const char* what) {
+  constexpr int smem = L > 0 ? MID_SMEM_HEAD : MID_SMEM;
   static std::atomic<uint64_t> attr_done{0};
-  if (int rc = ensure_dyn_smem(reinterpret_cast<const void*>(refiner_mid_kernel<T>), MID_SMEM, attr_done, "roma_refiner_block_mid")) return rc;
+  if (int rc = ensure_dyn_smem(reinterpret_cast<const void*>(refiner_mid_kernel<T, L>), smem, attr_done, what)) return rc;
   const int cus = num_cus() & ~7;
-  ROMA_REQUIRE(cus >= 8, ROMA_E_UNSUPPORTED, "roma_refiner_block_mid: needs a device with at least 8 compute units");
+  ROMA_REQUIRE(cus >= 8, ROMA_E_UNSUPPORTED, "%s: needs a device with at least 8 compute units", what);
   const unsigned want = (p.ntile + 7u) & ~7u;
   const int grid = want < (unsigned)cus ? (int)want : cus;
-  hipLaunchKernelGGL((refiner_mid_kernel<T>), dim3(grid), dim3(MID_NT), MID_SMEM, s, p);
+  hipLaunchKernelGGL((refiner_mid_kernel<T, L>), dim3(grid), dim3(MID_NT), smem, s, p);
   ROMA_CHECK_LAUNCH();
 }
 
-}
-}
-
-using namespace roma;
-
-extern "C" int roma_refiner_block_mid(const void* x, const float* w25, const float* scale, const float* shift, const void* wt,
-                                      const float* bias, void* y, int B, int C, int H, int W, int dtype, int x_pitch, int y_pitch,
-                                      void* stream) {
-  ROMA_REQUIRE(x && w25 && scale && shift && wt && bias && y, ROMA_E_ARG, "roma_refiner_block_mid: null pointer");
-  ROMA_REQUIRE(B > 0 && C > 0 && H > 0 && W > 0 && x_pitch >= C && y_pitch >= C, ROMA_E_SHAPE, "roma_refiner_block_mid: bad shape");
-  ROMA_REQUIRE(dtype == ROMA_F16 || dtype == ROMA_BF16, ROMA_E_DTYPE, "roma_refiner_block_mid: fp16 / bf16 only");
-  ROMA_REQUIRE(C > 32 && C <= MID_KPAD && C % 8 == 0, ROMA_E_UNSUPPORTED,
-               "roma_refiner_block_mid: C=%d (a multiple of 8, 32 < C <= 160)", C);
+int mid_params(MidParams& p, const char* what, const void* x, const float* w25, const float* scale, const float* shift, const void* wt,
+               const float* bias, void* y, int B, int C, int H, int W, int dtype, int x_pitch, int y_pitch) {
+  ROMA_REQUIRE(B > 0 && C > 0 && H > 0 && W > 0 && x_pitch >= C && y_pitch >= C, ROMA_E_SHAPE, "%s: bad shape", what);
+  ROMA_REQUIRE(dtype == ROMA_F16 || dtype == ROMA_BF16, ROMA_E_DTYPE, "%s: fp16 / bf16 only", what);
+  ROMA_REQUIRE(C > 32 && C <= MID_KPAD && C % 8 == 0, ROMA_E_UNSUPPORTED, "%s: C=%d (a multiple of 8, 32 < C <= 160)", what, C);
   ROMA_REQUIRE(x_pitch % 8 == 0 && y_pitch % 8 == 0 && aligned16(x) && aligned16(y) && aligned16(w25) && aligned16(scale) &&
                    aligned16(shift) && aligned16(wt),
-               ROMA_E_ALIGN, "roma_refiner_block_mid: pitches must be multiples of 8 and bases 16-byte aligned");
+               ROMA_E_ALIGN, "%s: pitches must be multiples of 8 and bases 16-byte aligned", what);
   const size_t npix = (size_t)B * H * W;
   ROMA_REQUIRE(npix * x_pitch * 2 < (1ull << 32) && npix * y_pitch * 2 < (1ull << 32), ROMA_E_SHAPE,
-               "roma_refiner_block_mid: a map of 4 GB or more in one launch");
+               "%s: a map of 4 GB or more in one launch", what);
   const char *xb = static_cast<const char*>(x), *yb = static_cast<const char*>(y);
-  ROMA_REQUIRE(yb + npix * y_pitch * 2 <= xb || xb + npix * x_pitch * 2 <= yb, ROMA_E_ARG, "roma_refiner_block_mid: x and y overlap");
-  MidParams p{x, y, w25, scale, shift, wt, bias, B, H, W, C, x_pitch, y_pitch, 0, 0, 0, 0};
+  ROMA_REQUIRE(!y || yb + npix * y_pitch * 2 <= xb || xb + npix * x_pitch * 2 <= yb, ROMA_E_ARG, "%s: x and y overlap", what);
+  p = MidParams{x, y, w25, scale, shift, wt, bias, B, H, W, C, x_pitch, y_pitch, 0, 0, 0, 0, nullptr, nullptr, nullptr, nullptr, nullptr, 0.f, 0.f};
   const int S0 = MID_NT / (C / 8);
   p.S = S0 < MID_SMAX ? S0 : MID_SMAX;
   p.nstrip = (unsigned)((size_t)B * H * ((W + mid::kStrip - 1) / mid::kStrip));
   p.ntile = (p.nstrip + p.S - 1) / p.S;
   p.band = (p.ntile + 7) / 8;
+  return 0;
+}
+
+}
+}
+
+using namespace roma;
+
+extern "C" int roma_refiner_block_mid(const void* x, const float* w25, const float* scale, const float* shift, const void* wt,
+                                      const float* bias, void* y, int B, int C, int H, int W, int dtype, int x_pitch, int y_pitch,
+                                      void* stream) {
+  const char* what = "roma_refiner_block_mid";
+  ROMA_REQUIRE(x && w25 && scale && shift && wt && bias && y, ROMA_E_ARG, "%s: null pointer", what);
+  MidParams p;
+  if (int rc = mid_params(p, what, x, w25, scale, shift, wt, bias, y, B, C, H, W, dtype, x_pitch, y_pitch)) return rc;
   hipStream_t s = static_cast<hipStream_t>(stream);
-  return dtype == ROMA_F16 ? launch_mid<half_t>(p, s) : launch_mid<bf16_t>(p, s);
-}
+  return dtype == ROMA_F16 ? launch_mid<half_t, 0>(p, s, what) : launch_mid<bf16_t, 0>(p, s, what);
+}
+
+extern "C" int roma_refiner_block_mid_head(const void* x, const float* w25, const float* scale, const float* shift, const void* wt,
+                                           const float* bias, int B, int C, int H, int W, int dtype, int x_pitch, const float* wo,
+                                           const float* bo, float* flow, const float* cert_in, float* cert_out, float sx, float sy,
+                                           void* stream) {
+  const char* what = "roma_refiner_block_mid_head";
+  ROMA_REQUIRE(x && w25 && scale && shift && wt && bias && wo && bo && flow && cert_out, ROMA_E_ARG, "%s: null pointer", what);
+  MidParams p;
+  if (int rc = mid_params(p, what, x, w25, scale, shift, wt, bias, nullptr, B, C, H, W, dtype, x_pitch, x_pitch)) return rc;
+  p.wo = wo; p.bo = bo; p.flow = flow; p.cert_in = cert_in; p.cert_out = cert_out; p.sx = sx; p.sy = sy;
+  hipStream_t s = static_cast<hipStream_t>(stream);
+  if (head::lanes_for(C / 8) == 16) return dtype == ROMA_F16 ? launch_mid<half_t, 16>(p, s, what) : launch_mid<bf16_t, 16>(p, s, what);
+  return dtype == ROMA_F16 ? launch_mid<half_t, 4>(p, s, what) : launch_mid<bf16_t, 4>(p, s, what);
+}
diff --git a/roma_amd/csrc/refiner_wide.hip b/roma_amd/csrc/refiner_wide.hip
--- a/roma_amd/csrc/refiner_wide.hip
+++ b/roma_amd/csrc/refiner_wide.hip
@@ -1,5 +1,6 @@
 #include "common.h"
 #include "lc_device.h"
+#include "refiner_head_device.h"
 
 namespace roma {
 namespace {
@@ -15,6 +16,12 @@
   const float* shift;
   const float* bias;
   int B, H, W, x_pitch, y_pitch, tiles_x, tiles_y;
+  const float* wo;
+  const float* bo;
+  float* flow;
+  const float* cert_in;
+  float* cert_out;
+  float sx, sy;
 };
 
 typedef const __attribute__((address_space(4))) float cfloat;
@@ -24,7 +31,7 @@
 constexpr int PLANE = HYH * HPR * 32 + 16;
 constexpr int NTAPV = 5 * 4 * 2 * 6;
 
-template <typename T, int D>
+template <typename T, int D, bool HEAD>
 __global__ __launch_bounds__(512, 1) void refiner_wide_kernel(RWParams p) {
   constexpr int NKP = D / 32, NB = D / 16, NBW = NB / 4, MBW = 4;
   constexpr int WBUF = D * 64, XBUF = 4 * PLANE, TBUF = TW * TH * 64, DWBUF = NTAPV * 16;
@@ -42,7 +49,7 @@
   const int b = blockIdx.x / tiles, tt = blockIdx.x - b * tiles;
   const int ty0 = (tt / p.tiles_x) * TH, tx0 = (tt % p.tiles_x) * TW;
   const T* xb = static_cast<const T*>(p.x) + (size_t)b * p.H * p.W * p.x_pitch;
-  T* yb = static_cast<T*>(p.y) + (size_t)b * p.H * p.W * p.y_pitch;
+  [[maybe_unused]] T* yb = static_cast<T*>(p.y) + (size_t)b * p.H * p.W * p.y_pitch;
 
   uint32_t xsrc[2], xdst;
   bool xok[2], xuse;
@@ -191,6 +198,32 @@
   constexpr int OPITCH = D * 2 + 16;
   static_assert(TW * TH * OPITCH <= 160 * 1024, "output tile fits LDS");
   unsigned char* s_o = smem;
+  constexpr int PKR = D / 8;
+  static_assert(!HEAD || (PKR > 64 && PKR <= 128), "the head variant: 64 lanes per pixel, two packets per lane at most");
+  [[maybe_unused]] float hw[2][24], hbo[3], hf0 = 0.f, hf1 = 0.f, hc = 0.f;
+  [[maybe_unused]] const int HW = p.H * p.W;
+  [[maybe_unused]] int hidx = -1;
+  if constexpr (HEAD) {
+#pragma unroll
+    for (int j = 0; j < 2; ++j) {
+      const int pk = lane + 64 * j;
+#pragma unroll
+      for (int i = 0; i < 6; ++i) {
+        float4_t v = float4_t{0.f, 0.f, 0.f, 0.f};
+        if (pk < PKR) v = *reinterpret_cast<const float4_t*>(p.wo + pk * 24 + i * 4);
+        hw[j][4 * i] = v[0]; hw[j][4 * i + 1] = v[1]; hw[j][4 * i + 2] = v[2]; hw[j][4 * i + 3] = v[3];
+      }
+    }
+    hbo[0] = p.bo[0]; hbo[1] = p.bo[1]; hbo[2] = p.bo[2];
+    const int oy = ty0 + wave, ox = tx0 + lane;
+    if (lane < TW && oy < p.H && ox < p.W) {
+      hidx = oy * p.W + ox;
+      const float* fl = p.flow + (size_t)b * 2 * HW + hidx;
+      hf0 = fl[0];
+      hf1 = fl[HW];
+      if (p.cert_in) hc = p.cert_in[(size_t)b * HW + hidx];
+    }
+  }
 #pragma unroll
   for (int nb = 0; nb < NBW; ++nb) {
     const int ch = (nq * NBW + nb) * 16 + 4 * kg;
@@ -206,13 +239,51 @@
     }
   }
   __syncthreads();
-  constexpr int PKR = D / 8;
-  for (int id = tid; id < TW * TH * PKR; id += 512) {
-    const int px = id / PKR, pk = id - px * PKR;
-    const int oy = ty0 + (px >> 4), ox = tx0 + (px & 15);
-    if (oy < p.H && ox < p.W)
-      *reinterpret_cast<u32x4*>(yb + (size_t)(oy * p.W + ox) * p.y_pitch + pk * 8) = *reinterpret_cast<const u32x4*>(s_o + px * OPITCH + pk * 16);
-  }
+  if constexpr (HEAD) {
+    float r0 = 0.f, r1 = 0.f, r2 = 0.f;
+#pragma unroll 4
+    for (int i = 0; i < TW; ++i) {
+      const unsigned char* row = s_o + (wave * TW + i) * OPITCH;
+      float a0 = 0.f, a1 = 0.f, a2 = 0.f;
+      head::fma_packet<T>(*reinterpret_cast<const u32x4*>(row + lane * 16), hw[0], a0, a1, a2);
+      if (lane + 64 < PKR) head::fma_packet<T>(*reinterpret_cast<const u32x4*>(row + (lane + 64) * 16), hw[1], a0, a1, a2);
+      head::reduce<64>(a0, a1, a2);
+      if (lane == i) { r0 = a0; r1 = a1; r2 = a2; }
+    }
+    if (hidx >= 0) {
+      float* fl = p.flow + (size_t)b * 2 * HW + hidx;
+      head::finish(r0, r1, r2, hbo, p.sx, p.sy, hf0, hf1, hc);
+      fl[0] = hf0;
+      fl[HW] = hf1;
+      p.cert_out[(size_t)b * HW + hidx] = hc;
+    }
+  } else {
+    for (int id = tid; id < TW * TH * PKR; id += 512) {
+      const int px = id / PKR, pk = id - px * PKR;
+      const int oy = ty0 + (px >> 4), ox = tx0 + (px & 15);
+      if (oy < p.H && ox < p.W)
+        *reinterpret_cast<u32x4*>(yb + (size_t)(oy * p.W + ox) * p.y_pitch + pk * 8) = *reinterpret_cast<const u32x4*>(s_o + px * OPITCH + pk * 16);
+    }
+  }
+}
+
+template <bool HEAD>
+int launch_wide(RWParams p, const char* what, int D, int dtype, const void* w25p, const void* wp, void* stream) {
+  ROMA_REQUIRE(p.B > 0 && p.H > 0 && p.W > 0, ROMA_E_SHAPE, "%s: bad shape", what);
+  ROMA_REQUIRE(D == 576 && dtype == ROMA_F16, ROMA_E_UNSUPPORTED, "%s: built for D = 576, fp16 (got D = %d, dtype %d)", what, D, dtype);
+  ROMA_REQUIRE(p.x_pitch >= D && p.y_pitch >= D && p.x_pitch % 8 == 0 && p.y_pitch % 4 == 0 && aligned16(p.x) && aligned16(wp) &&
+                   aligned16(w25p) && aligned16(p.y) && p.y_pitch % 8 == 0 && aligned16(p.bias) && aligned16(p.wo),
+               ROMA_E_ALIGN, "%s: pitch / alignment", what);
+  ROMA_REQUIRE((size_t)p.H * p.W * p.x_pitch < (1ull << 31), ROMA_E_SHAPE, "%s: map too large for 32-bit offsets", what);
+  p.tiles_x = (p.W + TW - 1) / TW;
+  p.tiles_y = (p.H + TH - 1) / TH;
+  constexpr int smem_loop = 2 * (576 * 64 + 4 * PLANE + TW * TH * 64 + NTAPV * 16), smem_out = TW * TH * (576 * 2 + 16);
+  constexpr int smem = smem_loop > smem_out ? smem_loop : smem_out;
+  static std::atomic<uint64_t> attr_done{0};
+  if (int rc = ensure_dyn_smem(reinterpret_cast<const void*>(refiner_wide_kernel<half_t, 576, HEAD>), smem, attr_done, what)) return rc;
+  hipLaunchKernelGGL((refiner_wide_kernel<half_t, 576, HEAD>), dim3(p.B * p.tiles_x * p.tiles_y), dim3(512), smem,
+                     static_cast<hipStream_t>(stream), p);
+  ROMA_CHECK_LAUNCH();
 }
 
 }
@@ -258,16 +329,16 @@
                                        const float* bias, void* y, int B, int H, int W, int D, int x_pitch, int y_pitch, int dtype,
                                        void* stream) {
   ROMA_REQUIRE(x && w25p && scale && shift && wp && bias && y, ROMA_E_ARG, "roma_refiner_block_wide: null pointer");
-  ROMA_REQUIRE(B > 0 && H > 0 && W > 0, ROMA_E_SHAPE, "roma_refiner_block_wide: bad shape");
-  ROMA_REQUIRE(D == 576 && dtype == ROMA_F16, ROMA_E_UNSUPPORTED, "roma_refiner_block_wide: built for D = 576, fp16 (got D = %d, dtype %d)", D, dtype);
-  ROMA_REQUIRE(x_pitch >= D && y_pitch >= D && x_pitch % 8 == 0 && y_pitch % 4 == 0 && aligned16(x) && aligned16(wp) && aligned16(w25p) &&
-               aligned16(y) && y_pitch % 8 == 0 && aligned16(bias), ROMA_E_ALIGN, "roma_refiner_block_wide: pitch / alignment");
-  ROMA_REQUIRE((size_t)H * W * x_pitch < (1ull << 31), ROMA_E_SHAPE, "roma_refiner_block_wide: map too large for 32-bit offsets");
-  RWParams p{x, y, w25p, wp, scale, shift, bias, B, H, W, x_pitch, y_pitch, (W + TW - 1) / TW, (H + TH - 1) / TH};
-  constexpr int smem_loop = 2 * (576 * 64 + 4 * PLANE + TW * TH * 64 + NTAPV * 16), smem_out = TW * TH * (576 * 2 + 16);
-  constexpr int smem = smem_loop > smem_out ? smem_loop : smem_out;
-  static std::atomic<uint64_t> attr_done{0};
-  if (int rc = ensure_dyn_smem(reinterpret_cast<const void*>(refiner_wide_kernel<half_t, 576>), smem, attr_done, "roma_refiner_block_wide")) return rc;
-  hipLaunchKernelGGL((refiner_wide_kernel<half_t, 576>), dim3(B * p.tiles_x * p.tiles_y), dim3(512), smem, static_cast<hipStream_t>(stream), p);
-  ROMA_CHECK_LAUNCH();
-}
+  RWParams p{x, y, w25p, wp, scale, shift, bias, B, H, W, x_pitch, y_pitch, 0, 0, nullptr, nullptr, nullptr, nullptr, nullptr, 0.f, 0.f};
+  return launch_wide<false>(p, "roma_refiner_block_wide", D, dtype, w25p, wp, stream);
+}
+
+extern "C" int roma_refiner_block_wide_head(const void* x, const void* w25p, const float* scale, const float* shift, const void* wp,
+                                            const float* bias, int B, int H, int W, int D, int x_pitch, int dtype, const float* wo,
+                                            const float* bo, float* flow, const float* cert_in, float* cert_out, float sx, float sy,
+                                            void* stream) {
+  ROMA_REQUIRE(x && w25p && scale && shift && wp && bias && wo && bo && flow && cert_out, ROMA_E_ARG,
+               "roma_refiner_block_wide_head: null pointer");
+  RWParams p{x, nullptr, w25p, wp, scale, shift, bias, B, H, W, x_pitch, x_pitch, 0, 0, wo, bo, flow, cert_in, cert_out, sx, sy};
+  return launch_wide<true>(p, "roma_refiner_block_wide_head", D, dtype, w25p, wp, stream);
+}
diff --git a/roma_amd/matcher.py b/roma_amd/matcher.py
--- a/roma_amd/matcher.py
+++ b/roma_amd/matcher.py
@@ -64,6 +64,17 @@
     if not (half and 32 < Dp <= 160):
         return "two"
     return "one" if B * h * w >= MID_ONE_MIN_PIXELS else "two"
+
+
+def tail_impl(Dp, dtype, B, h, w):
+    impl = block_impl(Dp, dtype, B, h, w)
+    if impl == "wide":
+        return "fused"
+    if impl == "fused":
+        return "fused" if Dp == 24 else "split"
+    if impl == "split_mfma" and mid_block_impl(dtype, Dp, B, h, w) == "one":
+        return "fused"
+    return "split"
 
 
 def project_impl(dtype, channels_last, K, N, out_pitch):
@@ -145,7 +156,7 @@
         return torch.empty((B, h, w, self.prepare(dtype).Dp), dtype=dtype, device=device)
 
     @torch.no_grad()
-    def _body(self, x, y, flow, scale_factor, dtype, buf=None, batch_shift=0):
+    def _body(self, x, y, flow, scale_factor, dtype, buf=None, batch_shift=0, last_block=True):
         P = self.prepare(dtype)
         B, C, h, w = x.shape
         D, Dp = P.D, P.Dp
@@ -178,7 +189,7 @@
         cur = buf
         mid_one = impl == "split_mfma" and mid_block_impl(dtype, Dp, B, h, w) == "one"
         nxt = torch.empty_like(buf) if impl in ("wide", "fused") or mid_one else None
-        for blk in P.blocks[impl]:
+        for blk in P.blocks[impl] if last_block else P.blocks[impl][:-1]:
             if impl == "wide":
                 ops.refiner_block_wide(cur, blk.taps, blk.scale, blk.shift, blk.wt_panels, blk.bias, out=nxt)
                 cur, nxt = nxt, cur
@@ -211,8 +222,23 @@
 
     @torch.no_grad()
     def forward_update(self, x, y, flow, certainty, scale_factor, sx, sy, dtype=None, buf=None, batch_shift=0):
-        cur, P = self._body(x, y, flow, scale_factor, dtype or self.amp_dtype, buf=buf, batch_shift=batch_shift)
-        return ops.refiner_head(cur, P.wo, P.bo, flow, certainty, sx, sy)
+        dtype = dtype or self.amp_dtype
+        B, _, h, w = x.shape
+        Dp = self.prepare(dtype).Dp
+        if tail_impl(Dp, dtype, B, h, w) == "split":
+            cur, P = self._body(x, y, flow, scale_factor, dtype, buf=buf, batch_shift=batch_shift)
+            return ops.refiner_head(cur, P.wo, P.bo, flow, certainty, sx, sy)
+        cur, P = self._body(x, y, flow, scale_factor, dtype, buf=buf, batch_shift=batch_shift, last_block=False)
+        impl = block_impl(Dp, dtype, B, h, w)
+        blk = P.blocks[impl][-1]
+        if impl == "wide":
+            return ops.refiner_block_wide_head(cur, blk.taps, blk.scale, blk.shift, blk.wt_panels, blk.bias, P.wo, P.bo, flow, certainty,
+                                               sx, sy)
+        if impl == "fused":
+            return ops.refiner_block_head(cur, blk.w25, blk.scale, blk.shift, blk.wt_out_in, blk.bias, Dp, P.wo, P.bo, flow, certainty,
+                                          sx, sy)
+        return ops.refiner_block_mid_head(cur, blk.w25, blk.scale, blk.shift, blk.wt_out_in, blk.bias, Dp, P.wo, P.bo, flow, certainty,
+                                          sx, sy)
 
 
 class CosKernel(nn.Module):
diff --git a/roma_amd/ops.py b/roma_amd/ops.py
--- a/roma_amd/ops.py
+++ b/roma_amd/ops.py
@@ -709,6 +709,56 @@
     return (flow, cert, delta) if want_delta else (flow, cert)
 
 
+def _head_args(x_nhwc, wo, bo, flow, certainty):
+    B, h, w, _ = x_nhwc.shape
+    assert flow.shape == (B, 2, h, w) and flow.is_contiguous() and flow.dtype == torch.float32
+    assert wo.is_contiguous() and wo.dtype == torch.float32 and wo.shape[1] == 3 and bo.dtype == torch.float32 and bo.numel() == 3
+    cert_in = None if certainty is None else certainty.float().contiguous()
+    assert cert_in is None or cert_in.numel() == B * h * w
+    return cert_in, torch.empty((B, 1, h, w), dtype=torch.float32, device=flow.device)
+
+
+def refiner_block_head(x_nhwc, w25, scale, shift, wt, bias, C, wo, bo, flow, certainty, sx, sy):
+    _need_gpu(x_nhwc, w25, scale, shift, wt, bias, wo, bo, flow, certainty)
+    B, h, w, pitch = x_nhwc.shape
+    kpad = wt.shape[0]
+    assert x_nhwc.is_contiguous() and wt.is_contiguous() and w25.is_contiguous() and wt.dtype == x_nhwc.dtype == w25.dtype
+    assert w25.shape == (25, kpad) and wt.shape == (kpad, kpad) and scale.numel() == shift.numel() == bias.numel() == kpad
+    assert wo.shape[0] >= C
+    cert_in, cert = _head_args(x_nhwc, wo, bo, flow, certainty)
+    check(_lib.load().roma_refiner_block_head(_p(x_nhwc), _p(w25), _p(scale), _p(shift), _p(wt), _p(bias), B, C, h, w, kpad,
+                                              _dt(x_nhwc), pitch, _p(wo), _p(bo), _p(flow), _p(cert_in), _p(cert), float(sx),
+                                              float(sy), _stream()), "roma_refiner_block_head")
+    return flow, cert
+
+
+def refiner_block_mid_head(x_nhwc, w25, scale, shift, wt, bias, C, wo, bo, flow, certainty, sx, sy):
+    _need_gpu(x_nhwc, w25, scale, shift, wt, bias, wo, bo, flow, certainty)
+    B, h, w, pitch = x_nhwc.shape
+    assert x_nhwc.is_contiguous() and wt.is_contiguous() and w25.is_contiguous() and wt.dtype == x_nhwc.dtype
+    assert w25.shape == (25, C) and wt.shape == (160, 160) and scale.numel() == shift.numel() == C and bias.numel() == 160
+    assert all(t.dtype == torch.float32 and t.is_contiguous() for t in (w25, scale, shift, bias))
+    assert wo.shape[0] >= C
+    cert_in, cert = _head_args(x_nhwc, wo, bo, flow, certainty)
+    check(_lib.load().roma_refiner_block_mid_head(_p(x_nhwc), _p(w25), _p(scale), _p(shift), _p(wt), _p(bias), B, C, h, w,
+                                                  _dt(x_nhwc), pitch, _p(wo), _p(bo), _p(flow), _p(cert_in), _p(cert), float(sx),
+                                                  float(sy), _stream()), "roma_refiner_block_mid_head")
+    return flow, cert
+
+
+def refiner_block_wide_head(x_nhwc, w25p, scale, shift, wp, bias, wo, bo, flow, certainty, sx, sy):
+    _need_gpu(x_nhwc, w25p, scale, shift, wp, bias, wo, bo, flow, certainty)
+    B, H, W, D = x_nhwc.shape
+    assert x_nhwc.is_contiguous() and w25p.shape == (D // 32, 5, 4, 2, 6, 4, 2) and w25p.dtype == x_nhwc.dtype and w25p.is_contiguous()
+    assert all(t.dtype == torch.float32 and t.numel() == D and t.is_contiguous() for t in (scale, shift, bias))
+    assert wo.shape[0] == D
+    cert_in, cert = _head_args(x_nhwc, wo, bo, flow, certainty)
+    check(_lib.load().roma_refiner_block_wide_head(_p(x_nhwc), _p(w25p), _p(scale), _p(shift), _p(wp), _p(bias), B, H, W, D, D,
+                                                   _dt(x_nhwc), _p(wo), _p(bo), _p(flow), _p(cert_in), _p(cert), float(sx),
+                                                   float(sy), _stream()), "roma_refiner_block_wide_head")
+    return flow, cert
+
+
 def pointwise_small(x_rows, wt, bias, out=None):
     _need_gpu(x_rows, wt, bias, out)
     M, C = x_rows.shape
```

Result: no change. 61.02 image-pairs/s (median of 5 runs) (+0.8%).
